# maxnorman569/Variational-Gridded-Gaussian-Processes

Measured on AMD Instinct MI355X. Metric: ELBO-step grid-points/sec (value + 5-component gradient), 1024x1024 RBF grid per GPU, higher is better.
Workload: dtype f64; 1 GPU; 2D Kronecker rbf GP (points basis), 1024x1024 grid (1024x1024 per GPU), m_d=128, Adam fit loop (lr 0.01), eigensolver warm start on; parallelism=single GPU

## Files before the change

include/vggp.h:

```cpp
#ifndef VGGP_H
#define VGGP_H

#include <stdint.h>

#ifdef __cplusplus
extern "C" {
#endif

#define VGGP_VERSION 200

#define VGGP_OK        0
#define VGGP_EINVAL   -1
#define VGGP_ENOTPD   -2
#define VGGP_EHIP     -3
#define VGGP_ENOMEM   -4
#define VGGP_ESTATE   -5
#define VGGP_ENOCONV  -6
#define VGGP_ERCCL    -7

#define VGGP_KIND_MATERN12 0
#define VGGP_KIND_MATERN32 1
#define VGGP_KIND_MATERN52 2
#define VGGP_KIND_RBF      3

#define VGGP_BASIS_POINTS 0
#define VGGP_BASIS_B0     1
#define VGGP_BASIS_ONE    2
#define VGGP_BASIS_VFF    3
#define VGGP_BASIS_B1     4

#define VGGP_FLAG_B0_F32_KDELTA 1
#define VGGP_FLAG_BLOCK_JACOBI 2
#define VGGP_FLAG_SCATTERED 4
#define VGGP_FLAG_PAIRED_Z 8

typedef struct vggp_ctx vggp_ctx;

typedef struct vggp_desc {
    int32_t kind1, basis1;
    int32_t kind2, basis2;
    int64_t n1, n2;
    int64_t m1, m2;
    int64_t n_total;
    const double* x1;
    const double* x2;
    const double* grid1;
    const double* grid2;
    int32_t warm_start;
    int32_t flags;
} vggp_desc;

typedef struct vggp_info {
    double jitter1, jitter2;
    int32_t sweeps1, sweeps2;
    int32_t rounds1, rounds2;
    int32_t status;
    int32_t polished;
} vggp_info;

int         vggp_version(void);
const char* vggp_last_error(void);

#define VGGP_UNIQUE_ID_BYTES 128
int vggp_create(vggp_ctx** out, int device, int n_ranks, int rank, const void* unique_id);
int vggp_destroy(vggp_ctx* ctx);
int vggp_unique_id(void* out );
typedef int (*vggp_allreduce_fn)(void* user, double* buf, int64_t count);
int vggp_set_allreduce(vggp_ctx* ctx, vggp_allreduce_fn fn, void* user);
int vggp_allreduce(vggp_ctx* ctx, double* buf, int64_t count, void* stream);
int vggp_comm_info(const vggp_ctx* ctx, int* n_ranks, int* rank, int* transport);
int vggp_plan(vggp_ctx* ctx, const vggp_desc* desc);
int64_t vggp_payload_len(const vggp_ctx* ctx);
int64_t vggp_workspace_bytes(const vggp_ctx* ctx);

int vggp_elbo_step(vggp_ctx* ctx, const double* Y, double yy_total, const double theta[5],
                   double* elbo_out, double grad_out[5], vggp_info* info, void* stream);

int vggp_elbo_partials(vggp_ctx* ctx, const double* Y, const double theta[5],
                       double* payload, void* stream);
int vggp_elbo_finish(vggp_ctx* ctx, const double* payload, double yy_total, const double theta[5],
                     double* elbo_out, double grad_out[5], vggp_info* info, void* stream);

int vggp_elbo_step_masked(vggp_ctx* ctx, const double* Ym, const double* W, double n_obs, double yy_obs,
                          const double theta[5], double* elbo_out, double grad_out[5], vggp_info* info, void* stream);
int vggp_elbo_step_masked_iter(vggp_ctx* ctx, const double* Ym, const double* W, double n_obs, double yy_obs,
                               const double theta[5], int n_probes, double tol, int max_iter, double* elbo_out, double grad_out[5],
                               vggp_info* info, void* stream);
int vggp_qv_masked(vggp_ctx* ctx, double* mean, double* var, void* stream);
int vggp_posterior_masked(vggp_ctx* ctx, const double* xs1, const double* xs2, int64_t n_star, double* mean, double* var,
                          void* stream);

#define VGGP_READOUT_LITERAL 1
int vggp_readout(vggp_ctx* ctx, const double* C1, int64_t mv1, const double* C2, int64_t mv2, const double* kd1, const double* kd2,
                 double* mean, double* var, int flags, void* stream);

int vggp_readout_masked(vggp_ctx* ctx, const double* C1, int64_t mv1, const double* C2, int64_t mv2, const double* kd1, const double* kd2,
                        double* mean, double* var, int flags, void* stream);

int vggp_qv(vggp_ctx* ctx, double* mean, double* var, void* stream);
int vggp_qv_cov(vggp_ctx* ctx, double* cov, void* stream);

int vggp_zgrad(vggp_ctx* ctx, const double* Y, double* gz1, double* gz2, void* stream);

int vggp_elbo_step_scattered(vggp_ctx* ctx, const double* y, double yy, const double theta[5], double* elbo_out,
                             double grad_out[5], vggp_info* info, void* stream);

int vggp_zgrad_scattered(vggp_ctx* ctx, const double* y, double* gz1, double* gz2, void* stream);

int vggp_set_inducing(vggp_ctx* ctx, int dim, const double* z, int64_t m);

int vggp_posterior(vggp_ctx* ctx, const double* xs1, const double* xs2, int64_t ns,
                   double* mean, double* var, void* stream);

int vggp_posterior_cov(vggp_ctx* ctx, const double* xs1, const double* xs2, int64_t ns, double* cov, void* stream);
int vggp_posterior_cov_masked(vggp_ctx* ctx, const double* xs1, const double* xs2, int64_t ns, double* cov, void* stream);
int vggp_qv_cov_masked(vggp_ctx* ctx, double* cov, void* stream);

int vggp_factor_build(vggp_ctx* ctx, int kind, int basis, const double* x, int64_t n,
                      const double* grid, int64_t m, double ell, int flags,
                      double* A0, double* dA0, double* K0, double* dK0, void* stream);

int vggp_cholesky_inverse(vggp_ctx* ctx, const double* K, int64_t m, double* L, double* Linv,
                          double* jitter_out, void* stream);

int vggp_eigh(vggp_ctx* ctx, const double* G, int64_t m, double* lam, double* Qt,
              int32_t* sweeps_out, int flags, void* stream);

int vggp_gemm(vggp_ctx* ctx, const double* A, int64_t sa_m, int64_t sa_k,
              const double* B, int64_t sb_k, int64_t sb_n,
              double* C, int64_t ldc, int64_t M, int64_t N, int64_t K, void* stream);

int vggp_trsm(vggp_ctx* ctx, const double* L, int64_t m, const double* R, int64_t ncols, double* X, int trans, void* stream);

int vggp_kron_solve(vggp_ctx* ctx, const double* L1, int64_t n1, const double* L2, int64_t n2,
                    const double* Y, double* X, void* stream);

#define VGGP_NSTAGE 20
int         vggp_profile(vggp_ctx* ctx, int enable);
int         vggp_profile_read(vggp_ctx* ctx, double ms_out[VGGP_NSTAGE], int32_t* steps_out, int reset);
const char* vggp_stage_name(int stage);
const char* vggp_project_kernel_name(void);

int vggp_sumsq(vggp_ctx* ctx, const double* y, int64_t n, double* out, void* stream);

#ifdef __cplusplus
}
#endif
#endif
```

variational_gridded_gaussian_processes_amd/_lib.py:

```python
from __future__ import annotations

import ctypes as C
import os

HERE = os.path.dirname(os.path.abspath(__file__))
LIB_PATH = os.path.join(HERE, "libvggp_hip.so")

VGGP_OK, VGGP_EINVAL, VGGP_ENOTPD, VGGP_EHIP, VGGP_ENOMEM, VGGP_ESTATE, VGGP_ENOCONV, VGGP_ERCCL = 0, -1, -2, -3, -4, -5, -6, -7
UNIQUE_ID_BYTES = 128
ALLREDUCE_FN = C.CFUNCTYPE(C.c_int, C.c_void_p, C.POINTER(C.c_double), C.c_int64)
KIND = {"matern12": 0, "matern32": 1, "matern52": 2, "rbf": 3}
NSTAGE = 20
FLAG_B0_F32_KDELTA = 1
FLAG_BLOCK_JACOBI = 2
FLAG_SCATTERED = 4
FLAG_PAIRED_Z = 8
BASIS = {"points": 0, "b0": 1, "one": 2, "vff": 3, "b1": 4}


class VggpError(RuntimeError):
    def __init__(self, code: int, msg: str):
        super().__init__(f"libvggp_hip: {msg} (code {code})")
        self.code = code


class Desc(C.Structure):
    _fields_ = [("kind1", C.c_int32), ("basis1", C.c_int32), ("kind2", C.c_int32), ("basis2", C.c_int32),
                ("n1", C.c_int64), ("n2", C.c_int64), ("m1", C.c_int64), ("m2", C.c_int64),
                ("n_total", C.c_int64),
                ("x1", C.c_void_p), ("x2", C.c_void_p), ("grid1", C.c_void_p), ("grid2", C.c_void_p),
                ("warm_start", C.c_int32), ("flags", C.c_int32)]


class Info(C.Structure):
    _fields_ = [("jitter1", C.c_double), ("jitter2", C.c_double),
                ("sweeps1", C.c_int32), ("sweeps2", C.c_int32),
                ("rounds1", C.c_int32), ("rounds2", C.c_int32),
                ("status", C.c_int32), ("polished", C.c_int32)]


_P, _I64, _D, _I = C.c_void_p, C.c_int64, C.c_double, C.c_int
SYMBOLS = {
    "vggp_version": (_I, []),
    "vggp_last_error": (C.c_char_p, []),
    "vggp_create": (_I, [C.POINTER(_P), _I, _I, _I, _P]),
    "vggp_unique_id": (_I, [_P]),
    "vggp_set_allreduce": (_I, [_P, ALLREDUCE_FN, _P]),
    "vggp_allreduce": (_I, [_P, _P, _I64, _P]),
    "vggp_comm_info": (_I, [_P, C.POINTER(_I), C.POINTER(_I), C.POINTER(_I)]),
    "vggp_destroy": (_I, [_P]),
    "vggp_plan": (_I, [_P, C.POINTER(Desc)]),
    "vggp_payload_len": (_I64, [_P]),
    "vggp_workspace_bytes": (_I64, [_P]),
    "vggp_elbo_step": (_I, [_P, _P, _D, C.POINTER(_D), C.POINTER(_D), C.POINTER(_D), C.POINTER(Info), _P]),
    "vggp_elbo_partials": (_I, [_P, _P, C.POINTER(_D), _P, _P]),
    "vggp_elbo_finish": (_I, [_P, _P, _D, C.POINTER(_D), C.POINTER(_D), C.POINTER(_D), C.POINTER(Info), _P]),
    "vggp_elbo_step_masked": (_I, [_P, _P, _P, _D, _D, C.POINTER(_D), C.POINTER(_D), C.POINTER(_D), C.POINTER(Info), _P]),
    "vggp_elbo_step_masked_iter": (_I, [_P, _P, _P, _D, _D, C.POINTER(_D), _I, _D, _I, C.POINTER(_D), C.POINTER(_D), C.POINTER(Info), _P]),
    "vggp_elbo_step_scattered": (_I, [_P, _P, _D, C.POINTER(_D), C.POINTER(_D), C.POINTER(_D), C.POINTER(Info), _P]),
    "vggp_qv_masked": (_I, [_P, _P, _P, _P]),
    "vggp_qv": (_I, [_P, _P, _P, _P]),
    "vggp_qv_cov": (_I, [_P, _P, _P]),
    "vggp_zgrad": (_I, [_P, _P, _P, _P, _P]),
    "vggp_zgrad_scattered": (_I, [_P, _P, _P, _P, _P]),
    "vggp_set_inducing": (_I, [_P, C.c_int, _P, C.c_int64]),
    "vggp_posterior": (_I, [_P, _P, _P, _I64, _P, _P, _P]),
    "vggp_readout": (_I, [_P, _P, _I64, _P, _I64, _P, _P, _P, _P, _I, _P]),
    "vggp_readout_masked": (_I, [_P, _P, _I64, _P, _I64, _P, _P, _P, _P, _I, _P]),
    "vggp_posterior_masked": (_I, [_P, _P, _P, _I64, _P, _P, _P]),
    "vggp_posterior_cov": (_I, [_P, _P, _P, _I64, _P, _P]),
    "vggp_posterior_cov_masked": (_I, [_P, _P, _P, _I64, _P, _P]),
    "vggp_qv_cov_masked": (_I, [_P, _P, _P]),
    "vggp_factor_build": (_I, [_P, _I, _I, _P, _I64, _P, _I64, _D, _I, _P, _P, _P, _P, _P]),
    "vggp_cholesky_inverse": (_I, [_P, _P, _I64, _P, _P, C.POINTER(_D), _P]),
    "vggp_eigh": (_I, [_P, _P, _I64, _P, _P, C.POINTER(C.c_int32), _I, _P]),
    "vggp_gemm": (_I, [_P, _P, _I64, _I64, _P, _I64, _I64, _P, _I64, _I64, _I64, _I64, _P]),
    "vggp_kron_solve": (_I, [_P, _P, _I64, _P, _I64, _P, _P, _P]),
    "vggp_trsm": (_I, [_P, _P, _I64, _P, _I64, _P, _I, _P]),
    "vggp_sumsq": (_I, [_P, _P, _I64, C.POINTER(_D), _P]),
    "vggp_profile": (_I, [_P, _I]),
    "vggp_profile_read": (_I, [_P, C.POINTER(_D), C.POINTER(C.c_int32), _I]),
    "vggp_stage_name": (C.c_char_p, [_I]),
    "vggp_project_kernel_name": (C.c_char_p, []),
}

_lib = None


def load() -> C.CDLL:
    global _lib
    if _lib is not None:
        return _lib
    if not os.path.exists(LIB_PATH):
        raise ImportError(
            f"{LIB_PATH} not found: build it with `python -m variational_gridded_gaussian_processes_amd.build` "
            "(needs hipcc); there is no CPU fallback")
    lib = C.CDLL(LIB_PATH)
    for name, (res, args) in SYMBOLS.items():
        fn = getattr(lib, name)
        fn.restype = res
        fn.argtypes = args
    _lib = lib
    return lib


def check(rc: int) -> None:
    if rc != VGGP_OK:
        msg = load().vggp_last_error()
        raise VggpError(rc, msg.decode() if msg else "unknown error")
```

variational_gridded_gaussian_processes_amd/build.py:

```python
from __future__ import annotations

import os
import shutil
import subprocess
import sys

HERE = os.path.dirname(os.path.abspath(__file__))
CSRC = os.path.join(HERE, "csrc")
SOURCES = ["api.hip", "gemm.hip", "factor_build.hip", "chol.hip", "trsm.hip", "eigh.hip", "mspace.hip", "thin.hip", "masked.hip", "comm.hip", "paired.hip"]
HEADERS = ["common.h", "ctx.h", "factor_elem.h", "gemm_body.h", os.path.join("..", "..", "include", "vggp.h")]
LIB = os.path.join(HERE, "libvggp_hip.so")


def _stale() -> bool:
    if not os.path.exists(LIB):
        return True
    t = os.path.getmtime(LIB)
    deps = [os.path.join(CSRC, s) for s in SOURCES] + [os.path.normpath(os.path.join(CSRC, h)) for h in HEADERS]
    return any(os.path.getmtime(d) > t for d in deps)


def build(force: bool = False, verbose: bool = False) -> str:
    if not force and not _stale():
        return LIB
    hipcc = shutil.which("hipcc") or "/opt/rocm/bin/hipcc"
    if not os.path.exists(hipcc):
        raise RuntimeError("hipcc not found: libvggp_hip.so cannot be built (ROCm toolchain required)")
    cmd = [hipcc, "--offload-arch=gfx950", "-O3", "-std=c++17", "-shared", "-fPIC", "-o", LIB + ".tmp"] + \
          [os.path.join(CSRC, s) for s in SOURCES] + ["-ldl"]
    if verbose:
        print(" ".join(cmd), file=sys.stderr)
    subprocess.run(cmd, check=True, cwd=CSRC)
    os.replace(LIB + ".tmp", LIB)
    return LIB


if __name__ == "__main__":
    print(build(force="--force" in sys.argv, verbose=True))
```

variational_gridded_gaussian_processes_amd/csrc/api.hip:

```cpp
#include "common.h"

#include <math.h>
#include <stdarg.h>
#include <stdio.h>
#include <stdlib.h>
#include <string.h>
#include <time.h>

#include <algorithm>
#include <vector>

static thread_local char g_err[512] = "";
void vg_set_error(const char* fmt, ...) {
    va_list ap;
    va_start(ap, fmt);
    vsnprintf(g_err, sizeof(g_err), fmt, ap);
    va_end(ap);
}
extern "C" const char* vggp_last_error(void) { return g_err; }
extern "C" int vggp_version(void) { return VGGP_VERSION; }

#include "ctx.h"
#include "factor_elem.h"
#define VG_CHOL_MAXJOBS_HOST 8
#define VG_SP_SLABS 4
#define VG_NEWTON_TOL 1e-12
#define VG_NEWTON_NULL 1e-12
#define VG_NEWTON_CLUSTER 1e-7
#define VG_NEWTON_NOISE 1e-13
#define VG_NEWTON_ACCEPT 1e-11

static void graphs_clear(vggp_ctx* c);
static int vg_quiesce(vggp_ctx* c);

static const char* VG_STAGE_NAMES[VGGP_NSTAGE] = {
    "factor_build", "cholesky_inverse", "trsm_BV(L^-1[A|dA|dK])", "extrap_basis(3 small gemms)", "gemm_project(S=[B2;V2]Y)",
    "gemm_C(B1*S)", "gemm_gram(G,H,Mk)", "reduce_slabs", "warm_first_gemm([Z,G]|TM)", "rowqr|refine", "warm_mid_gemms",
    "ritz_eigh", "warm_last_gemms(->Gw)", "jacobi_eigh+replay(fused)", "gemm_rotate_right", "gemm_rotate_left", "dstage",
    "gemm_betaGram", "final_reduce", "(unused)"};
extern "C" const char* vggp_stage_name(int i) { return (i >= 0 && i < VGGP_NSTAGE) ? VG_STAGE_NAMES[i] : ""; }

#define VG_MARK(id)                                                                                     \
    do {                                                                                                \
        if (c->prof && c->nev < VG_MAXEV) { VG_HIP(hipEventRecord(c->ev[c->nev], st)); c->ev_stage[c->nev++] = (id); } \
    } while (0)

static hipStream_t vg_side(vggp_ctx* c, hipStream_t st) {
    static const bool on = getenv("VGGP_FORK") != nullptr;
    return (c->prof || !on) ? st : c->side_stream;
}
#define VG_FORK(i)                                                                                      \
    do { if (sx != st) { VG_HIP(hipEventRecord(c->ev_fork[i], st)); VG_HIP(hipStreamWaitEvent(sx, c->ev_fork[i], 0)); } } while (0)
#define VG_JOIN_RECORD(i) do { if (sx != st) VG_HIP(hipEventRecord(c->ev_join[i], sx)); } while (0)
#define VG_JOIN_WAIT(i) do { if (sx != st) VG_HIP(hipStreamWaitEvent(st, c->ev_join[i], 0)); } while (0)

int vg_ensure_misc(vggp_ctx* c, size_t bytes) {
    if (c->misc_bytes >= bytes) return VGGP_OK;
    if (c->misc) { VG_HIP(hipFree(c->misc)); c->misc = nullptr; c->misc_bytes = 0; }
    VG_HIP(hipMalloc(&c->misc, bytes));
    c->misc_bytes = bytes;
    return VGGP_OK;
}

extern "C" int vggp_create(vggp_ctx** out, int device, int n_ranks, int rank, const void* unique_id) {
    if (!out) { vg_set_error("vggp_create: null out"); return VGGP_EINVAL; }
    VG_REQUIRE(n_ranks >= 1 && rank >= 0 && rank < n_ranks, "vggp_create: rank %d of %d", rank, n_ranks);
    int ndev = 0;
    VG_HIP(hipGetDeviceCount(&ndev));
    VG_REQUIRE(device >= 0 && device < ndev, "vggp_create: device %d out of range (%d devices)", device, ndev);
    VG_ENTER_DEVICE(device);
    hipDeviceProp_t prop;
    VG_HIP(hipGetDeviceProperties(&prop, device));
    if (strncmp(prop.gcnArchName, "gfx950", 6) != 0) {
        vg_set_error("vggp_create: device %d is %s; this library is built for gfx950 only", device, prop.gcnArchName);
        return VGGP_EHIP;
    }
    VG_HIP(vg_chol_setup());
    VG_HIP(vg_eigh_setup());
    VG_HIP(vg_trsm_setup());
    VG_HIP(vg_thin_tail_setup());
    vggp_ctx* c = new (std::nothrow) vggp_ctx();
    if (!c) { vg_set_error("out of host memory"); return VGGP_ENOMEM; }
    c->device = device;
    const char* ng = getenv("VGGP_NO_GRAPH");
    c->use_graph = !(ng && ng[0] == '1');
    VG_HIP(hipStreamCreate(&c->own_stream));
    VG_HIP(hipStreamCreateWithFlags(&c->side_stream, hipStreamNonBlocking));
    for (int i = 0; i < VG_NFORK; ++i) {
        VG_HIP(hipEventCreateWithFlags(&c->ev_fork[i], hipEventDisableTiming));
        VG_HIP(hipEventCreateWithFlags(&c->ev_join[i], hipEventDisableTiming));
    }
    VG_HIP(hipHostMalloc((void**)&c->h_theta, 8 * sizeof(double), hipHostMallocDefault));
    VG_HIP(hipHostMalloc((void**)&c->h_out, sizeof(HostOut), hipHostMallocDefault));
    VG_HIP(hipHostGetDevicePointer((void**)&c->d_hout, c->h_out, 0));
    VG_HIP(hipHostGetDevicePointer((void**)&c->d_htheta, c->h_theta, 0));
    VG_HIP(hipMalloc((void**)&c->ticket, 4 * sizeof(int)));
    VG_HIP(hipMemset(c->ticket, 0, 4 * sizeof(int)));
    VG_HIP(hipMalloc((void**)&c->sumsq_partial, 1024 * sizeof(double)));
    VG_HIP(hipMalloc((void**)&c->sumsq_out, 8 * sizeof(double)));
    const int rcc = vg_comm_init(c, n_ranks, rank, unique_id);
    if (rcc) { (void)vggp_destroy(c); return rcc; }
    *out = c;
    return VGGP_OK;
}

extern "C" int vggp_destroy(vggp_ctx* c) {
    if (!c) return VGGP_OK;
    VgDeviceGuard guard;
    (void)guard.enter(c->device);
    (void)vg_quiesce(c);
    for (int i = 0; i < 20; ++i) if (c->gexec[i]) (void)hipGraphExecDestroy(c->gexec[i]);
    for (int i = 0; i < VG_MAXEV; ++i) if (c->ev[i]) (void)hipEventDestroy(c->ev[i]);
    for (int i = 0; i < VG_NFORK; ++i) {
        if (c->ev_fork[i]) (void)hipEventDestroy(c->ev_fork[i]);
        if (c->ev_join[i]) (void)hipEventDestroy(c->ev_join[i]);
    }
    if (c->side_stream) (void)hipStreamDestroy(c->side_stream);
    vg_masked_free(c);
    vg_paired_free(c);
    vg_comm_destroy(c);
    if (c->own_stream) (void)hipStreamDestroy(c->own_stream);
    if (c->arena) (void)hipFree(c->arena);
    if (c->misc) (void)hipFree(c->misc);
    if (c->h_theta) (void)hipHostFree(c->h_theta);
    if (c->h_out) (void)hipHostFree(c->h_out);
    if (c->ticket) (void)hipFree(c->ticket);
    if (c->sumsq_partial) (void)hipFree(c->sumsq_partial);
    if (c->sumsq_out) (void)hipFree(c->sumsq_out);
    delete c;
    return VGGP_OK;
}

struct Bump {
    char* base;
    size_t off = 0;
    bool dry;
    template <typename T>
    T* take(size_t count) {
        off = (off + 255) & ~size_t(255);
        T* p = dry ? nullptr : reinterpret_cast<T*>(base + off);
        off += count * sizeof(T);
        return p;
    }
};

static int pick_split(int tiles, int K, int target) {
    int s = (target + tiles - 1) / tiles;
    int maxs = std::max(1, K / (4 * VG_BK));
    return std::max(1, std::min(s, maxs));
}

static long vg_grid_len(int basis, long m) {
    if (basis == VGGP_BASIS_B0) return m + 1;
    if (basis == VGGP_BASIS_VFF) return 2 + (m - 1) / 2 + 1;
    return m;
}
static int vg_uexp(int basis) { return (basis == VGGP_BASIS_VFF || basis == VGGP_BASIS_B1) ? -1 : 1; }

static void layout(vggp_ctx* c, Bump& b) {
    const vggp_desc& D = c->desc;
    const long n1 = D.n1, n2 = D.n2, m1 = D.m1, m2 = D.m2;
    c->out = b.take<double>(8);
    c->theta = b.take<double>(8);
    c->rowpart = b.take<double>(m1 * 8);
    c->r1 = b.take<double>(m1);
    c->r1l = b.take<double>(m1);
    c->r2 = b.take<double>(2 * m2);
    c->r2l = c->r2 + m2;
    c->dotpart = b.take<double>(64 * 4);
    c->ol = b.take<double>(2 * m1);
    for (int k = 0; k < 2; ++k) {
        VgDim& d = c->d[k];
        const long m = d.m, m2e = m + (m & 1);
        d.lam0 = b.take<double>(m);
        d.jitter = b.take<double>(2);
        d.counters = b.take<int>(8);
        d.counters2 = d.counters + 4;
        d.perm = b.take<int>(m2e);
        d.perm2 = b.take<int>(m2e);
        d.lam_s = b.take<double>(m);
        d.status = b.take<int>(2);
    }
    c->invD = b.take<double>(m1 * m2);
    c->beta = b.take<double>(m1 * m2);
    c->bl2 = b.take<double>(m1 * m2);
    c->bl1 = b.take<double>(m1 * m2);
    for (int k = 0; k < 2; ++k) {
        VgDim& d = c->d[k];
        d.E = b.take<double>((long)d.m * d.m);
        d.F = b.take<double>((long)d.m * d.m);
    }
    c->P3 = b.take<double>(3 * m1 * m2);
    c->T3 = b.take<double>(3 * m1 * m2);
    for (int k = 0; k < 2; ++k) {
        VgDim& d = c->d[k];
        const long m = d.m;
        d.TM = b.take<double>(m * m);
        d.TH = b.take<double>(m * m);
        d.Qt = b.take<double>(m * m);
        d.QtPrev = b.take<double>(m * m);
        d.QtPrev2 = b.take<double>(m * m);
        d.U = b.take<double>(m * m);
        d.Ep = b.take<double>(m * m);
        d.Fp = b.take<double>(m * m);
        d.Wp = b.take<double>(m * m);
        d.Id = b.take<double>(m * m);
        d.Gw = b.take<double>(m * m);
        d.GH = b.take<double>(2 * m * m);
        d.Mk = b.take<double>(m * m);
    }
    c->payload_len = 2 * m2 * m2 + 3 * m1 * m2;
    c->payload = b.take<double>(c->payload_len + 8);
    for (int k = 0; k < 2; ++k) {
        VgDim& d = c->d[k];
        const long m = d.m;
        const int glen = (int)vg_grid_len(d.basis, m);
        d.grid = b.take<double>(glen);
        d.K0 = b.take<double>(m * m);
        d.dK0 = b.take<double>(m * m);
        d.L0 = b.take<double>(m * m);
        d.Linv0 = b.take<double>(m * m);
        d.Dinv0 = b.take<double>(((m + 15) / 16) * 256);
        if (m > 128) {
            d.Kc = b.take<double>(4 * m * m); d.Lc = b.take<double>(4 * m * m); d.Dc = b.take<double>(4 * ((m + 15) / 16) * 256);
            d.st8 = b.take<int>(8);
        }
        d.X = b.take<double>(m * m);
        d.chol_scratch = b.take<double>(m * (m + 1));
        d.RQ = b.take<double>(m * m);
        d.RQsq = b.take<double>(m * m);
    }
    c->wq = b.take<double>(2 * m1 * m2);
    for (int k = 0; k < 2; ++k) {
        VgDim& d = c->d[k];
        const long m = d.m, n = d.n, m2e = m + (m & 1);
        d.x = b.take<double>(n);
        d.AD = b.take<double>(2 * m * n);
        d.BV = b.take<double>(2 * m * n);
        static const char* ghe = getenv("VGGP_GH_TARGET");
        d.gh_split = pick_split((int)(((m + 63) / 64) * ((m + 63) / 64)), (int)n, ghe ? atoi(ghe) : 32);
        d.GHslab = b.take<double>((size_t)d.gh_split * 2 * m * m);
        d.gwork = b.take<double>(m2e * (m2e + 1));
        d.max_rounds = (int)(VG_EIG_MAXSWEEP * (m2e - 1));
        d.rotlog = b.take<double2>(vg_eigh_log_bytes((int)m) / sizeof(double2) + 1);
        d.roundlog = b.take<int>(d.max_rounds);
        if (m >= 24 && m <= 256) {
            d.gwork2 = b.take<double>(m2e * (m2e + 1));
            d.rotlog2 = b.take<double2>(vg_eigh_log_bytes((int)m) / sizeof(double2) + 1);
            d.roundlog2 = b.take<int>(d.max_rounds);
            d.Zs = b.take<double>(m * m); d.V1s = b.take<double>(m * m); d.Hs = b.take<double>(m * m); d.Ws = b.take<double>(m * m);
            d.tMV = b.take<double>(VG_THIN_MAXR * m); d.tHV = b.take<double>(VG_THIN_MAXR * m);
            d.tAM = b.take<double>(VG_THIN_MAXR * VG_THIN_MAXR); d.tAH = b.take<double>(VG_THIN_MAXR * VG_THIN_MAXR);
            d.Omega = b.take<double>(VG_THIN_MAXR * m);
        }
    }
    const int st_tiles = (int)(((2 * m2 + 63) / 64) * ((n1 + 63) / 64));
    static const char* ste = getenv("VGGP_ST_TARGET");
    c->st_split = pick_split(st_tiles, (int)n2, ste ? atoi(ste) : 256);
    c->St = b.take<double>((size_t)std::max(c->st_split, VG_SP_SLABS) * 2 * m2 * n1);
    c->Sp = b.take<double>((size_t)VG_SP_SLABS * 2 * m2 * n1);
    const int cc_tiles = (int)(((2 * m1 + 63) / 64) * ((m2 + 63) / 64));
    const char* cce = getenv("VGGP_CC_TARGET");
    c->cc_split = pick_split(cc_tiles, (int)n1, cce ? atoi(cce) : 64);
    c->CCslab = b.take<double>((size_t)c->cc_split * 3 * m1 * m2);
    c->tCV = b.take<double>(3 * m1 * VG_THIN_MAXR);
    c->tAC = b.take<double>(3 * VG_THIN_MAXR * VG_THIN_MAXR + 64);
}

static int check_dim(int kind, int basis, long n, long m, const char* which) {
    VG_REQUIRE(kind >= 0 && kind <= 3, "vggp_plan: bad kind for %s", which);
    VG_REQUIRE(basis >= 0 && basis <= 4, "vggp_plan: bad basis for %s", which);
    VG_REQUIRE(!((basis == VGGP_BASIS_VFF || basis == VGGP_BASIS_B1) && kind != VGGP_KIND_MATERN12),
               "vggp_plan: the VFF and B1 features exist for Matern-1/2 only (%s)", which);
    VG_REQUIRE(!(basis == VGGP_BASIS_VFF && (m < 3 || (m & 1) == 0)), "vggp_plan: VFF needs m = 2M + 1 >= 3 (%s)", which);
    VG_REQUIRE(!(basis == VGGP_BASIS_B1 && m < 2), "vggp_plan: B1 needs at least 2 knots (%s)", which);
    VG_REQUIRE(!(basis == VGGP_BASIS_B0 && kind != VGGP_KIND_MATERN12),
               "vggp_plan: the B0 basis exists for Matern-1/2 only (%s)", which);
    VG_REQUIRE(n >= 1, "vggp_plan: %s has no observations", which);
    VG_REQUIRE(m >= 1 && m <= 256, "vggp_plan: m=%ld for %s outside [1, 256]", m, which);
    VG_REQUIRE(!(basis == VGGP_BASIS_ONE && m != 1), "vggp_plan: BASIS_ONE needs m=1 (%s)", which);
    return VGGP_OK;
}

extern "C" int vggp_plan(vggp_ctx* c, const vggp_desc* desc) {
    if (!c || !desc) { vg_set_error("vggp_plan: null argument"); return VGGP_EINVAL; }
    VG_ENTER_DEVICE(c->device);
    int rc;
    if (desc->flags & VGGP_FLAG_PAIRED_Z) {
        c->planned = false;
        graphs_clear(c);
        VG_HIP(hipDeviceSynchronize());
        c->have_partials = c->have_step = c->have_masked = false;
        c->acc_valid = false; c->last_payload = nullptr;
        c->is_paired = false;
        if ((rc = vg_paired_plan(c, desc))) return rc;
        c->desc = *desc;
        c->desc.x1 = c->desc.x2 = c->desc.grid1 = c->desc.grid2 = nullptr;
        c->desc.n_total = (desc->flags & VGGP_FLAG_SCATTERED) ? desc->n1 : desc->n1 * desc->n2;
        c->payload_len = 0;
        c->is_paired = true;
        c->planned = true;
        return VGGP_OK;
    }
    if (c->is_paired || c->paired) { VG_HIP(hipDeviceSynchronize()); vg_paired_free(c); c->is_paired = false; }
    if ((rc = check_dim(desc->kind1, desc->basis1, desc->n1, desc->m1, "dimension 1"))) return rc;
    if ((rc = check_dim(desc->kind2, desc->basis2, desc->n2, desc->m2, "dimension 2"))) return rc;
    VG_REQUIRE(desc->x1 && desc->x2, "vggp_plan: null coordinate arrays");
    VG_REQUIRE((desc->basis1 == VGGP_BASIS_ONE || desc->grid1) && (desc->basis2 == VGGP_BASIS_ONE || desc->grid2),
               "vggp_plan: null grid arrays");
    if (desc->flags & VGGP_FLAG_SCATTERED)
        VG_REQUIRE(desc->n1 == desc->n2 && desc->basis1 != VGGP_BASIS_ONE && desc->basis2 != VGGP_BASIS_ONE,
                   "vggp_plan: scattered points need n1 == n2 (one coordinate pair per point) and two real dimensions");
    else
        VG_REQUIRE(desc->n_total >= desc->n1 * desc->n2, "vggp_plan: n_total smaller than the local grid");
    VG_REQUIRE(desc->n1 < (1L << 24) && desc->n2 < (1L << 24), "vggp_plan: grid axis too long");
    c->planned = false;
    graphs_clear(c);
    VG_HIP(hipDeviceSynchronize());
    c->warm_run = 0;
    c->refine_next = false;
    c->sub_next = false; c->sub_mode = false; c->sub_r_cap[0] = c->sub_r_cap[1] = 0;
    c->pred_consumed = false;
    c->acc_valid = false; c->last_warm = false; c->last_slabs = false; c->last_payload = nullptr;
    c->last_thin = false; c->thin_off = false; c->thin_block = 0;
    c->cur_newton = 0; c->last_newton = false; c->newton_next = false; c->newton_block = 0; c->newton_iters = 3; c->newton_ok_run = 0;
    c->desc = *desc;
    c->d[0] = VgDim();
    c->d[1] = VgDim();
    c->d[0].kind = desc->kind1; c->d[0].basis = desc->basis1; c->d[0].n = (int)desc->n1; c->d[0].m = (int)desc->m1;
    c->d[1].kind = desc->kind2; c->d[1].basis = desc->basis2; c->d[1].n = (int)desc->n2; c->d[1].m = (int)desc->m2;
    Bump dry{nullptr, 0, true};
    layout(c, dry);
    const size_t need = dry.off + 4096;
    if (need > c->arena_bytes) {
        if (c->arena) { VG_HIP(hipFree(c->arena)); c->arena = nullptr; c->arena_bytes = 0; }
        VG_HIP(hipMalloc(&c->arena, need));
        c->arena_bytes = need;
    }
    Bump wet{reinterpret_cast<char*>(c->arena), 0, false};
    layout(c, wet);
    c->arena_used = wet.off;
    VG_HIP(hipMemset(c->arena, 0, c->arena_used));
    const double one = 1.0;
    for (int k = 0; k < 2; ++k) {
        VgDim& d = c->d[k];
        const double* hx = k == 0 ? desc->x1 : desc->x2;
        const double* hg = k == 0 ? desc->grid1 : desc->grid2;
        VG_HIP(hipMemcpy(d.x, hx, sizeof(double) * d.n, hipMemcpyHostToDevice));
        if (d.basis == VGGP_BASIS_ONE) {
            VG_HIP(hipMemcpy(d.grid, &one, sizeof(double), hipMemcpyHostToDevice));
        } else {
            const int glen = (int)vg_grid_len(d.basis, d.m);
            VG_HIP(hipMemcpy(d.grid, hg, sizeof(double) * glen, hipMemcpyHostToDevice));
        }
    }
    for (int k = 0; k < 2; ++k) VG_HIP(vg_identity_launch(c->d[k].Id, c->d[k].m, nullptr));
    for (int k = 0; k < 2; ++k) {
        VgDim& d = c->d[k];
        if (!d.Omega) continue;
        std::vector<double> om((size_t)VG_THIN_MAXR * d.m);
        unsigned long long z = 0x9E3779B97F4A7C15ull * (unsigned long long)(k + 1);
        for (double& v : om) {
            z += 0x9E3779B97F4A7C15ull;
            unsigned long long x = z;
            x = (x ^ (x >> 30)) * 0xBF58476D1CE4E5B9ull; x = (x ^ (x >> 27)) * 0x94D049BB133111EBull; x ^= x >> 31;
            v = (double)(x >> 11) * (2.0 / 9007199254740992.0) - 1.0;
        }
        VG_HIP(hipMemcpy(d.Omega, om.data(), sizeof(double) * om.size(), hipMemcpyHostToDevice));
    }
    VG_HIP(hipDeviceSynchronize());
    c->desc.x1 = c->desc.x2 = c->desc.grid1 = c->desc.grid2 = nullptr;
    c->have_partials = c->have_step = c->have_masked = false;
    vg_masked_new_plan(c);
    c->planned = true;
    return VGGP_OK;
}

extern "C" int vggp_set_inducing(vggp_ctx* c, int dim, const double* z, int64_t m) {
    if (c && c->is_paired) {
        if (!c->planned) { vg_set_error("context not planned"); return VGGP_ESTATE; }
        VG_ENTER_DEVICE(c->device);
        return vg_paired_set_inducing(c, dim, z, m);
// ... 38 lines not shown
                else
                    vg_gemm_add(&g, q.X + k0, q.sc, 1, Tp, t_k, t_i, q.X + r0, (int)q.sc, (int)q.ncols, (int)rb, (int)kn, 1, 0, 1, 0,
                                -1.0, 1);
            }
            if (nt >= 12) { vg_set_error("trsm_batch: too many jobs"); return VGGP_EINVAL; }
            tj[nt++] = VgTrsmJob{q.L + r0 * q.ldl + r0, q.Dinv + (r0 / 16) * q.dinv_blk, q.X + r0 * q.sk, q.X + r0 * q.sk, q.ldl,
                                 q.dinv_blk, q.dinv_ld, q.sk, q.sc, q.sk, q.sc, q.ncols, (int)rb, q.trans};
        }
        if (g.nprob) VG_HIP(vg_gemm_launch(&g, st));
        if (nt) VG_HIP(vg_trsm_launch(tj, nt, st));
    }
    return VGGP_OK;
}
static int trsm_inplace(const double* L, long m, long ldl, const double* Dinv, double* X, long x_sk, long x_sc, long ncols,
                        int trans, hipStream_t st) {
    VgTrsmSpec q{L, ldl, Dinv, 256, 16, X, x_sk, x_sc, ncols, m, trans};
    return trsm_batch(&q, 1, st);
}

static bool vg_ride(const vggp_ctx* c) {
    static const bool off = getenv("VGGP_NO_RIDE") != nullptr;
    return !off && !c->prof && c->desc.m1 <= 128 && c->desc.m2 <= 128;
}

static int vg_chol_big_enqueue(vggp_ctx* c, const int* dims, int ndims, hipStream_t st) {
    VgCholJob cj[VG_CHOL_MAXJOBS_HOST];
    int nj = 0;
    for (int t = 0; t < ndims; ++t) {
        VgDim& d = c->d[dims[t]];
        VG_HIP(vg_jitcopy_launch(d.K0, d.m, d.Kc, st));
    }
    const long NB = 128;
    for (int stage = 0; stage < 2; ++stage) {
        if (stage == 1) {
            VgTrsmJob tj[8];
            int nt = 0;
            VgGemmBatch g;
            vg_gemm_init(&g);
            for (int t = 0; t < ndims; ++t) {
                VgDim& d = c->d[dims[t]];
                const long m = d.m, mm = m * m, rest = m - NB, nb16 = (m + 15) / 16;
                for (int l = 0; l < 4; ++l) {
                    double* Kl = d.Kc + l * mm;
                    double* Ll = d.Lc + l * mm;
                    tj[nt++] = VgTrsmJob{Ll, d.Dc + l * nb16 * 256, Kl + NB * m, Ll + NB * m, m, 256, 16, 1, m, 1, m, rest, (int)NB, 0};
                    vg_gemm_add(&g, Ll + NB * m, m, 1, Ll + NB * m, 1, m, Kl + NB * m + NB, (int)m, (int)rest, (int)rest, (int)NB, 1, 0, 1, 0, -1.0, 1);
                }
            }
            VG_HIP(vg_trsm_launch(tj, nt, st));
            VG_HIP(vg_gemm_launch(&g, st));
        }
        nj = 0;
        for (int t = 0; t < ndims; ++t) {
            VgDim& d = c->d[dims[t]];
            const long m = d.m, mm = m * m, nb16 = (m + 15) / 16;
            const long o = stage ? NB : 0;
            const int mb = stage ? (int)(m - NB) : (int)NB;
            for (int l = 0; l < 4; ++l) {
                VgCholJob j{d.Kc + l * mm + o * m + o, d.Lc + l * mm + o * m + o, nullptr, d.chol_scratch, nullptr, d.st8 + 2 * l + stage, mb};
                j.ldk = (int)m; j.ldl = (int)m; j.only_level0 = 1;
                j.Dinv_out = d.Dc + l * nb16 * 256 + (o / 16) * 256;
                cj[nj++] = j;
            }
        }
        VG_HIP(vg_chol_launch(cj, nj, st));
    }
    for (int t = 0; t < ndims; ++t) {
        VgDim& d = c->d[dims[t]];
        VG_HIP(vg_cholsel_launch(d.Lc, d.Dc, d.st8, d.m, d.L0, d.Dinv0, d.jitter, d.status, st));
    }
    return VGGP_OK;
}

int vg_partials_enqueue(vggp_ctx* c, const double* Y, double* payload, hipStream_t st, bool reduce, bool extrap, bool fused, bool apply_ns,
                        int early) {
    const long n1 = c->desc.n1, n2 = c->desc.n2, m1 = c->desc.m1, m2 = c->desc.m2;
    VgDim &d1 = c->d[0], &d2 = c->d[1];
    hipStream_t sx = vg_side(c, st);
    VgGemmBatch g;
    VG_MARK(-1);

    VgFactorJob fj[2];
    VgCholJob cj[2];
    static const bool chol_legacy = getenv("VGGP_CHOL_LEGACY") != nullptr;
    const bool dinv_path = d1.m <= VG_TRSM_BLK && d2.m <= VG_TRSM_BLK && !chol_legacy;
    VgClearArgs clr;
    clr.n = 0;
    for (int k = 0; k < 2; ++k) {
        VgDim& d = c->d[k];
        fj[k] = VgFactorJob{d.x, d.grid, d.AD, d.AD + (long)d.m * d.n, d.K0, d.dK0, d.n, d.m, d.kind, d.basis, k, 0.0, c->desc.flags};
        clr.ptr[clr.n] = d.status; clr.nwords[clr.n++] = 2;
        clr.ptr[clr.n] = reinterpret_cast<int*>(d.chol_scratch); clr.nwords[clr.n++] = 16;
        clr.ptr[clr.n] = d.counters; clr.nwords[clr.n++] = 8;
        if (k == 0) { clr.ptr[clr.n] = reinterpret_cast<int*>(c->payload + c->payload_len); clr.nwords[clr.n++] = 2; }
        if (d.st8) { clr.ptr[clr.n] = d.st8; clr.nwords[clr.n++] = 8; }
        cj[k] = VgCholJob{d.K0, d.L0, dinv_path ? nullptr : d.Linv0, d.chol_scratch, d.jitter, d.status, d.m};
        cj[k].Dinv_out = d.Dinv0;
    }
    VG_HIP(vg_factor_build_launch(fj, 2, c->d_htheta, st, c->theta, &clr));
    VG_MARK(0);

    const bool ns_on_chol = extrap && apply_ns && dinv_path;
    VgGemmBatch gns;
    vg_gemm_init(&gns);
    if (ns_on_chol)
        for (int k = 0; k < 2; ++k) {
            VgDim& d = c->d[k];
            vg_gemm_add(&gns, d.Wp, d.m, 1, d.Ep, d.m, 1, d.Fp, d.m, d.m, d.m, d.m, 1, 0, 1, 0, -0.5, 1);
        }
    static const bool chol_big_off = getenv("VGGP_NO_CHOL_BIG") != nullptr;
    const bool any_big = (d1.m > VG_TRSM_BLK || d2.m > VG_TRSM_BLK) && !chol_legacy && !chol_big_off;
    VgGemmBatch gsp;
    vg_gemm_init(&gsp);
    int sp_slabs = 1;
    if (early) {
        const bool ok_fused = fused && !reduce && (vg_ride(c) || c->prof);
        const bool ok_partials = reduce;
        if (!(dinv_path && !any_big && (ok_fused || ok_partials) && Y && sx == st)) {
            vg_set_error("internal: the early projection was requested where it cannot run");
            return VGGP_ESTATE;
        }
        vg_gemm_add(&gsp, d2.AD, n2, 1, Y, n1, 1, c->Sp, (int)n1, (int)(2 * m2), (int)n1, (int)n2, std::min(c->st_split, VG_SP_SLABS), 2L * m2 * n1);
        sp_slabs = gsp.p[0].ksplit;
        if (c->prof) {
            vg_gemm_xcd_group(&gsp, 0);
            VG_HIP(vg_gemm_launch(&gsp, st, VG_GEMM_TAG_GRAM_PROJECT));
            VG_MARK(4);
        }
    }
    if (!any_big) {
        VgGemmBatch gr2 = gns;
        if (early && !c->prof) {
            gr2 = gsp;
            if (ns_on_chol)
                for (int k = 0; k < 2; ++k) {
                    VgDim& d = c->d[k];
                    vg_gemm_add(&gr2, d.Wp, d.m, 1, d.Ep, d.m, 1, d.Fp, d.m, d.m, d.m, d.m, 1, 0, 1, 0, -0.5, 1);
                }
        }
        VG_HIP(vg_chol_launch(cj, 2, st, ((early && !c->prof) || ns_on_chol) ? &gr2 : nullptr));
    } else {
        int big[2], nbig = 0;
        for (int k = 0; k < 2; ++k) {
            if (c->d[k].m > VG_TRSM_BLK) big[nbig++] = k;
            else { cj[k].Linv = nullptr; VG_HIP(vg_chol_launch(&cj[k], 1, st)); }
        }
        const int rcb = vg_chol_big_enqueue(c, big, nbig, st);
        if (rcb) return rcb;
    }
    c->dinv_valid = dinv_path || any_big;
    VG_MARK(1);

    {
        const bool big = d1.m > VG_TRSM_BLK || d2.m > VG_TRSM_BLK;
        if (!big) {
            VgTrsmJob tj[16];
            int nt = 0;
            for (int k = 0; k < 2; ++k) {
                VgDim& d = c->d[k];
                const long mn = (long)d.m * d.n;
                const double* dv = dinv_path ? d.Dinv0 : d.Linv0;
                const long dblk = dinv_path ? 256 : 16L * d.m + 16, dld = dinv_path ? 16 : d.m;
                for (int b = 0; b < 2; ++b)
                    tj[nt++] = VgTrsmJob{d.L0, dv, d.AD + b * mn, d.BV + b * mn, d.m, dblk, dld, d.n, 1, d.n, 1, d.n, d.m, 0};
                tj[nt++] = VgTrsmJob{d.L0, dv, d.dK0, d.X, d.m, dblk, dld, d.m, 1, d.m, 1, d.m, d.m, 0};
                if (dinv_path) {
                    tj[nt] = VgTrsmJob{d.L0, dv, d.L0, d.Linv0, d.m, dblk, dld, d.m, 1, d.m, 1, d.m, d.m, 0};
                    tj[nt++].rhs_ident = 1;
                }
            }
            if (early)
                for (int sl = 0; sl < sp_slabs; ++sl)
                    for (int b = 0; b < 2; ++b) {
                        const long o = (long)sl * 2 * m2 * n1 + (long)b * m2 * n1;
                        tj[nt++] = VgTrsmJob{d2.L0, d2.Dinv0, c->Sp + o, c->St + o, m2, 256, 16, n1, 1, n1, 1, n1, (int)m2, 0};
                    }
            VG_HIP(vg_trsm_launch(tj, nt, st));
        } else {
            VgTrsmSpec q[8];
            int nq = 0;
            for (int k = 0; k < 2; ++k) {
                VgDim& d = c->d[k];
                const long mn = (long)d.m * d.n;
                const double* dv = any_big ? d.Dinv0 : d.Linv0;
                const long dblk = any_big ? 256 : 16L * d.m + 16, dld = any_big ? 16 : d.m;
                VG_HIP(hipMemcpyAsync(d.BV, d.AD, sizeof(double) * 2 * mn, hipMemcpyDeviceToDevice, st));
                VG_HIP(hipMemcpyAsync(d.X, d.dK0, sizeof(double) * d.m * d.m, hipMemcpyDeviceToDevice, st));
                for (int b = 0; b < 2; ++b) q[nq++] = VgTrsmSpec{d.L0, d.m, dv, dblk, dld, d.BV + b * mn, d.n, 1, d.n, d.m, 0};
                q[nq++] = VgTrsmSpec{d.L0, d.m, dv, dblk, dld, d.X, d.m, 1, d.m, d.m, 0};
                if (any_big) {
                    VG_HIP(hipMemcpyAsync(d.Linv0, d.Id, sizeof(double) * d.m * d.m, hipMemcpyDeviceToDevice, st));
                    q[nq++] = VgTrsmSpec{d.L0, d.m, dv, dblk, dld, d.Linv0, d.m, 1, d.m, d.m, 0};
                }
            }
            const int rc = trsm_batch(q, nq, st);
            if (rc) return rc;
        }
    }
    VG_MARK(2);

    if (!Y) {
        vg_gemm_init(&g);
        for (int k = 0; k < 2; ++k) {
            VgDim& d = c->d[k];
            vg_gemm_add(&g, d.X, d.m, 1, d.Linv0, 1, d.m, d.Mk, d.m, d.m, d.m, d.m);
        }
        VG_HIP(vg_gemm_launch(&g, st));
        return VGGP_OK;
    }
    hipStream_t sp = (fused && !extrap) ? sx : st;
    const bool ride = fused && !reduce && sp == st && vg_ride(c);
    if (sp != st) VG_FORK(1);
    VgGemmBatch gp, gc;
    vg_gemm_init(&gp);
    vg_gemm_add(&gp, d2.BV, n2, 1, Y, n1, 1, c->St, (int)n1, (int)(2 * m2), (int)n1, (int)n2, c->st_split, 2L * m2 * n1);
    const int st_slabs = early ? sp_slabs : gp.p[0].ksplit;
    vg_gemm_xcd_group(&gp, 0);
    auto add_ns = [&](VgGemmBatch* b) {
        if (extrap && apply_ns && !ns_on_chol)
            for (int k = 0; k < 2; ++k) {
                VgDim& d = c->d[k];
                vg_gemm_add(b, d.Wp, d.m, 1, d.Ep, d.m, 1, d.Fp, d.m, d.m, d.m, d.m, 1, 0, 1, 0, -0.5, 1);
            }
    };
    if (!ride && !early) {
        add_ns(&gp);
        VG_HIP(vg_gemm_launch(&gp, sp, VG_GEMM_TAG_GRAM_PROJECT));
        if (sp == st) VG_MARK(4);
    }
    vg_gemm_init(&gc);
    const long cc_slab = 3L * m1 * m2;
    vg_gemm_add(&gc, d1.BV, n1, 1, c->St, 1, n1, c->CCslab, (int)m2, (int)(2 * m1), (int)m2, (int)n1, c->cc_split, cc_slab,
                st_slabs, 2L * m2 * n1);
    vg_gemm_add(&gc, d1.BV, n1, 1, c->St + m2 * n1, 1, n1, c->CCslab + 2 * m1 * m2, (int)m2, (int)m1, (int)m2, (int)n1,
                c->cc_split, cc_slab, st_slabs, 2L * m2 * n1);
    const int cc_slabs = gc.p[0].ksplit;
    int gh_slabs[2] = {1, 1};
    auto add_gram = [&](VgGemmBatch* b) {
        for (int k = 0; k < 2; ++k) {
            VgDim& d = c->d[k];
            const int ig = vg_gemm_add(b, d.BV, d.n, 1, d.BV, 1, d.n, d.GHslab, d.m, 2 * d.m, d.m, d.n, d.gh_split, 2L * d.m * d.m);
            gh_slabs[k] = b->p[ig].ksplit;
            vg_gemm_add(b, d.X, d.m, 1, d.Linv0, 1, d.m, d.Mk, d.m, d.m, d.m, d.m);
        }
    };
    if (ride) {
        vg_gemm_init(&g);
        add_gram(&g);
        add_ns(&g);
        VG_HIP(vg_gemm_launch(&g, st));
        c->ride_proj = gp; c->ride_cc = gc;
        c->ride_pending = early != 1;
        c->ride_stage0 = early == 2 ? 1 : 0;
    } else {
        if (sp == st) add_gram(&gc);
        VG_HIP(vg_gemm_launch(&gc, sp));
        if (sp == st) { VG_MARK(5); VG_MARK(6); }
        if (sp != st) {
            VG_JOIN_RECORD(1);
            vg_gemm_init(&g);
            add_gram(&g);
            VG_HIP(vg_gemm_launch(&g, st));
            VG_MARK(6);
        }
    }

    c->gh_slabs[0] = gh_slabs[0]; c->gh_slabs[1] = gh_slabs[1]; c->cc_slabs = cc_slabs; c->st_slabs = st_slabs;
    if (!reduce) return VGGP_OK;
    if (sp != st) VG_JOIN_WAIT(1);
    VgRedBatch r;
    vg_red_init(&r);
    vg_red_add(&r, d1.GHslab, d1.GH, 2L * m1 * m1, 2L * m1 * m1, gh_slabs[0]);
    vg_red_add(&r, d2.GHslab, payload, 2L * m2 * m2, 2L * m2 * m2, gh_slabs[1]);
    vg_red_add(&r, c->CCslab, payload + 2 * m2 * m2, 3L * m1 * m2, cc_slab, cc_slabs);
    VG_HIP(vg_red_launch(&r, st));
    VG_MARK(7);
    return VGGP_OK;
}

static bool vg_sub_ident() { static const bool ex = getenv("VGGP_SUB_EXTRAP") != nullptr; return !ex; }

static int finish_enqueue(vggp_ctx* c, const double* payload, double yy_total, bool warm, hipStream_t st, bool copy_theta,
                          bool from_slabs = false, bool extrap = false, bool refine = false, bool subspace = false, bool thin = false,
                          int newton = 0, bool thin_early = false) {
    if (copy_theta) VG_HIP(hipMemcpyAsync(c->theta, c->h_theta, 6 * sizeof(double), hipMemcpyHostToDevice, st));
    const long m1 = c->desc.m1, m2 = c->desc.m2;
    VgDim &d1 = c->d[0], &d2 = c->d[1];
    const double* G0[2] = {from_slabs ? d1.GHslab : d1.GH, from_slabs ? d2.GHslab : payload};
    const double* H0[2] = {G0[0] + m1 * m1, G0[1] + m2 * m2};
    const double* C3 = from_slabs ? c->CCslab : payload + 2 * m2 * m2;
    const int ghn[2] = {from_slabs ? c->gh_slabs[0] : 1, from_slabs ? c->gh_slabs[1] : 1};
    const long ghs[2] = {2L * m1 * m1, 2L * m2 * m2};
    const int ccn = from_slabs ? c->cc_slabs : 1;
    const long ccs = 3L * m1 * m2;
    VgGemmBatch g;
    const bool ride = from_slabs && c->ride_pending;
    int ride_stage = ride ? c->ride_stage0 : 0;

    hipStream_t sx = vg_side(c, st);
    VG_MARK(-1);
    const double* Hr[2] = {H0[0], H0[1]};
    int hrn[2] = {ghn[0], ghn[1]};
    VgEigJob ej[2];
    if (warm && subspace && thin) {
        const bool early = thin_early && !ride;
        const double* Gr[2] = {G0[0], G0[1]};
        int grn[2] = {ghn[0], ghn[1]};
        double* gdst[2] = {d1.GH, c->payload};
        vg_gemm_init(&g);
        for (int k = 0; k < 2; ++k) {
            VgDim& d = c->d[k];
            vg_gemm_add(&g, d.QtPrev, d.m, 1, G0[k], d.m, 1, d.TM, d.m, d.sub_r, d.m, d.m, 1, 0, ghn[k], ghs[k]);
            if (from_slabs && ghn[k] > 1) {
                vg_gemm_add(&g, d.Id, d.m, 1, G0[k], d.m, 1, gdst[k], d.m, d.m, d.m, d.m, 1, 0, ghn[k], ghs[k]);
                vg_gemm_add(&g, d.Id, d.m, 1, H0[k], d.m, 1, gdst[k] + (long)d.m * d.m, d.m, d.m, d.m, d.m, 1, 0, ghn[k], ghs[k]);
            }
        }
        VG_HIP(vg_gemm_launch(&g, st));
        VG_MARK(8);
        for (int k = 0; k < 2; ++k)
            if (from_slabs && ghn[k] > 1) { Gr[k] = gdst[k]; grn[k] = 1; Hr[k] = gdst[k] + (long)c->d[k].m * c->d[k].m; hrn[k] = 1; }
        VgRowQrJob qj[2];
        for (int k = 0; k < 2; ++k) { VgDim& d = c->d[k]; qj[k] = VgRowQrJob{d.TM, d.V1s, d.sub_r, d.m, nullptr, nullptr, 0}; }
        VG_HIP(vg_rowqr_launch(qj, 2, st, early ? ((c->prof || !from_slabs) ? nullptr : &c->ride_cc) : (ride ? &c->ride_proj : nullptr)));
        if (ride) ride_stage = 1;
        VG_MARK(9);
        vg_gemm_init(&g);
        for (int k = 0; k < 2; ++k) {
            VgDim& d = c->d[k];
            const int r = d.sub_r;
            vg_gemm_add(&g, d.V1s, d.m, 1, Gr[k], d.m, 1, d.Zs, d.m, r, d.m, d.m, 1, 0, grn[k], ghs[k]);
            vg_gemm_add(&g, d.V1s, d.m, 1, d.Mk, d.m, 1, d.tMV, d.m, r, d.m, d.m);
            vg_gemm_add(&g, d.V1s, d.m, 1, Hr[k], d.m, 1, d.tHV, d.m, r, d.m, d.m, 1, 0, hrn[k], ghs[k]);
        }
        if (early) {
            const int ic = vg_gemm_add(&g, C3, m2, 1, d2.V1s, 1, m2, c->tCV, d2.sub_r, (int)(3 * m1), d2.sub_r, (int)m2);
            g.p[ic].a_nslab = ccn; g.p[ic].a_slab = ccs;
        }
        VG_HIP(vg_gemm_launch(&g, st));
        VG_MARK(10);
        VgGemmBatch gx;
        vg_gemm_init(&gx);
        if (ride) gx = c->ride_cc;
        for (int k = 0; k < 2; ++k) {
            VgDim& d = c->d[k];
            const int r = d.sub_r;
            vg_gemm_add(&gx, d.tMV, d.m, 1, d.V1s, 1, d.m, d.tAM, r, r, r, d.m);
            vg_gemm_add(&gx, d.tHV, d.m, 1, d.V1s, 1, d.m, d.tAH, r, r, r, d.m);
        }
        if (early)
            for (int q = 0; q < 3; ++q)
                vg_gemm_add(&gx, d1.V1s, m1, 1, c->tCV + (long)q * m1 * d2.sub_r, d2.sub_r, 1, c->tAC + (long)q * d1.sub_r * d2.sub_r,
                            d2.sub_r, d1.sub_r, d2.sub_r, (int)m1);
        VgEigJob sj[2];
        for (int k = 0; k < 2; ++k) {
            VgDim& d = c->d[k];
            sj[k] = VgEigJob{nullptr, d.lam_s, d.Ws, nullptr, d.gwork2, d.rotlog2, d.roundlog2, d.counters2, d.sub_r, d.max_rounds,
                             (long)vg_eigh_log_bytes(d.m), 0};
            sj[k].Hl = d.Zs; sj[k].Hr = d.V1s; sj[k].hk = d.m;
            sj[k].perm = d.perm2;
            sj[k].err = d.status + 1;
            sj[k].newton = 1;
        }
        VG_HIP(vg_eigh_launch(sj, 2, st, &gx));
        if (ride) ride_stage = 2;
        c->ride_pending = false;
        VG_MARK(11);
        const int ac_nslab = 1;
        const long ac_slab = 3L * d1.sub_r * d2.sub_r;
        if (!early) {
            vg_gemm_init(&g);
            {
                const int ic = vg_gemm_add(&g, C3, m2, 1, d2.V1s, 1, m2, c->tCV, d2.sub_r, (int)(3 * m1), d2.sub_r, (int)m2);
                g.p[ic].a_nslab = ccn; g.p[ic].a_slab = ccs;
            }
            for (int k = 0; k < 2; ++k) {
                VgDim& d = c->d[k];
                vg_gemm_add(&g, d.Ws, d.sub_r, 1, d.V1s, d.m, 1, d.QtPrev, d.m, d.sub_r, d.m, d.sub_r);
            }
            VG_HIP(vg_gemm_launch(&g, st));
            VG_MARK(14);
            vg_gemm_init(&g);
            for (int q = 0; q < 3; ++q)
                vg_gemm_add(&g, d1.V1s, m1, 1, c->tCV + (long)q * m1 * d2.sub_r, d2.sub_r, 1, c->tAC + (long)q * d1.sub_r * d2.sub_r, d2.sub_r,
                            d1.sub_r, d2.sub_r, (int)m1);
            VG_HIP(vg_gemm_launch(&g, st));
            VG_MARK(15);
        }
        VgThinTail tt{};
        tt.theta = c->theta; tt.n_total = (double)c->desc.n_total; tt.yy = yy_total;
        tt.r1 = d1.sub_r; tt.r2 = d2.sub_r; tt.m1 = (int)m1; tt.m2 = (int)m2;
        tt.W1 = d1.Ws; tt.W2 = d2.Ws; tt.lam1 = d1.lam_s; tt.lam2 = d2.lam_s;
        tt.AM1 = d1.tAM; tt.AH1 = d1.tAH; tt.AM2 = d2.tAM; tt.AH2 = d2.tAH; tt.AC = c->tAC;
        tt.ac_nslab = ac_nslab; tt.ac_slab = ac_slab;
        tt.G1 = Gr[0]; tt.H1 = Hr[0]; tt.G2 = Gr[1]; tt.H2 = Hr[1];
        tt.out = c->out; tt.hout = c->d_hout;
        tt.beta_out = c->beta; tt.invd_out = c->invD;
        tt.peer_fail = (payload == c->payload && (c->n_ranks > 1 || c->comm || c->cb)) ? c->payload + c->payload_len : nullptr;
        for (int k = 0; k < 2; ++k) { tt.jit[k] = c->d[k].jitter; tt.status[k] = c->d[k].status; tt.rcounters[k] = c->d[k].counters2; }
#ifdef VGGP_DIAG
        tt.stamps = reinterpret_cast<unsigned long long*>(c->tAC + 3 * VG_THIN_MAXR * VG_THIN_MAXR);
#endif
        VG_HIP(vg_thin_tail_launch(&tt, st));
        VG_MARK(18);
        if (early) {
            vg_gemm_init(&g);
            for (int k = 0; k < 2; ++k) {
                VgDim& d = c->d[k];
                vg_gemm_add(&g, d.Ws, d.sub_r, 1, d.V1s, d.m, 1, d.QtPrev, d.m, d.sub_r, d.m, d.sub_r);
            }
            VG_HIP(vg_gemm_launch(&g, st));
        }
        return VGGP_OK;
    }
    if (warm && subspace) {
        VgRowQrJob qj[2];
        const double* Gr[2] = {G0[0], G0[1]};
        int grn[2] = {ghn[0], ghn[1]};
        double* gdst[2] = {d1.GH, c->payload};
        vg_gemm_init(&g);
        for (int k = 0; k < 2; ++k) {
            VgDim& d = c->d[k];
            vg_gemm_add(&g, d.Fp, d.m, 1, G0[k], d.m, 1, d.TM, d.m, d.m, d.m, d.m, 1, 0, ghn[k], ghs[k]);
            if (from_slabs && ghn[k] > 1) {
                vg_gemm_add(&g, d.Id, d.m, 1, G0[k], d.m, 1, gdst[k], d.m, d.m, d.m, d.m, 1, 0, ghn[k], ghs[k]);
                vg_gemm_add(&g, d.Id, d.m, 1, H0[k], d.m, 1, gdst[k] + (long)d.m * d.m, d.m, d.m, d.m, d.m, 1, 0, ghn[k], ghs[k]);
            }
        }
        VG_HIP(vg_gemm_launch(&g, st));
        VG_MARK(8);
        for (int k = 0; k < 2; ++k)
            if (from_slabs && ghn[k] > 1) { Gr[k] = gdst[k]; grn[k] = 1; Hr[k] = gdst[k] + (long)c->d[k].m * c->d[k].m; hrn[k] = 1; }
        for (int k = 0; k < 2; ++k) {
            VgDim& d = c->d[k];
            const long r = d.sub_r;
            qj[k] = VgRowQrJob{d.TM, d.V1s, d.sub_r, d.m, d.Fp + r * d.m, d.E + r * d.m, (long)(d.m - r) * d.m};
        }
        VG_HIP(vg_rowqr_launch(qj, 2, st, ride ? &c->ride_proj : nullptr));
        if (ride) ride_stage = 1;
        VG_MARK(9);
        vg_gemm_init(&g);
        for (int k = 0; k < 2; ++k) {
            VgDim& d = c->d[k];
            const long r = d.sub_r;
            vg_gemm_add(&g, d.V1s, d.m, 1, Gr[k], d.m, 1, d.Zs, d.m, (int)r, d.m, d.m, 1, 0, grn[k], ghs[k]);
            vg_gemm_add(&g, d.Fp + r * d.m, d.m, 1, d.V1s, 1, d.m, d.TH, (int)r, (int)(d.m - r), (int)r, d.m);
        }
        VG_HIP(vg_gemm_launch(&g, st));
        VG_MARK(10);
        VgGemmBatch gx;
        vg_gemm_init(&gx);
        if (ride) gx = c->ride_cc;
        for (int k = 0; k < 2; ++k) {
            VgDim& d = c->d[k];
            const long r = d.sub_r;
            vg_gemm_add(&gx, d.TH, r, 1, d.V1s, d.m, 1, d.E + r * d.m, d.m, (int)(d.m - r), d.m, (int)r, 1, 0, 1, 0, -1.0, 1);
            vg_gemm_add(&gx, d.TH, r, 1, d.Zs, d.m, 1, d.TM + r * d.m, d.m, (int)(d.m - r), d.m, (int)r, 1, 0, 1, 0, -1.0, 1);
        }
        VgEigJob sj[2];
        for (int k = 0; k < 2; ++k) {
            VgDim& d = c->d[k];
            sj[k] = VgEigJob{nullptr, d.lam_s, d.Ws, nullptr, d.gwork2, d.rotlog2, d.roundlog2, d.counters2, d.sub_r, d.max_rounds,
                             (long)vg_eigh_log_bytes(d.m), 0};
            sj[k].Hl = d.Zs; sj[k].Hr = d.V1s; sj[k].hk = d.m;
            sj[k].perm = d.perm2;
            sj[k].err = d.status + 1;
            sj[k].newton = 1;
        }
        VG_HIP(vg_eigh_launch(sj, 2, st, &gx));
        if (ride) ride_stage = 2;
        VG_MARK(11);
        vg_gemm_init(&g);
        for (int k = 0; k < 2; ++k) {
            VgDim& d = c->d[k];
            const long r = d.sub_r;
            vg_gemm_add(&g, d.Ws, r, 1, d.V1s, d.m, 1, d.E, d.m, (int)r, d.m, (int)r);
            vg_gemm_add(&g, d.Ws, r, 1, d.Zs, d.m, 1, d.TM, d.m, (int)r, d.m, (int)r);
        }
        VG_HIP(vg_gemm_launch(&g, st));
        vg_gemm_init(&g);
        for (int k = 0; k < 2; ++k) {
            VgDim& d = c->d[k];
            vg_gemm_add(&g, d.TM, d.m, 1, d.E, 1, d.m, d.Gw, d.m, d.m, d.m, d.m);
        }
        VG_HIP(vg_gemm_launch(&g, st));
    } else if (warm && newton > 0) {
        const double* Gr[2] = {G0[0], G0[1]};
        int grn[2] = {ghn[0], ghn[1]};
        double* gdst[2] = {d1.GH, c->payload};
        const double* Scur[2] = {extrap ? d1.Fp : d1.QtPrev, extrap ? d2.Fp : d2.QtPrev};
        vg_gemm_init(&g);
        for (int k = 0; k < 2; ++k) {
            VgDim& d = c->d[k];
            vg_gemm_add(&g, Scur[k], d.m, 1, G0[k], d.m, 1, d.TM, d.m, d.m, d.m, d.m, 1, 0, ghn[k], ghs[k]);
            if (from_slabs && ghn[k] > 1) {
                vg_gemm_add(&g, d.Id, d.m, 1, G0[k], d.m, 1, gdst[k], d.m, d.m, d.m, d.m, 1, 0, ghn[k], ghs[k]);
                vg_gemm_add(&g, d.Id, d.m, 1, H0[k], d.m, 1, gdst[k] + (long)d.m * d.m, d.m, d.m, d.m, d.m, 1, 0, ghn[k], ghs[k]);
            }
        }
        VG_HIP(vg_gemm_launch(&g, st));
        VG_MARK(8);
        for (int k = 0; k < 2; ++k)
            if (from_slabs && ghn[k] > 1) { Gr[k] = gdst[k]; grn[k] = 1; Hr[k] = gdst[k] + (long)c->d[k].m * c->d[k].m; hrn[k] = 1; }
        vg_gemm_init(&g);
        for (int k = 0; k < 2; ++k) { VgDim& d = c->d[k]; vg_gemm_add(&g, d.TM, d.m, 1, Scur[k], 1, d.m, d.Gw, d.m, d.m, d.m, d.m); }
        VG_HIP(vg_gemm_launch(&g, st));
        VG_MARK(12);
        static const bool newton_null = getenv("VGGP_NO_NULL_SKIP") == nullptr;
        int bi = 0;
        for (int it = 0; it < newton; ++it) {
            VgRefineJob rj[2];
            for (int k = 0; k < 2; ++k) {
                VgDim& d = c->d[k];
                rj[k] = VgRefineJob{d.Gw, d.U, d.TH, d.m, VG_NEWTON_TOL};
                rj[k].emax = 0.3; rj[k].flag = d.counters2; rj[k].noise = VG_NEWTON_NOISE;
                if (newton_null) { rj[k].lam_prev = d.lam0; rj[k].null_cut = it == 0 ? VG_NEWTON_CLUSTER : VG_NEWTON_NULL; }
            }
            const VgGemmBatch* rd = !ride ? nullptr : (ride_stage == 0 ? &c->ride_proj : (ride_stage == 1 ? &c->ride_cc : nullptr));
            VG_HIP(vg_refine_launch(rj, 2, st, rd));
            if (rd) ++ride_stage;
            VG_MARK(9);
            vg_gemm_init(&g);
            for (int k = 0; k < 2; ++k) { VgDim& d = c->d[k]; vg_gemm_add(&g, d.U, d.m, 1, d.U, d.m, 1, d.TH, d.m, d.m, d.m, d.m, 1, 0, 1, 0, 0.5, 1); }
            VG_HIP(vg_gemm_launch(&g, st));
            double* Snew[2];
            vg_gemm_init(&g);
            for (int k = 0; k < 2; ++k) {
                VgDim& d = c->d[k];
                double* bufs[3] = {d.E, d.X, d.F};
                Snew[k] = bufs[bi];
                vg_gemm_add(&g, d.TH, d.m, 1, Scur[k], d.m, 1, Snew[k], d.m, d.m, d.m, d.m);
            }
            VG_HIP(vg_gemm_launch(&g, st));
            bi = (bi + 1) % 3;
            if (it + 1 < newton) {
                double* Sns[2];
                vg_gemm_init(&g);
                for (int k = 0; k < 2; ++k) {
                    VgDim& d = c->d[k];
                    double* bufs[3] = {d.E, d.X, d.F};
                    Sns[k] = bufs[bi];
                    vg_gemm_add(&g, Snew[k], d.m, 1, Snew[k], 1, d.m, d.TM, d.m, d.m, d.m, d.m);
                    vg_gemm_add(&g, d.Id, d.m, 1, Snew[k], d.m, 1, Sns[k], d.m, d.m, d.m, d.m, 1, 0, 1, 0, 1.5, 0);
                }
                VG_HIP(vg_gemm_launch(&g, st));
                vg_gemm_init(&g);
                for (int k = 0; k < 2; ++k) { VgDim& d = c->d[k]; vg_gemm_add(&g, d.TM, d.m, 1, Snew[k], d.m, 1, Sns[k], d.m, d.m, d.m, d.m, 1, 0, 1, 0, -0.5, 1); }
                VG_HIP(vg_gemm_launch(&g, st));
                bi = (bi + 1) % 3;
                for (int k = 0; k < 2; ++k) Scur[k] = Sns[k];
            } else {
                for (int k = 0; k < 2; ++k) Scur[k] = Snew[k];
            }
            vg_gemm_init(&g);
            for (int k = 0; k < 2; ++k) { VgDim& d = c->d[k]; vg_gemm_add(&g, Scur[k], d.m, 1, Gr[k], d.m, 1, d.TM, d.m, d.m, d.m, d.m, 1, 0, grn[k], ghs[k]); }
            VG_HIP(vg_gemm_launch(&g, st));
            vg_gemm_init(&g);
            for (int k = 0; k < 2; ++k) { VgDim& d = c->d[k]; vg_gemm_add(&g, d.TM, d.m, 1, Scur[k], 1, d.m, d.Gw, d.m, d.m, d.m, d.m); }
            VG_HIP(vg_gemm_launch(&g, st));
        }
        VgNewtonCheckJob nj[2];
        for (int k = 0; k < 2; ++k) {
            VgDim& d = c->d[k];
            nj[k] = VgNewtonCheckJob{d.Gw, d.lam0, d.counters, d.status + 1, d.counters2, d.m, newton, VG_NEWTON_ACCEPT, VG_NEWTON_NOISE};
            if (newton_null) nj[k].null_cut = VG_NEWTON_NULL;
            VG_HIP(hipMemcpyAsync(d.Qt, Scur[k], sizeof(double) * d.m * d.m, hipMemcpyDeviceToDevice, st));
        }
        VG_HIP(vg_newton_check_launch(nj, 2, st));
        {
            const int* er[2] = {d1.status + 1, d2.status + 1};
            const double* sa[2] = {Scur[0], Scur[1]};
            double* da[2] = {d1.QtPrev, d2.QtPrev};
            const double* sb[2] = {d1.QtPrev, d2.QtPrev};
            double* db[2] = {d1.QtPrev2, d2.QtPrev2};
            const long nn[2] = {m1 * m1, m2 * m2};
            VG_HIP(vg_copy_if_launch(er, sa, da, sb, db, nn, 2, st));
        }
        VG_MARK(13);
        while (ride && ride_stage < 2) {
            VG_HIP(vg_gemm_launch(ride_stage == 0 ? &c->ride_proj : &c->ride_cc, st));
            ++ride_stage;
        }
    } else if (warm) {
        const double* Gr[2] = {G0[0], G0[1]};
        int grn[2] = {ghn[0], ghn[1]};
        double* gdst[2] = {d1.GH, c->payload};
        vg_gemm_init(&g);
        for (int k = 0; k < 2; ++k) {
            VgDim& d = c->d[k];
            vg_gemm_add(&g, extrap ? d.Fp : d.QtPrev, d.m, 1, G0[k], d.m, 1, d.TM, d.m, d.m, d.m, d.m, 1, 0, ghn[k], ghs[k]);
            if (from_slabs && ghn[k] > 1) {
                if (refine) {
                    vg_gemm_add(&g, d.Id, d.m, 1, G0[k], d.m, 1, gdst[k], d.m, d.m, d.m, d.m, 1, 0, ghn[k], ghs[k]);
                    Gr[k] = gdst[k]; grn[k] = 1;
                }
                vg_gemm_add(&g, d.Id, d.m, 1, H0[k], d.m, 1, gdst[k] + (long)d.m * d.m, d.m, d.m, d.m, d.m, 1, 0, ghn[k], ghs[k]);
                Hr[k] = gdst[k] + (long)d.m * d.m; hrn[k] = 1;
            }
        }
        VG_HIP(vg_gemm_launch(&g, st));
        VG_MARK(8);
        vg_gemm_init(&g);
        for (int k = 0; k < 2; ++k) {
            VgDim& d = c->d[k];
            vg_gemm_add(&g, d.TM, d.m, 1, extrap ? d.Fp : d.QtPrev, 1, d.m, d.Gw, d.m, d.m, d.m, d.m);
        }
        VG_HIP(vg_gemm_launch(&g, st));
        VG_MARK(12);
        if (refine) {
            VgRefineJob rj[2];
            static const bool null_skip = getenv("VGGP_NO_NULL_SKIP") == nullptr;
            for (int k = 0; k < 2; ++k) {
                VgDim& d = c->d[k];
                rj[k] = VgRefineJob{d.Gw, d.U, d.TH, d.m, 0.0};
                if (null_skip) { rj[k].lam_prev = d.lam0; rj[k].null_cut = 1e-12; }
            }
            {
                const VgGemmBatch* rr = !ride ? nullptr : (ride_stage == 0 ? &c->ride_proj : (ride_stage == 1 ? &c->ride_cc : nullptr));
                VG_HIP(vg_refine_launch(rj, 2, st, rr));
                if (rr) ++ride_stage;
            }
            VG_MARK(9);
            vg_gemm_init(&g);
            for (int k = 0; k < 2; ++k) {
                VgDim& d = c->d[k];
                const double* S0 = extrap ? d.Fp : d.QtPrev;
                vg_gemm_add(&g, d.TH, d.m, 1, S0, d.m, 1, d.E, d.m, d.m, d.m, d.m);
                vg_gemm_add(&g, d.U, d.m, 1, d.U, d.m, 1, d.X, d.m, d.m, d.m, d.m);
            }
            VG_HIP(vg_gemm_launch(&g, st));
            vg_gemm_init(&g);
            for (int k = 0; k < 2; ++k) {
                VgDim& d = c->d[k];
                const double* S0 = extrap ? d.Fp : d.QtPrev;
                vg_gemm_add(&g, d.X, d.m, 1, S0, d.m, 1, d.E, d.m, d.m, d.m, d.m, 1, 0, 1, 0, 0.5, 1);
            }
            VG_HIP(vg_gemm_launch(&g, st));
            vg_gemm_init(&g);
            for (int k = 0; k < 2; ++k) {
                VgDim& d = c->d[k];
                vg_gemm_add(&g, d.E, d.m, 1, Gr[k], d.m, 1, d.TM, d.m, d.m, d.m, d.m, 1, 0, grn[k], ghs[k]);
            }
            VG_HIP(vg_gemm_launch(&g, st));
            vg_gemm_init(&g);
            for (int k = 0; k < 2; ++k) {
                VgDim& d = c->d[k];
                vg_gemm_add(&g, d.TM, d.m, 1, d.E, 1, d.m, d.Gw, d.m, d.m, d.m, d.m);
            }
            VG_HIP(vg_gemm_launch(&g, st));
        }
    }
    VG_MARK(12);
    for (int k = 0; k < 2; ++k) {
        VgDim& d = c->d[k];
        ej[k] = VgEigJob{warm ? d.Gw : G0[k], d.lam0, d.Qt, warm ? ((refine || subspace) ? d.E : (extrap ? d.Fp : d.QtPrev)) : nullptr, d.gwork, d.rotlog, d.roundlog,
                         d.counters, d.m, d.max_rounds, (long)vg_eigh_log_bytes(d.m),
                         (c->desc.flags & VGGP_FLAG_BLOCK_JACOBI) ? 1 : 0};
        ej[k].Qt2 = d.QtPrev;
        ej[k].perm = d.perm;
        ej[k].cp_src = d.QtPrev; ej[k].cp_dst = d.QtPrev2;
        ej[k].err = d.status + 1;
        ej[k].polish0 = (warm && refine) ? 1 : 0;
        ej[k].sparse_first = (warm && subspace) ? 1 : 0;
        ej[k].null_from = (warm && subspace) ? d.sub_r : 0;
    }
    const VgGemmBatch* mr = !ride ? nullptr : (ride_stage == 0 ? &c->ride_proj : (ride_stage == 1 ? &c->ride_cc : nullptr));
    if (!(warm && newton > 0)) {
        VG_HIP(vg_eigh_launch(ej, 2, st, mr));
        VG_MARK(13);
        if (mr) ++ride_stage;
    }
    if (ride && ride_stage == 1) { VG_HIP(vg_gemm_launch(&c->ride_cc, st)); ride_stage = 2; }
    c->ride_pending = false;
    if (from_slabs) VG_JOIN_WAIT(1);

    vg_gemm_init(&g);
    for (int k = 0; k < 2; ++k) {
        VgDim& d = c->d[k];
        vg_gemm_add(&g, d.Mk, d.m, 1, d.Qt, 1, d.m, d.TM, d.m, d.m, d.m, d.m);
        const int ih = vg_gemm_add(&g, Hr[k], d.m, 1, d.Qt, 1, d.m, d.TH, d.m, d.m, d.m, d.m);
        g.p[ih].a_nslab = hrn[k]; g.p[ih].a_slab = ghs[k];
    }
    const int ic = vg_gemm_add(&g, C3, m2, 1, d2.Qt, 1, m2, c->T3, (int)m2, (int)(3 * m1), (int)m2, (int)m2);
    g.p[ic].a_nslab = ccn; g.p[ic].a_slab = ccs;
    const bool predict = c->desc.warm_start && !(c->desc.flags & VGGP_FLAG_BLOCK_JACOBI);
    const bool pred_ident = c->sub_mode && vg_sub_ident();
    if (predict && !pred_ident)
        for (int k = 0; k < 2; ++k) {
            VgDim& d = c->d[k];
            vg_gemm_add(&g, d.QtPrev, d.m, 1, d.QtPrev2, 1, d.m, d.U, d.m, d.m, d.m, d.m);
        }
    VG_HIP(vg_gemm_launch(&g, st));
    VG_MARK(14);
    vg_gemm_init(&g);
    for (int k = 0; k < 2; ++k) {
        VgDim& d = c->d[k];
        vg_gemm_add(&g, d.Qt, d.m, 1, d.TM, d.m, 1, d.E, d.m, d.m, d.m, d.m);
        vg_gemm_add(&g, d.Qt, d.m, 1, d.TH, d.m, 1, d.F, d.m, d.m, d.m, d.m);
    }
    for (int q = 0; q < 3; ++q)
        vg_gemm_add(&g, d1.Qt, m1, 1, c->T3 + q * m1 * m2, m2, 1, c->P3 + q * m1 * m2, (int)m2, (int)m1, (int)m2, (int)m1);
    if (predict)
        for (int k = 0; k < 2; ++k) {
            VgDim& d = c->d[k];
            const double* Uk = pred_ident ? d.Id : d.U;
            vg_gemm_add(&g, Uk, d.m, 1, d.QtPrev, d.m, 1, d.Ep, d.m, d.m, d.m, d.m);
            vg_gemm_add(&g, Uk, d.m, 1, d.QtPrev, d.m, 1, d.Fp, d.m, d.m, d.m, d.m, 1, 0, 1, 0, 1.5, 0);
        }
    VG_HIP(vg_gemm_launch(&g, st));
    VG_MARK(15);

    VgMspace ms;
    ms.theta = c->theta; ms.lam1 = d1.lam0; ms.lam2 = d2.lam0; ms.P3 = c->P3;
    ms.E1 = d1.E; ms.F1 = d1.F; ms.E2 = d2.E; ms.F2 = d2.F;
    ms.beta = c->beta; ms.bl2 = c->bl2; ms.bl1 = c->bl1; ms.invD = c->invD;
    ms.rowpart = c->rowpart; ms.r1 = c->r1; ms.r1l = c->r1l; ms.out = c->out;
    ms.r2 = c->r2; ms.r2l = c->r2l; ms.dotp = c->dotpart; ms.ol = c->ol;
    ms.m1 = (int)m1; ms.m2 = (int)m2; ms.n_total = (double)c->desc.n_total; ms.yy = yy_total;
    ms.ticket = c->ticket; ms.hout = c->d_hout;
    ms.peer_fail = (payload == c->payload && (c->n_ranks > 1 || c->comm || c->cb)) ? c->payload + c->payload_len : nullptr;
    for (int k = 0; k < 2; ++k) { ms.jit[k] = c->d[k].jitter; ms.status[k] = c->d[k].status; ms.counters[k] = c->d[k].counters; }
    VG_HIP(vg_dstage_launch(&ms, st));
    VG_MARK(16);
    vg_gemm_init(&g);
    {
        const int idot[4] = {
            vg_gemm_add(&g, d1.E, 1, m1, c->beta, m2, 1, nullptr, (int)m2, (int)m1, (int)m2, (int)m1),
            vg_gemm_add(&g, d1.F, 1, m1, c->bl2, m2, 1, nullptr, (int)m2, (int)m1, (int)m2, (int)m1),
            vg_gemm_add(&g, c->beta, m2, 1, d2.E, m2, 1, nullptr, (int)m2, (int)m1, (int)m2, (int)m2),
            vg_gemm_add(&g, c->bl1, m2, 1, d2.F, m2, 1, nullptr, (int)m2, (int)m1, (int)m2, (int)m2)};
        for (int q = 0; q < 4; ++q) { g.p[idot[q]].dotw = c->beta; g.p[idot[q]].dotw_ld = (int)m2; g.p[idot[q]].dot_out = c->dotpart + 64 * q; }
        vg_gemm_add(&g, c->ol, m1, 1, c->invD, m2, 1, c->r2, (int)m2, 2, (int)m2, (int)m1);
    }
    if (predict)
        for (int k = 0; k < 2; ++k) {
            VgDim& d = c->d[k];
            vg_gemm_add(&g, d.Ep, d.m, 1, d.Ep, 1, d.m, d.Wp, d.m, d.m, d.m, d.m);
        }
    VG_HIP(vg_gemm_launch(&g, st));
    VG_MARK(17);
    VG_HIP(vg_final_launch(&ms, st));
    VG_MARK(18);

    return VGGP_OK;
}

enum { VG_G_PARTIALS = 0, VG_G_PARTIALS_X, VG_G_FINISH_COLD, VG_G_FINISH_WARM, VG_G_FINISH_WARM_X, VG_G_STEP_COLD, VG_G_STEP_WARM,
       VG_G_STEP_WARM_X, VG_G_FINISH_WARM_XR, VG_G_STEP_WARM_XR, VG_G_FINISH_WARM_S, VG_G_STEP_WARM_S, VG_G_FINISH_WARM_T, VG_G_STEP_WARM_T,
       VG_G_FINISH_WARM_N, VG_G_STEP_WARM_N, VG_G_PARTIALS_E, VG_G_FINISH_WARM_TE, VG_G_STEP_COLD_T, VG_G_PARTIALS_XE, VG_G_COUNT };
static_assert(VG_G_COUNT <= 20, "vggp_ctx::gexec");

static void graphs_clear(vggp_ctx* c) {
    (void)vg_quiesce(c);
    for (int i = 0; i < VG_G_COUNT; ++i) {
        if (c->gexec[i]) { (void)hipGraphExecDestroy(c->gexec[i]); c->gexec[i] = nullptr; }
        c->gkey[i] = VgGraphKey();
    }
}

template <typename F>
static int run_graph(vggp_ctx* c, int which, const VgGraphKey& key, hipStream_t st, F enqueue, bool bypass = false) {
    if (!c->use_graph || c->prof || bypass) return enqueue();
    if (!c->gexec[which] || !(c->gkey[which] == key)) {
        if (c->gexec[which]) { (void)vg_quiesce(c); (void)hipGraphExecDestroy(c->gexec[which]); c->gexec[which] = nullptr; }
        VG_HIP(hipStreamBeginCapture(st, hipStreamCaptureModeThreadLocal));
        const int rc = enqueue();
        hipGraph_t graph = nullptr;
        const hipError_t e = hipStreamEndCapture(st, &graph);
        if (rc) { if (graph) (void)hipGraphDestroy(graph); return rc; }
        if (e != hipSuccess) { vg_set_error("hipStreamEndCapture -> %s", hipGetErrorString(e)); return VGGP_EHIP; }
        const hipError_t ei = hipGraphInstantiate(&c->gexec[which], graph, nullptr, nullptr, 0);
        (void)hipGraphDestroy(graph);
        if (ei != hipSuccess) { c->gexec[which] = nullptr; vg_set_error("hipGraphInstantiate -> %s", hipGetErrorString(ei)); return VGGP_EHIP; }
        c->gkey[which] = key;
    }
    VG_HIP(hipGraphLaunch(c->gexec[which], st));
    return VGGP_OK;
}

static bool vg_refine(const vggp_ctx* c, bool extrap) {
    static const bool off = getenv("VGGP_NO_REFINE") != nullptr;
    return !off && extrap && c->refine_next;
}

static bool vg_extrapolate(const vggp_ctx* c) {
    static const bool off = getenv("VGGP_NO_EXTRAP") != nullptr;
    return !off && c->desc.warm_start && !(c->desc.flags & VGGP_FLAG_BLOCK_JACOBI) && c->d[0].have_prev && c->d[1].have_prev &&
           c->d[0].have_prev2 && c->d[1].have_prev2;
}

struct VgStart { bool extrap, refine, subspace, thin; int newton; };
static bool vg_thin_ok(const vggp_ctx* c, bool own_payload) {
    static const bool off = getenv("VGGP_NO_THIN") != nullptr;
    if (off || c->thin_off || c->thin_block > 0 || !own_payload || !c->desc.warm_start || (c->desc.flags & VGGP_FLAG_BLOCK_JACOBI) || !c->sub_next) return false;
    for (int k = 0; k < 2; ++k) {
        const VgDim& d = c->d[k];
        if (!d.have_prev || !d.tMV || d.sub_r < 1 || d.sub_r > VG_THIN_MAXR || d.sub_r > d.thin_rows) return false;
    }
    return true;
}
static bool vg_warm(vggp_ctx* c, bool own_payload) {
    bool warm = c->desc.warm_start && c->d[0].have_prev && c->d[1].have_prev;
    if (warm && (c->d[0].thin_rows < c->d[0].m || c->d[1].thin_rows < c->d[1].m) && !vg_thin_ok(c, own_payload)) {
        c->warm_run = 0;
        for (int k = 0; k < 2; ++k) c->d[k].have_prev = c->d[k].have_prev2 = false;
        warm = false;
    }
    return warm;
}
static int vg_start_prepare(vggp_ctx* c, bool warm, hipStream_t st, VgStart* out, bool own_payload) {
    out->thin = warm && vg_thin_ok(c, own_payload);
    out->extrap = !out->thin && vg_extrapolate(c);
    const bool lds_sized = c->d[0].m <= 128 && c->d[1].m <= 128;
    out->subspace = out->thin || (lds_sized && warm && out->extrap && c->sub_next && c->d[0].sub_r > 0 && c->d[1].sub_r > 0);
    {
        static const bool off = getenv("VGGP_NO_NEWTON_CHAIN") != nullptr;
        static const char* ite = getenv("VGGP_NEWTON_ITERS");
        const bool big = c->d[0].m > 128 || c->d[1].m > 128;
        const bool roomy = c->d[0].m >= 96 && c->d[1].m >= 96;
        const bool want = warm && !out->subspace && out->extrap && !off && c->newton_block == 0 && (big || (c->newton_next && roomy)) &&
                          !(c->desc.flags & VGGP_FLAG_BLOCK_JACOBI) && c->d[0].m >= 8 && c->d[1].m >= 8;
        out->newton = want ? (ite ? atoi(ite) : c->newton_iters) : 0;
        if (c->newton_block > 0) --c->newton_block;
    }
    out->refine = warm && !out->subspace && !out->newton && vg_refine(c, out->extrap);
    c->sub_mode = out->subspace;
    if (out->subspace && (c->sub_r_cap[0] != c->d[0].sub_r || c->sub_r_cap[1] != c->d[1].sub_r)) {
        for (int v : {(int)VG_G_FINISH_WARM_S, (int)VG_G_STEP_WARM_S, (int)VG_G_FINISH_WARM_T, (int)VG_G_STEP_WARM_T, (int)VG_G_FINISH_WARM_TE})
            if (c->gexec[v]) { (void)vg_quiesce(c); (void)hipGraphExecDestroy(c->gexec[v]); c->gexec[v] = nullptr; c->gkey[v] = VgGraphKey(); }
        c->sub_r_cap[0] = c->d[0].sub_r; c->sub_r_cap[1] = c->d[1].sub_r;
    }
    if (out->newton && out->newton != c->newton_cap) {
        for (int v : {(int)VG_G_FINISH_WARM_N, (int)VG_G_STEP_WARM_N})
            if (c->gexec[v]) { (void)vg_quiesce(c); (void)hipGraphExecDestroy(c->gexec[v]); c->gexec[v] = nullptr; c->gkey[v] = VgGraphKey(); }
        c->newton_cap = out->newton;
    }
    c->cur_thin = out->thin;
    c->cur_extrap = out->extrap;
    c->cur_newton = out->newton;
    c->cur_r[0] = c->d[0].sub_r; c->cur_r[1] = c->d[1].sub_r;
    return VGGP_OK;
}

static int set_theta(vggp_ctx* c, const double theta[5]) {
    for (int i = 0; i < 5; ++i) {
        VG_REQUIRE(theta[i] > 0.0 && std::isfinite(theta[i]), "theta[%d]=%g must be positive and finite", i, theta[i]);
        c->h_theta[i] = theta[i];
    }
    c->h_theta[5] = (double)(++c->seq);
    return VGGP_OK;
}

static int vg_quiesce(vggp_ctx* c) {
    if (c->poll_stream_valid) { c->poll_stream_valid = false; VG_HIP(hipStreamSynchronize(c->poll_stream)); }
    return VGGP_OK;
}
static int vg_wait_step(vggp_ctx* c, hipStream_t st) {
    static const bool nopoll = getenv("VGGP_NO_POLL") != nullptr;
    const volatile double* seq = &c->h_out->seq;
    const double want = c->h_theta[5];
    if (nopoll || c->prof || (c->n_ranks > 1 && !c->comm && !c->cb)) { c->poll_stream_valid = false; return vg_comm_wait(c, st); }
    if (c->comm && !c->cb) {
        const int wrc = vg_comm_wait(c, st, seq, want);
        c->poll_stream = st; c->poll_stream_valid = (wrc == VGGP_OK);
        return wrc;
    }
    timespec t0, t1;
    clock_gettime(CLOCK_MONOTONIC, &t0);
    for (long spin = 0;; ++spin) {
        if (*seq == want) {
            __atomic_thread_fence(__ATOMIC_ACQUIRE);
            c->poll_stream = st; c->poll_stream_valid = true;
            return VGGP_OK;
        }
        __builtin_ia32_pause();
        if ((spin & 4095) == 4095) {
            clock_gettime(CLOCK_MONOTONIC, &t1);
            if ((double)(t1.tv_sec - t0.tv_sec) + 1e-9 * (double)(t1.tv_nsec - t0.tv_nsec) > 0.02) break;
        }
    }
    c->poll_stream_valid = false;
    VG_HIP(hipStreamSynchronize(st));
    return VGGP_OK;
}

static int finish_collect(vggp_ctx* c, double* elbo_out, double grad_out[5], vggp_info* info, hipStream_t st) {
    {
        const int wrc = vg_wait_step(c, st);
        if (wrc) {
            c->warm_run = 0;
            for (int k = 0; k < 2; ++k) c->d[k].have_prev = c->d[k].have_prev2 = false;
            c->have_step = false;
            return wrc;
        }
    }
    c->pred_consumed = false;
    c->acc_valid = false;
    if (c->prof && c->nev > 1) {
        for (int i = 1; i < c->nev; ++i) {
            const int id = c->ev_stage[i];
            float ms = 0.f;
            if (id >= 0 && id < VGGP_NSTAGE && hipEventElapsedTime(&ms, c->ev[i - 1], c->ev[i]) == hipSuccess) c->prof_ms[id] += ms;
        }
        c->prof_steps++;
    }
    c->nev = 0;
    if (c->h_out->seq != c->h_theta[5]) {
        vg_set_error("step %.0f: the result block carries sequence number %.0f (stale results)", c->h_theta[5], c->h_out->seq);
        c->warm_run = 0;
        for (int k = 0; k < 2; ++k) c->d[k].have_prev = c->d[k].have_prev2 = false;
        c->have_step = false;
        return VGGP_ESTATE;
    }
    if (c->h_out->out[6] != 0.0) {
        vg_set_error("rank %d / %d: %.0f rank(s) of the job failed their half of this step; the result is discarded", c->rank,
                     c->n_ranks, c->h_out->out[6]);
        c->warm_run = 0;
        for (int k = 0; k < 2; ++k) c->d[k].have_prev = c->d[k].have_prev2 = false;
        c->have_step = false;
        return VGGP_ERCCL;
    }
    *elbo_out = c->h_out->out[0];
    for (int i = 0; i < 5; ++i) grad_out[i] = c->h_out->out[1 + i];
    int status = 0;
    for (int k = 0; k < 2; ++k) {
        if (c->h_out->status[k]) status = c->h_out->status[k];
        else if (c->h_out->counters[k][2]) status = c->h_out->counters[k][2];
    }
    if (info) {
        info->jitter1 = c->h_out->jitter[0]; info->jitter2 = c->h_out->jitter[1];
        info->sweeps1 = c->h_out->counters[0][1] & 0xff; info->sweeps2 = c->h_out->counters[1][1] & 0xff;
        info->rounds1 = c->h_out->counters[0][0]; info->rounds2 = c->h_out->counters[1][0];
        info->status = status;
        info->polished = ((c->h_out->counters[0][3] >> 28) & 1) | (((c->h_out->counters[1][3] >> 28) & 1) << 1);
    }
    {
        static const bool off = getenv("VGGP_NO_SUBSPACE") != nullptr;
        bool ok = !status && !off && c->desc.warm_start && !(c->desc.flags & VGGP_FLAG_BLOCK_JACOBI);
        for (int k = 0; k < 2; ++k) {
            VgDim& d = c->d[k];
            const int rank = (c->h_out->counters[k][1] >> 8) & 0x1ff;
            int want = 0;
            static const bool relax = getenv("VGGP_NO_SUB_RELAX") == nullptr;
            if (d.Zs && rank >= 1 && 3 * rank <= d.m) {
                static const bool m8 = getenv("VGGP_SUB_MARGIN8") != nullptr;
                want = m8 ? ((rank + 4 + 7) / 8) * 8 : ((rank + 3 + 1) / 2) * 2;
                if (want < 16) want = 16;
                if (want > 64 || 2 * want > d.m) want = 0;
            } else if (relax && d.Zs && rank >= 1 && d.m <= 64 && rank + 2 <= d.m - 8) {
                want = ((rank + 2 + 3) / 4) * 4;
                if (want > d.m - 8) want = d.m - 8;
                if (want < 8 || want > 48) want = 0;
            }
            if (d.m > 128 && want > VG_THIN_MAXR) want = 0;
            if (want == 0) d.sub_r = 0;
            else if (want > d.sub_r || want < d.sub_r - 8) d.sub_r = want;
            ok = ok && d.sub_r > 0;
        }
        c->sub_next = ok;
    }
    c->refine_next = !status && ((c->h_out->counters[0][3] >> 28) & 1) && ((c->h_out->counters[1][3] >> 28) & 1) &&
                     (c->h_out->counters[0][1] & 0xff) <= 1 && (c->h_out->counters[1][1] & 0xff) <= 1;
    if (status == VG_ESUBMISS && c->cur_newton) {
        static const bool dbg = getenv("VGGP_NEWTON_DBG") != nullptr;
        if (dbg)
            fprintf(stderr, "[vggp] step %ld: Newton chain (%d iterations) missed: dim1 flags %d, 10 log10(offdiag / thr) = %d; dim2 flags %d, %d\n",
                    c->seq, c->cur_newton, c->h_out->counters[0][3] & 0xff, (c->h_out->counters[0][3] >> 8) - 100,
                    c->h_out->counters[1][3] & 0xff, (c->h_out->counters[1][3] >> 8) - 100);
        c->newton_block = (c->d[0].m > 128 || c->d[1].m > 128) ? 2 : 16; c->newton_next = false;
        if (c->newton_iters < 5) ++c->newton_iters;
        c->newton_ok_run = 0;
        c->have_step = false;
        return VG_ESUBMISS;
    }
    if (status) {
        c->warm_run = 0;
        for (int k = 0; k < 2; ++k) c->d[k].have_prev = c->d[k].have_prev2 = false;
        c->have_step = false;
    }
    if (status == VG_ESUBMISS) {
        c->sub_next = false;
        if (c->cur_thin) c->thin_block = 32;
        return VG_ESUBMISS;
    }
    if (status == VGGP_ENOTPD) { vg_set_error("a Kuu factor is not positive definite after jitter 1e-6"); return VGGP_ENOTPD; }
    if (status == VGGP_ENOCONV) { vg_set_error("Jacobi eigensolver did not converge"); return VGGP_ENOCONV; }
    for (int k = 0; k < 2; ++k) {
        c->d[k].have_prev2 = c->d[k].have_prev;
        c->d[k].have_prev = true;
        c->d[k].thin_rows = c->cur_thin ? c->cur_r[k] : c->d[k].m;
    }
    c->last_thin = c->cur_thin;
    if (c->thin_block > 0) --c->thin_block;
    c->last_newton = c->cur_newton > 0;
    if (c->cur_newton > 0 && ++c->newton_ok_run >= 64) {
        c->newton_ok_run = 0;
        if (c->newton_iters > 3) --c->newton_iters;
    }
    {
        const bool polished = ((c->h_out->counters[0][3] >> 28) & 1) && ((c->h_out->counters[1][3] >> 28) & 1);
        c->newton_next = c->cur_newton > 0 ||
                         (c->last_warm && c->cur_extrap && !c->cur_thin && !polished && (c->h_out->counters[0][0] + c->h_out->counters[1][0]) > 0) ||
                         (c->last_warm && c->cur_extrap && !c->cur_thin && c->d[0].m >= 96 && c->d[1].m >= 96 &&
                          (2 * c->h_out->counters[0][0] >= 3 * c->d[0].m || 2 * c->h_out->counters[1][0] >= 3 * c->d[1].m));
    }
    if (++c->warm_run >= 512) {
        c->warm_run = 0;
        for (int k = 0; k < 2; ++k) c->d[k].have_prev = c->d[k].have_prev2 = false;
    }
    c->have_step = true;
    return VGGP_OK;
}

extern "C" int vggp_elbo_partials(vggp_ctx* c, const double* Y, const double theta[5], double* payload, void* stream) {
    VG_NOT_PAIRED(c, "vggp_elbo_partials");
    if (!c || !c->planned) { vg_set_error("vggp_elbo_partials: context not planned"); return VGGP_ESTATE; }
    VG_REQUIRE(Y && theta && payload, "vggp_elbo_partials: null argument");
    VG_ENTER_DEVICE(c->device);
    hipStream_t st = stream ? (hipStream_t)stream : c->own_stream;
    int rc = set_theta(c, theta);
    if (rc) return rc;
    c->nev = 0;
    const VgGraphKey key{Y, payload, 0.0};
    VgStart sp;
    if ((rc = vg_start_prepare(c, vg_warm(c, false), st, &sp, false))) return rc;
    const bool extrap = sp.extrap;
    const bool apply_ns = extrap && !c->pred_consumed;
    rc = run_graph(c, extrap ? VG_G_PARTIALS_X : VG_G_PARTIALS, key, st,
                   [&] { return vg_partials_enqueue(c, Y, payload, st, true, extrap, false, apply_ns); }, extrap && !apply_ns);
    if (rc) return rc;
    if (extrap) c->pred_consumed = true;
    c->have_partials = true;
    return VGGP_OK;
}

static int elbo_finish_once(vggp_ctx* c, const double* payload, double yy_total, const double theta[5],
                            double* elbo_out, double grad_out[5], vggp_info* info, void* stream);
extern "C" int vggp_elbo_finish(vggp_ctx* c, const double* payload, double yy_total, const double theta[5],
                                double* elbo_out, double grad_out[5], vggp_info* info, void* stream) {
    VG_NOT_PAIRED(c, "vggp_elbo_finish");
    int rc = elbo_finish_once(c, payload, yy_total, theta, elbo_out, grad_out, info, stream);
    if (rc == VG_ESUBMISS) rc = elbo_finish_once(c, payload, yy_total, theta, elbo_out, grad_out, info, stream);
// ... 332 lines not shown
    const long m1 = c->desc.m1, m2 = c->desc.m2;
    const long chunk = std::min<long>(ns, 65536);
    if (ns == 0) return VGGP_OK;
    const size_t per = (size_t)chunk * (2 * m1 + 3 * m2 + 2 * m1) + (size_t)(m1 * m1 + m2 * m2);
    const bool thin_ro = vg_thin_readout(c);
    int rc = thin_ro ? VGGP_OK : vg_accurate_state(c, st);
    if (rc) return rc;
    const int q1 = thin_ro ? c->d[0].thin_rows : (int)m1, q2 = thin_ro ? c->d[1].thin_rows : (int)m2;
    if ((rc = vg_ensure_misc(c, per * sizeof(double)))) return rc;
    double* p = (double*)c->misc;
    double* A1 = p; p += m1 * chunk;
    double* T1 = p; p += m1 * chunk;
    double* A2 = p; p += m2 * chunk;
    double* T2 = p; p += m2 * chunk;
    double* T2sq = p; p += m2 * chunk;
    double* U = p; p += m1 * chunk;
    double* Uv = p; p += m1 * chunk;
    double* W1 = p; p += m1 * m1;
    double* W2 = p;
    VgDim &d1 = c->d[0], &d2 = c->d[1];
    VG_HIP(vg_qv_weights_launch(c->theta, c->beta, c->invD, c->wq, (long)q1 * q2, st));
    {
        VgGemmBatch g;
        vg_gemm_init(&g);
        vg_gemm_add(&g, d1.QtPrev, m1, 1, d1.Linv0, m1, 1, W1, (int)m1, q1, (int)m1, (int)m1);
        vg_gemm_add(&g, d2.QtPrev, m2, 1, d2.Linv0, m2, 1, W2, (int)m2, q2, (int)m2, (int)m2);
        VG_HIP(vg_gemm_launch(&g, st));
    }
    for (long off = 0; off < ns; off += chunk) {
        const int cn = (int)std::min<long>(chunk, ns - off);
        VgFactorJob fj[2] = {
            VgFactorJob{xs1 + off, d1.grid, A1, nullptr, nullptr, nullptr, cn, d1.m, d1.kind, d1.basis, 0, 0.0, c->desc.flags},
            VgFactorJob{xs2 + off, d2.grid, A2, nullptr, nullptr, nullptr, cn, d2.m, d2.kind, d2.basis, 1, 0.0, c->desc.flags}};
        VG_HIP(vg_factor_build_launch(fj, 2, c->theta, st));
        VgGemmBatch g;
        vg_gemm_init(&g);
        vg_gemm_add(&g, W1, m1, 1, A1, cn, 1, T1, cn, q1, cn, (int)m1);
        vg_gemm_add(&g, W2, m2, 1, A2, cn, 1, T2, cn, q2, cn, (int)m2);
        VG_HIP(vg_gemm_launch(&g, st));
        VG_HIP(vg_scale_sq_launch(T2, T2sq, (long)q2 * cn, st));
        vg_gemm_init(&g);
        vg_gemm_add(&g, c->wq, q2, 1, T2, cn, 1, U, cn, q1, cn, q2);
        vg_gemm_add(&g, c->wq + (long)q1 * q2, q2, 1, T2sq, cn, 1, Uv, cn, q1, cn, q2);
        VG_HIP(vg_gemm_launch(&g, st));
        VG_HIP(vg_post_combine_launch(c->theta, T1, U, Uv, nullptr, q1, q2, cn, mean + off, var + off, st));
    }
    return VGGP_OK;
}

__global__ void vg_khatri_rao_kernel(const double* U1, const double* U2, const double* w, int m1, int m2, long ns, double* T,
                                     double* Tw) {
    const long idx = (long)blockIdx.x * blockDim.x + threadIdx.x;
    const long total = (long)m1 * m2 * ns;
    if (idx >= total) return;
    const long u = idx / ns, p = idx - u * ns;
    const int i1 = (int)(u / m2), i2 = (int)(u - (long)i1 * m2);
    const double v = U1[(long)i1 * ns + p] * U2[(long)i2 * ns + p];
    T[idx] = v;
    if (Tw) Tw[idx] = v * w[u];
}
__global__ void vg_prior_cov_kernel(const double* xs1, const double* xs2, long ns, int kind1, int kind2, const double* theta,
                                    double* cov) {
    const long idx = (long)blockIdx.x * blockDim.x + threadIdx.x;
    if (idx >= ns * ns) return;
    const long p = idx / ns, q = idx - p * ns;
    double k1, k2, d;
    vg_kappa(kind1, fabs(xs1[p] - xs1[q]), 1.0 / theta[0], k1, d);
    vg_kappa(kind2, fabs(xs2[p] - xs2[q]), 1.0 / theta[1], k2, d);
    cov[idx] += theta[2] * theta[3] * k1 * k2;
}
hipError_t vg_prior_cov_launch(const double* xs1, const double* xs2, long ns, int kind1, int kind2, const double* theta,
                               double* cov, hipStream_t st) {
    hipLaunchKernelGGL(vg_prior_cov_kernel, dim3((unsigned)((ns * ns + 255) / 256)), dim3(256), 0, st, xs1, xs2, ns, kind1,
                       kind2, theta, cov);
    return hipGetLastError();
}

static int posterior_factors(vggp_ctx* c, const double* xs1, const double* xs2, int ns, double* A1, double* A2, double* U1,
                             double* U2, hipStream_t st, bool rotate) {
    VgDim &d1 = c->d[0], &d2 = c->d[1];
    VgFactorJob fj[2] = {
        VgFactorJob{xs1, d1.grid, A1, nullptr, nullptr, nullptr, ns, d1.m, d1.kind, d1.basis, 0, 0.0, c->desc.flags},
        VgFactorJob{xs2, d2.grid, A2, nullptr, nullptr, nullptr, ns, d2.m, d2.kind, d2.basis, 1, 0.0, c->desc.flags}};
    VG_HIP(vg_factor_build_launch(fj, 2, c->theta, st));
    VgTrsmSpec q[2] = {{d1.L0, d1.m, d1.Linv0, 16L * d1.m + 16, d1.m, A1, ns, 1, ns, d1.m, 0},
                       {d2.L0, d2.m, d2.Linv0, 16L * d2.m + 16, d2.m, A2, ns, 1, ns, d2.m, 0}};
    int rc = trsm_batch(q, 2, st);
    if (rc || !rotate) return rc;
    VgGemmBatch g;
    vg_gemm_init(&g);
    vg_gemm_add(&g, d1.QtPrev, d1.m, 1, A1, ns, 1, U1, ns, d1.m, ns, d1.m);
    vg_gemm_add(&g, d2.QtPrev, d2.m, 1, A2, ns, 1, U2, ns, d2.m, ns, d2.m);
    VG_HIP(vg_gemm_launch(&g, st));
    return VGGP_OK;
}

extern "C" int vggp_posterior_cov(vggp_ctx* c, const double* xs1, const double* xs2, int64_t ns, double* cov, void* stream) {
    VG_NOT_PAIRED(c, "vggp_posterior_cov");
    if (!c || !c->have_step) { vg_set_error("vggp_posterior_cov: no finished ELBO step"); return VGGP_ESTATE; }
    VG_REQUIRE(xs1 && xs2 && cov && ns >= 1, "vggp_posterior_cov: bad argument");
    const long m1 = c->desc.m1, m2 = c->desc.m2, M = m1 * m2;
    VG_REQUIRE(ns <= 8192 && M * ns <= (1L << 27), "vggp_posterior_cov: ns=%ld points x M=%ld is too large for a dense covariance "
               "(use vggp_posterior for mean / variance)", (long)ns, M);
    VG_ENTER_DEVICE(c->device);
    hipStream_t st = stream ? (hipStream_t)stream : c->own_stream;
    const size_t need = (size_t)(2 * (m1 + m2) * ns + 2 * M * ns + M) * sizeof(double);
    int rc = vg_accurate_state(c, st);
    if (rc) return rc;
    if ((rc = vg_ensure_misc(c, need))) return rc;
    double* p = (double*)c->misc;
    double* A1 = p; p += m1 * ns;
    double* A2 = p; p += m2 * ns;
    double* U1 = p; p += m1 * ns;
    double* U2 = p; p += m2 * ns;
    double* T = p; p += M * ns;
    double* Tw = p; p += M * ns;
    if ((rc = posterior_factors(c, xs1, xs2, (int)ns, A1, A2, U1, U2, st, true))) return rc;
    VG_HIP(vg_qv_weights_launch(c->theta, c->beta, c->invD, c->wq, M, st));
    hipLaunchKernelGGL(vg_khatri_rao_kernel, dim3((unsigned)((M * ns + 255) / 256)), dim3(256), 0, st, U1, U2, c->wq + M, (int)m1,
                       (int)m2, (long)ns, T, Tw);
    VG_HIP(hipGetLastError());
    VgGemmBatch g;
    vg_gemm_init(&g);
    vg_gemm_add(&g, Tw, 1, ns, T, ns, 1, cov, (int)ns, (int)ns, (int)ns, (int)M, 1, 0, 1, 0, c->h_theta[2] * c->h_theta[3], 0);
    VG_HIP(vg_gemm_launch(&g, st));
    VG_HIP(vg_prior_cov_launch(xs1, xs2, ns, c->d[0].kind, c->d[1].kind, c->theta, cov, st));
    return VGGP_OK;
}

extern "C" int vggp_readout(vggp_ctx* c, const double* C1, int64_t mv1, const double* C2, int64_t mv2, const double* kd1,
                            const double* kd2, double* mean, double* var, int flags, void* stream) {
    VG_NOT_PAIRED(c, "vggp_readout");
    if (!c || !c->have_step) { vg_set_error("vggp_readout: no finished ELBO step"); return VGGP_ESTATE; }
    VG_REQUIRE(C1 && C2 && kd1 && kd2 && mean && var && mv1 >= 1 && mv2 >= 1, "vggp_readout: bad argument");
    VG_ENTER_DEVICE(c->device);
    hipStream_t st = stream ? (hipStream_t)stream : c->own_stream;
    const long m1 = c->desc.m1, m2 = c->desc.m2;
    const size_t need = (size_t)(3 * (m1 * mv1 + m2 * mv2) + 2 * m1 * mv2) * sizeof(double);
    int rc = vg_accurate_state(c, st);
    if (rc) return rc;
    if ((rc = vg_ensure_misc(c, need))) return rc;
    double* p = (double*)c->misc;
    double* X1 = p; p += m1 * mv1;
    double* T1 = p; p += m1 * mv1;
    double* S1 = p; p += m1 * mv1;
    double* X2 = p; p += m2 * mv2;
    double* T2 = p; p += m2 * mv2;
    double* S2 = p; p += m2 * mv2;
    double* U = p; p += m1 * mv2;
    double* Uv = p;
    VgDim &d1 = c->d[0], &d2 = c->d[1];
    VG_HIP(vg_readout_weights_launch(c->theta, c->beta, c->invD, c->wq, m1 * m2, (flags & VGGP_READOUT_LITERAL) ? 1 : 0, st));
    VgGemmBatch g;
    vg_gemm_init(&g);
    vg_gemm_add(&g, d1.Linv0, m1, 1, C1, 1, m1, X1, (int)mv1, (int)m1, (int)mv1, (int)m1);
    vg_gemm_add(&g, d2.Linv0, m2, 1, C2, 1, m2, X2, (int)mv2, (int)m2, (int)mv2, (int)m2);
    VG_HIP(vg_gemm_launch(&g, st));
    vg_gemm_init(&g);
    vg_gemm_add(&g, d1.QtPrev, m1, 1, X1, mv1, 1, T1, (int)mv1, (int)m1, (int)mv1, (int)m1);
    vg_gemm_add(&g, d2.QtPrev, m2, 1, X2, mv2, 1, T2, (int)mv2, (int)m2, (int)mv2, (int)m2);
    VG_HIP(vg_gemm_launch(&g, st));
    VG_HIP(vg_scale_sq_launch(T1, S1, m1 * mv1, st));
    VG_HIP(vg_scale_sq_launch(T2, S2, m2 * mv2, st));
    vg_gemm_init(&g);
    vg_gemm_add(&g, c->wq, m2, 1, T2, mv2, 1, U, (int)mv2, (int)m1, (int)mv2, (int)m2);
    vg_gemm_add(&g, c->wq + m1 * m2, m2, 1, S2, mv2, 1, Uv, (int)mv2, (int)m1, (int)mv2, (int)m2);
    VG_HIP(vg_gemm_launch(&g, st));
    vg_gemm_init(&g);
    vg_gemm_add(&g, T1, 1, mv1, U, mv2, 1, mean, (int)mv2, (int)mv1, (int)mv2, (int)m1);
    vg_gemm_add(&g, S1, 1, mv1, Uv, mv2, 1, var, (int)mv2, (int)mv1, (int)mv2, (int)m1);
    VG_HIP(vg_gemm_launch(&g, st));
    VG_HIP(vg_readout_var_launch(c->theta, kd1, kd2, mv1, mv2, var, st));
    return VGGP_OK;
}

extern "C" int vggp_factor_build(vggp_ctx* c, int kind, int basis, const double* x, int64_t n, const double* grid,
                                 int64_t m, double ell, int flags, double* A0, double* dA0, double* K0, double* dK0, void* stream) {
    if (!c) { vg_set_error("null context"); return VGGP_EINVAL; }
    VG_REQUIRE(kind >= 0 && kind <= 3 && basis >= 0 && basis <= 4, "vggp_factor_build: bad kind/basis");
    VG_REQUIRE(!((basis == VGGP_BASIS_VFF || basis == VGGP_BASIS_B1) && kind != VGGP_KIND_MATERN12),
               "vggp_factor_build: VFF / B1 are Matern-1/2 only");
    VG_REQUIRE(!(basis == VGGP_BASIS_B0 && kind != VGGP_KIND_MATERN12), "vggp_factor_build: B0 is Matern-1/2 only");
    VG_REQUIRE(n >= 0 && m >= 1 && ell > 0.0, "vggp_factor_build: bad sizes / lengthscale");
    VG_REQUIRE(grid || basis == VGGP_BASIS_ONE, "vggp_factor_build: null grid");
    VG_REQUIRE((x || !(A0 || dA0)), "vggp_factor_build: null x");
    VG_ENTER_DEVICE(c->device);
    VgFactorJob j{x, grid, n > 0 ? A0 : nullptr, n > 0 ? dA0 : nullptr, K0, dK0, (int)n, (int)m, kind, basis, -1, ell, flags};
    VG_HIP(vg_factor_build_launch(&j, 1, nullptr, stream ? (hipStream_t)stream : c->own_stream));
    return VGGP_OK;
}

__global__ void vg_copy_jitter_kernel(const double* K, double* W, long m, double jit) {
    const long idx = (long)blockIdx.x * blockDim.x + threadIdx.x;
    if (idx >= m * m) return;
    W[idx] = K[idx] + ((idx / m == idx % m) ? jit : 0.0);
}

extern "C" int vggp_cholesky_inverse(vggp_ctx* c, const double* K, int64_t m, double* L, double* Linv, double* jitter_out,
                                     void* stream) {
    if (!c) { vg_set_error("null context"); return VGGP_EINVAL; }
    VG_REQUIRE(K && L && Linv && m >= 1 && m <= 8192, "vggp_cholesky_inverse: bad argument (1 <= m <= 8192)");
    VG_ENTER_DEVICE(c->device);
    hipStream_t st = stream ? (hipStream_t)stream : c->own_stream;
    if (m > 128) {
        const size_t nblk = (size_t)(m + VG_DENSE_MB - 1) / VG_DENSE_MB;
        const size_t need = ((size_t)m * m + nblk * VG_DENSE_MB * VG_DENSE_MB + (size_t)VG_DENSE_MB * m + VG_DENSE_MB * (VG_DENSE_MB + 1) + 64) * sizeof(double);
        int rc = vg_ensure_misc(c, need);
        if (rc) return rc;
        double* p = (double*)c->misc;
        VgDenseChol w{};
        w.S = p; p += (size_t)m * m;
        w.DI = p; p += nblk * VG_DENSE_MB * VG_DENSE_MB;
        w.Tmp = p; p += (size_t)VG_DENSE_MB * m;
        w.scratch = p; p += VG_DENSE_MB * (VG_DENSE_MB + 1);
        w.jit = p; p += 8;
        w.status = reinterpret_cast<int*>(p);
        w.L = L; w.X = Linv; w.M = m; w.Sinv = nullptr;
        static const double levels[4] = {0.0, 1e-8, 1e-7, 1e-6};
        for (int lvl = 0; lvl < 4; ++lvl) {
            VG_HIP(hipMemsetAsync(w.status, 0, 2 * sizeof(int), st));
            hipLaunchKernelGGL(vg_copy_jitter_kernel, dim3((unsigned)(((size_t)m * m + 255) / 256)), dim3(256), 0, st, K, w.S, (long)m, levels[lvl]);
            VG_HIP(hipGetLastError());
            if ((rc = vg_blocked_chol_inverse(w, st))) return rc;
            int hs = 0;
            VG_HIP(hipMemcpyAsync(&hs, w.status, sizeof(int), hipMemcpyDeviceToHost, st));
            VG_HIP(hipStreamSynchronize(st));
            if (!hs) { if (jitter_out) *jitter_out = levels[lvl]; return VGGP_OK; }
        }
        if (jitter_out) *jitter_out = -1.0;
        vg_set_error("vggp_cholesky_inverse: not positive definite after jitter 1e-6");
        return VGGP_ENOTPD;
    }
    int rc = vg_ensure_misc(c, (size_t)(m * (m + 1) + 16) * sizeof(double));
    if (rc) return rc;
    double* scratch = (double*)c->misc;
    double* jit = scratch + m * (m + 1);
    int* status = (int*)(jit + 2);
    VgClearArgs clr;
    clr.n = 2;
    clr.ptr[0] = reinterpret_cast<int*>(jit); clr.nwords[0] = 16;
    clr.ptr[1] = reinterpret_cast<int*>(scratch); clr.nwords[1] = 16;
    VG_HIP(vg_clear_launch(&clr, st));
    VgCholJob j{K, L, Linv, scratch, jit, status, (int)m};
    VG_HIP(vg_chol_launch(&j, 1, st));
    double hj = 0.0;
    int hs = 0;
    VG_HIP(hipMemcpyAsync(&hj, jit, sizeof(double), hipMemcpyDeviceToHost, st));
    VG_HIP(hipMemcpyAsync(&hs, status, sizeof(int), hipMemcpyDeviceToHost, st));
    VG_HIP(hipStreamSynchronize(st));
    if (jitter_out) *jitter_out = hj;
    if (hs) { vg_set_error("vggp_cholesky_inverse: not positive definite after jitter 1e-6"); return VGGP_ENOTPD; }
    return VGGP_OK;
}

extern "C" int vggp_eigh(vggp_ctx* c, const double* G, int64_t m, double* lam, double* Qt, int32_t* sweeps_out, int flags,
                         void* stream) {
    if (!c) { vg_set_error("null context"); return VGGP_EINVAL; }
    VG_REQUIRE(G && lam && Qt && m >= 1 && m <= 256, "vggp_eigh: bad argument (1 <= m <= 256)");
    VG_ENTER_DEVICE(c->device);
    hipStream_t st = stream ? (hipStream_t)stream : c->own_stream;
    const long m2e = m + (m & 1);
    const int max_rounds = (int)(VG_EIG_MAXSWEEP * (m2e - 1));
    const size_t logb = (vg_eigh_log_bytes((int)m) + 15) & ~size_t(15);
    const size_t need = (size_t)m2e * (m2e + 1) * 8 + logb + (size_t)max_rounds * 4 + 256 + (size_t)m2e * 4 + 64;
    int rc = vg_ensure_misc(c, need);
    if (rc) return rc;
    char* p = (char*)c->misc;
    double* gwork = (double*)p; p += (size_t)m2e * (m2e + 1) * 8;
    double2* rotlog = (double2*)p; p += logb;
    int* roundlog = (int*)p; p += (size_t)max_rounds * 4;
    p = (char*)(((uintptr_t)p + 63) & ~uintptr_t(63));
    int* counters = (int*)p;
    int* perm = counters + 16;
    VgClearArgs clr;
    clr.n = 1;
    clr.ptr[0] = counters; clr.nwords[0] = 8;
    VG_HIP(vg_clear_launch(&clr, st));
    VgEigJob j{G, lam, Qt, nullptr, gwork, rotlog, roundlog, counters, (int)m, max_rounds, (long)logb,
               (flags & VGGP_FLAG_BLOCK_JACOBI) ? 1 : 0};
    j.perm = perm;
    j.err = counters + 4;
    VG_HIP(vg_eigh_launch(&j, 1, st));
    int hc[8] = {0, 0, 0, 0, 0, 0, 0, 0};
    VG_HIP(hipMemcpyAsync(hc, counters, sizeof(hc), hipMemcpyDeviceToHost, st));
    VG_HIP(hipStreamSynchronize(st));
    if (sweeps_out) *sweeps_out = hc[1] & 0xff;
    if (hc[2] || hc[4]) { vg_set_error("vggp_eigh: no convergence"); return VGGP_ENOCONV; }
    return VGGP_OK;
}

extern "C" int vggp_gemm(vggp_ctx* c, const double* A, int64_t sa_m, int64_t sa_k, const double* B, int64_t sb_k,
                         int64_t sb_n, double* C, int64_t ldc, int64_t M, int64_t N, int64_t K, void* stream) {
    if (!c) { vg_set_error("null context"); return VGGP_EINVAL; }
    VG_REQUIRE(A && B && C && M >= 1 && N >= 1 && K >= 1 && ldc >= N, "vggp_gemm: bad argument");
    VG_REQUIRE(M < (1L << 30) && N < (1L << 30) && K < (1L << 30), "vggp_gemm: dimension too large");
    VG_ENTER_DEVICE(c->device);
    VgGemmBatch g;
    vg_gemm_init(&g);
    vg_gemm_add(&g, A, sa_m, sa_k, B, sb_k, sb_n, C, (int)ldc, (int)M, (int)N, (int)K);
    VG_HIP(vg_gemm_launch(&g, stream ? (hipStream_t)stream : c->own_stream));
    return VGGP_OK;
}

extern "C" int vggp_trsm(vggp_ctx* c, const double* L, int64_t m, const double* R, int64_t ncols, double* X, int trans,
                         void* stream) {
    if (!c) { vg_set_error("null context"); return VGGP_EINVAL; }
    VG_REQUIRE(L && R && X && m >= 1 && m <= 16384 && ncols >= 1, "vggp_trsm: bad argument (1 <= m <= 16384)");
    VG_REQUIRE(m * ncols < (1L << 31) && m * m < (1L << 31), "vggp_trsm: matrix too large");
    VG_ENTER_DEVICE(c->device);
    hipStream_t st = stream ? (hipStream_t)stream : c->own_stream;
    const long nb16 = (m + 15) / 16;
    int rc = vg_ensure_misc(c, (size_t)nb16 * 256 * sizeof(double));
    if (rc) return rc;
    double* Dinv = (double*)c->misc;
    VG_HIP(vg_tri_diaginv_launch(L, m, (int)m, Dinv, st));
    if (X != R) VG_HIP(hipMemcpyAsync(X, R, sizeof(double) * m * ncols, hipMemcpyDeviceToDevice, st));
    return trsm_inplace(L, m, m, Dinv, X, ncols, 1, ncols, trans ? 1 : 0, st);
}

struct VgTriInvSpec { const double* L; long n; const double* Dinv16; double* Xinv; double* tmp; };
static int tri_inverse_batch(const VgTriInvSpec* sp, int nf, hipStream_t st) {
    VgTrsmJob tj[16];
    int nt = 0;
    for (int f = 0; f < nf; ++f)
        for (long r0 = 0; r0 < sp[f].n; r0 += VG_TRSM_BLK) {
            const long rb = std::min<long>(VG_TRSM_BLK, sp[f].n - r0);
            if (nt == 16) { VG_HIP(vg_trsm_launch(tj, nt, st)); nt = 0; }
            VgTrsmJob j{sp[f].L + r0 * sp[f].n + r0, sp[f].Dinv16 + (r0 / 16) * 256, nullptr, sp[f].Xinv + r0 * sp[f].n + r0, sp[f].n, 256, 16,
                        sp[f].n, 1, sp[f].n, 1, rb, (int)rb, 0};
            j.rhs_ident = 1;
            tj[nt++] = j;
        }
    if (nt) VG_HIP(vg_trsm_launch(tj, nt, st));
    long nmax = 0;
    for (int f = 0; f < nf; ++f) nmax = std::max(nmax, sp[f].n);
    for (long b = VG_TRSM_BLK; b < nmax; b *= 2) {
        for (int pass = 0; pass < 2; ++pass) {
            VgGemmBatch g;
            vg_gemm_init(&g);
            for (int f = 0; f < nf; ++f) {
                const long n = sp[f].n;
                for (long a0 = 0; a0 + b < n; a0 += 2 * b) {
                    const long c0 = a0 + b, cb = std::min<long>(b, n - c0);
                    if (g.nprob == VG_GEMM_MAXP) { VG_HIP(vg_gemm_launch(&g, st)); vg_gemm_init(&g); }
                    int ip;
                    if (pass == 0) {
                        ip = vg_gemm_add(&g, sp[f].L + c0 * n + a0, n, 1, sp[f].Xinv + a0 * n + a0, n, 1, sp[f].tmp + c0 * n + a0, (int)n, (int)cb,
                                         (int)b, (int)b);
                        g.p[ip].tri = VG_TRI_B_LOWER;
                    } else {
                        ip = vg_gemm_add(&g, sp[f].Xinv + c0 * n + c0, n, 1, sp[f].tmp + c0 * n + a0, n, 1, sp[f].Xinv + c0 * n + a0, (int)n,
                                         (int)cb, (int)b, (int)cb, 1, 0, 1, 0, -1.0, 0);
                        g.p[ip].tri = VG_TRI_A_LOWER;
                    }
                }
            }
            if (g.nprob) VG_HIP(vg_gemm_launch(&g, st));
        }
    }
    return VGGP_OK;
}

extern "C" int vggp_kron_solve(vggp_ctx* c, const double* L1, int64_t n1, const double* L2, int64_t n2, const double* Y,
                               double* X, void* stream) {
    if (!c) { vg_set_error("null context"); return VGGP_EINVAL; }
    VG_REQUIRE(L1 && L2 && Y && X && n1 >= 1 && n2 >= 1 && n1 <= 16384 && n2 <= 16384, "vggp_kron_solve: bad argument");
    VG_REQUIRE(n1 * n2 < (1L << 31) && n1 * n1 < (1L << 31) && n2 * n2 < (1L << 31), "vggp_kron_solve: matrix too large");
    VG_ENTER_DEVICE(c->device);
    hipStream_t st = stream ? (hipStream_t)stream : c->own_stream;
    const long nb1 = (n1 + 15) / 16, nb2 = (n2 + 15) / 16;
    static const bool subst_only = getenv("VGGP_KRON_SUBST") != nullptr;
    const bool small = (n1 <= VG_TRSM_BLK && n2 <= VG_TRSM_BLK) || subst_only;
    const size_t need = (size_t)(nb1 + nb2) * 256 + (small ? 0 : (size_t)(2 * (n1 * n1 + n2 * n2) + 4 * n1 * n2));
    int rc = vg_ensure_misc(c, need * sizeof(double));
    if (rc) return rc;
    double* D1 = (double*)c->misc;
    double* D2 = D1 + nb1 * 256;
    VG_HIP(vg_tri_diaginv_launch(L1, n1, (int)n1, D1, st, L2, n2, (int)n2, D2));
    if (small) {
        if (X != Y) VG_HIP(hipMemcpyAsync(X, Y, sizeof(double) * n1 * n2, hipMemcpyDeviceToDevice, st));
        if ((rc = trsm_inplace(L1, n1, n1, D1, X, n2, 1, n2, 0, st))) return rc;
        if ((rc = trsm_inplace(L2, n2, n2, D2, X, 1, n2, n1, 0, st))) return rc;
        if ((rc = trsm_inplace(L1, n1, n1, D1, X, n2, 1, n2, 1, st))) return rc;
        if ((rc = trsm_inplace(L2, n2, n2, D2, X, 1, n2, n1, 1, st))) return rc;
        return VGGP_OK;
    }
    double* Li1 = D2 + nb2 * 256;
    double* Li2 = Li1 + n1 * n1;
    double* tmp1 = Li2 + n2 * n2;
    double* tmp2 = tmp1 + n1 * n1;
    double* T1 = tmp2 + n2 * n2;
    double* T2 = T1 + 2 * n1 * n2;
    VgTriInvSpec sp[2] = {{L1, (long)n1, D1, Li1, tmp1}, {L2, (long)n2, D2, Li2, tmp2}};
    if ((rc = tri_inverse_batch(sp, 2, st))) return rc;
    static const bool four = getenv("VGGP_KRON_FOUR") != nullptr;
    VgGemmBatch g;
    if (!four) {
        double* P1 = tmp1;
        double* P2 = tmp2;
        vg_gemm_init(&g);
        { const int i = vg_gemm_add(&g, Li1, 1, n1, Li1, n1, 1, P1, (int)n1, (int)n1, (int)n1, (int)n1); g.p[i].tri = VG_TRI_A_UPPER_B_LOWER; }
        { const int i = vg_gemm_add(&g, Li2, 1, n2, Li2, n2, 1, P2, (int)n2, (int)n2, (int)n2, (int)n2); g.p[i].tri = VG_TRI_A_UPPER_B_LOWER; g.p[i].rev = 1; }
        VG_HIP(vg_gemm_launch(&g, st, VG_GEMM_TAG_WIDE));
        vg_gemm_init(&g);
        vg_gemm_add(&g, P1, n1, 1, Y, n2, 1, T1, (int)n2, (int)n1, (int)n2, (int)n1);
        VG_HIP(vg_gemm_launch(&g, st, VG_GEMM_TAG_WIDE));
        vg_gemm_init(&g);
        vg_gemm_add(&g, T1, n2, 1, P2, n2, 1, X, (int)n2, (int)n1, (int)n2, (int)n2);
        VG_HIP(vg_gemm_launch(&g, st, VG_GEMM_TAG_WIDE));
        return VGGP_OK;
    }
    const long slab = (long)n1 * n2;
    static const char* kse = getenv("VGGP_KRON_KSPLIT");
    const int ks = kse ? atoi(kse) : 1;
    vg_gemm_init(&g);
    { const int i = vg_gemm_add(&g, Li1, n1, 1, Y, n2, 1, T1, (int)n2, (int)n1, (int)n2, (int)n1, ks, slab); g.p[i].tri = VG_TRI_A_LOWER; }
    const int s1 = g.p[0].ksplit;
    VG_HIP(vg_gemm_launch(&g, st, VG_GEMM_TAG_WIDE));
    vg_gemm_init(&g);
    { const int i = vg_gemm_add(&g, T1, n2, 1, Li2, 1, n2, T2, (int)n2, (int)n1, (int)n2, (int)n2, ks, slab); g.p[i].tri = VG_TRI_B_UPPER;
      g.p[i].a_nslab = s1; g.p[i].a_slab = slab; }
    const int s2 = g.p[0].ksplit;
    VG_HIP(vg_gemm_launch(&g, st, VG_GEMM_TAG_WIDE));
    vg_gemm_init(&g);
    { const int i = vg_gemm_add(&g, Li1, 1, n1, T2, n2, 1, T1, (int)n2, (int)n1, (int)n2, (int)n1, ks, slab, s2, slab); g.p[i].tri = VG_TRI_A_UPPER; }
    const int s3 = g.p[0].ksplit;
    VG_HIP(vg_gemm_launch(&g, st, VG_GEMM_TAG_WIDE));
    vg_gemm_init(&g);
    { const int i = vg_gemm_add(&g, T1, n2, 1, Li2, n2, 1, X, (int)n2, (int)n1, (int)n2, (int)n2); g.p[i].tri = VG_TRI_B_LOWER;
      g.p[i].a_nslab = s3; g.p[i].a_slab = slab; }
    VG_HIP(vg_gemm_launch(&g, st, VG_GEMM_TAG_WIDE));
    return VGGP_OK;
}

int vg_trsm_batch(const VgTrsmSpec* sp, int n, hipStream_t st) { return trsm_batch(sp, n, st); }

extern "C" int vggp_zgrad(vggp_ctx* c, const double* Y, double* gz1, double* gz2, void* stream) {
    if (c && c->is_paired) {
        if (!c->planned) { vg_set_error("context not planned"); return VGGP_ESTATE; }
        VG_ENTER_DEVICE(c->device);
        return vg_paired_zgrad(c, Y, gz1, gz2, stream ? (hipStream_t)stream : c->own_stream, false);
    }
    if (!c || !c->have_step) { vg_set_error("vggp_zgrad: no finished ELBO step"); return VGGP_ESTATE; }
    VG_REQUIRE(Y && gz1 && gz2, "vggp_zgrad: null argument");
    const bool multi = c->n_ranks > 1 || c->comm || c->cb;
    const bool lead = !multi || c->rank == 0;
    VG_ENTER_DEVICE(c->device);
    hipStream_t st = stream ? (hipStream_t)stream : c->own_stream;
    if (c->last_thin) {
        c->thin_off = true;
        const int rca = vg_accurate_state(c, st);
        if (rca) return rca;
    }
    const long n1 = c->desc.n1, n2 = c->desc.n2, m1 = c->desc.m1, m2 = c->desc.m2;
    VgDim &d1 = c->d[0], &d2 = c->d[1];
    const bool pts[2] = {d1.basis == VGGP_BASIS_POINTS, d2.basis == VGGP_BASIS_POINTS};
    if (!pts[0]) VG_HIP(hipMemsetAsync(gz1, 0, sizeof(double) * m1, st));
    if (!pts[1]) VG_HIP(hipMemsetAsync(gz2, 0, sizeof(double) * m2, st));
    if (!pts[0] && !pts[1]) return VGGP_OK;
    const double s1 = c->h_theta[2], s2 = c->h_theta[3], v = c->h_theta[4];
    const long mm1 = m1 * m1, mm2 = m2 * m2, m12 = m1 * m2;
    const size_t need = sizeof(double) * (size_t)(6 * mm1 + 6 * mm2 + 2 * m12 + m1 * n1 + m2 * n2 + m1 * n2 + m1 + m2);
    int rc = vg_ensure_misc(c, need);
    if (rc) return rc;
    double* w = reinterpret_cast<double*>(c->misc);
    double *Xa[2], *Xl[2], *WE[2], *WF[2], *TA[2], *TB[2];
    for (int k = 0; k < 2; ++k) {
        const long mm = k ? mm2 : mm1;
        Xa[k] = w; w += mm; Xl[k] = w; w += mm; WE[k] = w; w += mm; WF[k] = w; w += mm; TA[k] = w; w += mm; TB[k] = w; w += mm;
    }
    double* U = w; w += m12;
    double* T1 = w; w += m12;
    double* WV[2] = {w, w + m1 * n1}; w += m1 * n1 + m2 * n2;
    double* R1 = w; w += m1 * n2;
    double* gzbuf = w;
    VgGemmBatch g;
    vg_gemm_init(&g);
    vg_gemm_add(&g, c->beta, m2, 1, c->beta, 1, m2, Xa[0], (int)m1, (int)m1, (int)m1, (int)m2);
    vg_gemm_add(&g, c->bl2, m2, 1, c->beta, 1, m2, Xl[0], (int)m1, (int)m1, (int)m1, (int)m2);
    vg_gemm_add(&g, c->beta, 1, m2, c->beta, m2, 1, Xa[1], (int)m2, (int)m2, (int)m2, (int)m1);
    vg_gemm_add(&g, c->bl1, 1, m2, c->beta, m2, 1, Xl[1], (int)m2, (int)m2, (int)m2, (int)m1);
    if (pts[1]) vg_gemm_add(&g, d1.BV, n1, 1, Y, 1, n1, R1, (int)n2, (int)m1, (int)n2, (int)n1);
    VG_HIP(vg_gemm_launch(&g, st));
    VG_HIP(vg_zw_launch(c->theta, 0, d1.lam0, d2.lam0, (int)m1, (int)m2, Xa[0], Xl[0], c->r1, c->r1l, WE[0], WF[0], st));
    VG_HIP(vg_zw_launch(c->theta, 1, d2.lam0, d1.lam0, (int)m2, (int)m1, Xa[1], Xl[1], c->r2, c->r2l, WE[1], WF[1], st));
    vg_gemm_init(&g);
    for (int k = 0; k < 2; ++k) {
        VgDim& d = c->d[k];
        vg_gemm_add(&g, WE[k], d.m, 1, d.Qt, d.m, 1, TA[k], d.m, d.m, d.m, d.m);
        vg_gemm_add(&g, WF[k], d.m, 1, d.Qt, d.m, 1, TB[k], d.m, d.m, d.m, d.m);
    }
    vg_gemm_add(&g, c->beta, m2, 1, d2.Qt, m2, 1, U, (int)m2, (int)m1, (int)m2, (int)m2, 1, 0, 1, 0, 1.0 / (v * v));
    VG_HIP(vg_gemm_launch(&g, st));
    vg_gemm_init(&g);
    for (int k = 0; k < 2; ++k) {
        VgDim& d = c->d[k];
        vg_gemm_add(&g, d.Qt, 1, d.m, TA[k], d.m, 1, WE[k], d.m, d.m, d.m, d.m, 1, 0, 1, 0, lead ? 1.0 : 0.0);
        vg_gemm_add(&g, d.Qt, 1, d.m, TB[k], d.m, 1, WF[k], d.m, d.m, d.m, d.m);
    }
    vg_gemm_add(&g, d1.Qt, 1, m1, U, m2, 1, T1, (int)m2, (int)m1, (int)m2, (int)m1);
    VG_HIP(vg_gemm_launch(&g, st));
    vg_gemm_init(&g);
    for (int k = 0; k < 2; ++k) {
        VgDim& d = c->d[k];
        if (!pts[k]) continue;
        vg_gemm_add(&g, WF[k], d.m, 1, d.BV, d.n, 1, WV[k], d.n, d.m, d.n, d.m, 1, 0, 1, 0, k ? s2 : (lead ? s1 : 0.0));
    }
    VG_HIP(vg_gemm_launch(&g, st));
    vg_gemm_init(&g);
    const double rs = std::sqrt(s1 * s2);
    if (pts[0]) {
        const int ip = vg_gemm_add(&g, T1, m2, 1, c->St, n1, 1, WV[0], (int)n1, (int)m1, (int)n1, (int)m2, 1, 0, c->st_slabs, 2L * m2 * n1, rs, 1);
        (void)ip;
    }
    if (pts[1]) {
        vg_gemm_add(&g, T1, 1, m2, R1, n2, 1, WV[1], (int)n2, (int)m2, (int)n2, (int)m1, 1, 0, 1, 0, rs, 1);
    }
    VG_HIP(vg_gemm_launch(&g, st));
    for (int pass = 0; pass < 2; ++pass) {
        VgTrsmSpec q[4];
        int nq = 0;
        for (int k = 0; k < 2; ++k) {
            VgDim& d = c->d[k];
            if (!pts[k]) continue;
            const bool dv = d.m <= VG_TRSM_BLK && d.Dinv0 && c->dinv_valid;
            const double* dp = dv ? d.Dinv0 : d.Linv0;
            const long blk = dv ? 256 : 16L * d.m + 16, dld = dv ? 16 : d.m;
            if (pass == 0) {
                q[nq++] = VgTrsmSpec{d.L0, d.m, dp, blk, dld, WV[k], d.n, 1, d.n, d.m, 1};
                q[nq++] = VgTrsmSpec{d.L0, d.m, dp, blk, dld, WE[k], d.m, 1, d.m, d.m, 1};
            } else {
                q[nq++] = VgTrsmSpec{d.L0, d.m, dp, blk, dld, WE[k], 1, d.m, d.m, d.m, 1};
            }
        }
        if ((rc = trsm_batch(q, nq, st))) return rc;
    }
    double *o1 = multi ? gzbuf : gz1, *o2 = multi ? gzbuf + m1 : gz2;
    if (multi) VG_HIP(hipMemsetAsync(gzbuf, 0, sizeof(double) * (m1 + m2), st));
    if (pts[0]) VG_HIP(vg_zdot_launch(c->theta, 0, d1.grid, d1.x, (int)m1, n1, WV[0], d1.AD + m1 * n1, WE[0], d1.dK0, o1, st));
    if (pts[1]) VG_HIP(vg_zdot_launch(c->theta, 1, d2.grid, d2.x, (int)m2, n2, WV[1], d2.AD + m2 * n2, WE[1], d2.dK0, o2, st));
    if (multi) {
        if ((rc = vg_allreduce(c, gzbuf, m1 + m2, st))) return rc;
        VG_HIP(hipMemcpyAsync(gz1, gzbuf, sizeof(double) * m1, hipMemcpyDeviceToDevice, st));
        VG_HIP(hipMemcpyAsync(gz2, gzbuf + m1, sizeof(double) * m2, hipMemcpyDeviceToDevice, st));
    }
    { const int wrc_ = vg_comm_wait(c, st); if (wrc_) return wrc_; }
    return VGGP_OK;
}

#if defined(VGGP_DIAG) || defined(VG_EIG_RT) || defined(VG_CHOL_STAMP)
extern "C" int vggp_debug_read_out(vggp_ctx* c, double* host8) {
    if (!c || !c->out) return VGGP_EINVAL;
    VG_HIP(hipMemcpy(host8, c->out, 8 * sizeof(double), hipMemcpyDeviceToHost));
    return VGGP_OK;
}

extern "C" int vggp_debug_read_gwork(vggp_ctx* c, int dim, int which, void* host, int64_t offset_doubles, int64_t bytes) {
    if (!c || !c->planned || dim < 0 || dim > 1) return VGGP_EINVAL;
    if (which == 6) { VG_HIP(hipMemcpy(host, c->tAC + offset_doubles, bytes, hipMemcpyDeviceToHost)); return VGGP_OK; }
    const double* src = which == 5 ? reinterpret_cast<const double*>(c->d[dim].counters2) : which == 2 ? c->d[dim].Gw : which == 3 ? c->d[dim].Hs : which == 4 ? c->d[dim].lam0 : which ? c->d[dim].gwork2 : c->d[dim].gwork;
    if (!src) return VGGP_EINVAL;
    VG_HIP(hipMemcpy(host, src + offset_doubles, bytes, hipMemcpyDeviceToHost));
    return VGGP_OK;
}

extern "C" int vggp_debug_read_misc(vggp_ctx* c, void* host, int64_t bytes) {
    if (!c || !c->misc || (size_t)bytes > c->misc_bytes) return VGGP_EINVAL;
    VG_HIP(hipMemcpy(host, c->misc, bytes, hipMemcpyDeviceToHost));
    return VGGP_OK;
}
#endif

extern "C" const char* vggp_project_kernel_name(void) { return vg_last_project_kernel(); }

extern "C" int vggp_profile(vggp_ctx* c, int enable) {
    if (!c) { vg_set_error("null context"); return VGGP_EINVAL; }
    VG_ENTER_DEVICE(c->device);
    if (enable && !c->ev[0])
        for (int i = 0; i < VG_MAXEV; ++i) VG_HIP(hipEventCreate(&c->ev[i]));
    c->prof = enable != 0;
    return VGGP_OK;
}

extern "C" int vggp_profile_read(vggp_ctx* c, double ms_out[VGGP_NSTAGE], int32_t* steps_out, int reset) {
    if (!c || !ms_out) { vg_set_error("null argument"); return VGGP_EINVAL; }
    for (int i = 0; i < VGGP_NSTAGE; ++i) ms_out[i] = c->prof_ms[i];
    if (steps_out) *steps_out = c->prof_steps;
    if (reset) { for (int i = 0; i < VGGP_NSTAGE; ++i) c->prof_ms[i] = 0.0; c->prof_steps = 0; }
    return VGGP_OK;
}

extern "C" int vggp_sumsq(vggp_ctx* c, const double* y, int64_t n, double* out, void* stream) {
    if (!c) { vg_set_error("null context"); return VGGP_EINVAL; }
    VG_REQUIRE(y && out && n >= 0, "vggp_sumsq: bad argument");
    VG_ENTER_DEVICE(c->device);
    hipStream_t st = stream ? (hipStream_t)stream : c->own_stream;
    VG_HIP(vg_sumsq_launch(y, n, c->sumsq_partial, c->sumsq_out, st));
    const int rca = vg_allreduce(c, c->sumsq_out, 1, st);
    if (rca) return rca;
    VG_HIP(hipMemcpyAsync(out, c->sumsq_out, sizeof(double), hipMemcpyDeviceToHost, st));
    { const int wrc_ = vg_comm_wait(c, st); if (wrc_) return wrc_; }
    return VGGP_OK;
}
```

variational_gridded_gaussian_processes_amd/csrc/common.h:

```cpp
#pragma once
#if defined(__HIP_DEVICE_COMPILE__) && !defined(__gfx950__)
#error "libvggp_hip is written for gfx950 (MI355X) only: kernels rely on its wave64 barrier semantics, MFMA shapes and LDS size"
#endif
#include <hip/hip_runtime.h>
#include <stdint.h>
#include "../../include/vggp.h"

#define VG_WAVE 64

void vg_set_error(const char* fmt, ...);
#define VG_HIP(call)                                                              \
    do {                                                                          \
        hipError_t _e = (call);                                                   \
        if (_e != hipSuccess) {                                                   \
            vg_set_error("%s:%d: %s -> %s", __FILE__, __LINE__, #call,            \
                         hipGetErrorString(_e));                                  \
            return VGGP_EHIP;                                                     \
        }                                                                         \
    } while (0)
#define VG_REQUIRE(cond, ...)                                                     \
    do {                                                                          \
        if (!(cond)) {                                                            \
            vg_set_error(__VA_ARGS__);                                            \
            return VGGP_EINVAL;                                                   \
        }                                                                         \
    } while (0)

struct VgDeviceGuard {
    int prev = -1;
    bool switched = false;
    hipError_t enter(int dev) {
        hipError_t e = hipGetDevice(&prev);
        if (e != hipSuccess) return e;
        if (prev != dev) { e = hipSetDevice(dev); switched = (e == hipSuccess); }
        return e;
    }
    ~VgDeviceGuard() { if (switched) (void)hipSetDevice(prev); }
};
#define VG_ENTER_DEVICE(dev) VgDeviceGuard vg_dev_guard_; VG_HIP(vg_dev_guard_.enter(dev))

#define VG_GEMM_MAXP 12
#define VG_BM 64
#define VG_BN 64
#define VG_BK 16

struct VgGemmP {
    const double* A;
    const double* B;
    double* C;
    long sa_m, sa_k, sb_k, sb_n;
    long c_slab;
    long b_slab;
    long a_slab;
    int a_nslab;
    int M, N, K;
    int ldc;
    int ksplit;
    int b_nslab;
    int tiles_m, tiles_n;
    int tile_start;
    int kchunk;
    double alpha;
    int accum;
    int xcd_group;
    int tri;
    const double* dotw;
    double* dot_out;
    int dotw_ld;
    int deep;
    int rev;
};
#define VG_TRI_NONE 0
#define VG_TRI_A_LOWER 1
#define VG_TRI_A_UPPER 2
#define VG_TRI_B_UPPER 3
#define VG_TRI_B_LOWER 4
#define VG_TRI_A_UPPER_B_LOWER 5
struct VgGemmBatch {
    int nprob;
    int total_tiles;
    VgGemmP p[VG_GEMM_MAXP];
};

void vg_gemm_init(VgGemmBatch* b);
int vg_gemm_add(VgGemmBatch* b, const double* A, long sa_m, long sa_k, const double* B, long sb_k,
                long sb_n, double* C, int ldc, int M, int N, int K, int ksplit = 1, long c_slab = 0,
                int b_nslab = 1, long b_slab = 0, double alpha = 1.0, int accum = 0);
#define VG_GEMM_TAG_GRAM_PROJECT 1
#define VG_GEMM_TAG_WIDE 2
void vg_gemm_xcd_group(VgGemmBatch* b, int prob);
hipError_t vg_gemm_launch(const VgGemmBatch* b, hipStream_t st, int tag = 0);
const char* vg_last_project_kernel();

#define VG_RED_MAXSEG 8
struct VgRedSeg { const double* in; double* out; long n; long slab; int nslab; int block_start; };
struct VgRedBatch { int nseg; int total_blocks; VgRedSeg s[VG_RED_MAXSEG]; };
void vg_red_init(VgRedBatch* b);
void vg_red_add(VgRedBatch* b, const double* in, double* out, long n, long slab, int nslab);
hipError_t vg_red_launch(const VgRedBatch* b, hipStream_t st);

struct VgFactorJob {
    const double* x;
    const double* grid;
    double* A0;
    double* dA0;
    double* K0;
    double* dK0;
    int n, m, kind, basis;
    int theta_idx;
    double ell_imm;
    int flags;
};
struct VgClearArgs;
hipError_t vg_factor_build_launch(const VgFactorJob* jobs, int njobs, const double* theta_dev, hipStream_t st,
                                  double* theta_copy = nullptr, const VgClearArgs* clr = nullptr);

struct VgCholJob {
    const double* K;
    double* L;
    double* Linv;
    double* scratch;
    double* jitter_out;
    int* status;
    int m;
    int ldk = 0, ldl = 0;
    int only_level0 = 0;
    double* Dinv_out = nullptr;
};
struct VgGemmBatch;
hipError_t vg_chol_launch(const VgCholJob* jobs, int njobs, hipStream_t st, const VgGemmBatch* rider = nullptr);
hipError_t vg_chol_setup();
hipError_t vg_jitcopy_launch(const double* K, int m, double* Kc, hipStream_t st);
hipError_t vg_cholsel_launch(const double* Lc, const double* Dc, const int* st8, int m, double* L0, double* Dinv0, double* jitter_out,
                             int* status, hipStream_t st);

struct VgTrsmJob {
    const double* L;
    const double* Dinv;
    const double* R;
    double* X;
    long ldl, dinv_blk, dinv_ld;
    long r_sk, r_sc, x_sk, x_sc;
    long ncols;
    int m;
    int trans;
    int rhs_ident = 0;
};
hipError_t vg_trsm_launch(const VgTrsmJob* jobs, int njobs, hipStream_t st);
hipError_t vg_trsm_setup();
hipError_t vg_tri_diaginv_launch(const double* L, long ldl, int m, double* out , hipStream_t st,
                                 const double* L2 = nullptr, long ldl2 = 0, int m2 = 0, double* out2 = nullptr);

#define VG_EIG_MAXSWEEP 60
struct VgEigJob {
    const double* G;
    double* lam;
    double* Qt;
    const double* Qt0;
    double* gwork;
    double2* rotlog;
    int* roundlog;
    int* counters;
    int m;
    int max_rounds;
    long log_bytes;
    int block;
    double tol = 0.0;
    double* Qt2 = nullptr;
    const double* cp_src = nullptr;
    double* cp_dst = nullptr;
    int* perm = nullptr;
    int fast_switch = 112;
    int polish = 1;
    int* err = nullptr;
    int polish0 = 0;
    const double* Hl = nullptr;
    const double* Hr = nullptr;
    int hk = 0;
    int null_from = 0;
    int newton = 0;
    int sparse_first = 0;
};
#define VG_EIG_RANK_CUT 1e-14
struct VgRowQrJob { const double* Z; double* V1; int r; int m; const double* cp_src; double* cp_dst; long cp_n; };
struct VgGemmBatch;
hipError_t vg_rowqr_launch(const VgRowQrJob* jobs, int njobs, hipStream_t st, const VgGemmBatch* rider = nullptr);
hipError_t vg_identity_launch(double* A, int m, hipStream_t st);
struct VgRefineJob { const double* Gw; double* E; double* R1; int m; double tol;
                     double emax = 0.0;
                     int* flag = nullptr;
                     double noise = 0.0;
                     const double* lam_prev = nullptr;
                     double null_cut = 0.0;
};
struct VgNewtonCheckJob { const double* Gw; double* lam; int* counters; int* err; const int* flag; int m; int iters; double tol; double noise;
                          double null_cut = 0.0;
};
hipError_t vg_newton_check_launch(const VgNewtonCheckJob* jobs, int njobs, hipStream_t st);
hipError_t vg_copy_if_launch(const int* const* err, const double* const* src_a, double* const* dst_a, const double* const* src_b,
                             double* const* dst_b, const long* n, int njobs, hipStream_t st);
hipError_t vg_refine_launch(const VgRefineJob* jobs, int njobs, hipStream_t st, const VgGemmBatch* rider = nullptr);
size_t vg_eigh_log_bytes(int m);
hipError_t vg_eigh_launch(const VgEigJob* jobs, int njobs, hipStream_t st, const VgGemmBatch* rider = nullptr);
hipError_t vg_eigh_setup();

#define VG_ESUBMISS (-100)
struct VgHostOut {
    double out[8];
    double jitter[2];
    int counters[2][4];
    int status[2];
    double seq;
};
struct VgMspace {
    const double* theta;
    const double* lam1;
    const double* lam2;
    const double* P3;
    const double* E1;
    const double* F1;
    const double* E2;
    const double* F2;
    double* beta;
    double* bl2;
    double* bl1;
    double* invD;
    double* rowpart;
    double* r1;
    double* r1l;
    double* ol;
    const double* dotp;
    double* r2;
    double* r2l;
    double* dotpart;
    double* out;
    int m1, m2;
    double n_total;
    double yy;
    int* ticket = nullptr;
    VgHostOut* hout = nullptr;
    const double* peer_fail = nullptr;
    const double* jit[2] = {nullptr, nullptr};
    const int* status[2] = {nullptr, nullptr};
    const int* counters[2] = {nullptr, nullptr};
};
hipError_t vg_dstage_launch(const VgMspace* ms, hipStream_t st);
#define VG_THIN_MAXR 32
#define VG_THIN_ELBO_TOL 1e-10
#define VG_THIN_MISS 1e-12
struct VgThinTail {
    const double* theta;
    double n_total, yy;
    int r1, r2, m1, m2;
    const double *W1, *W2;
    const double *lam1, *lam2;
    const double *AM1, *AH1, *AM2, *AH2;
    const double* AC;
    int ac_nslab; long ac_slab;
    const double *G1, *H1, *G2, *H2;
    double* out;
    double *beta_out, *invd_out;
    VgHostOut* hout;
    const double* peer_fail;
    const double* jit[2];
    const int* status[2];
    const int* rcounters[2];
    unsigned long long* stamps = nullptr;
};
hipError_t vg_thin_tail_launch(const VgThinTail* tt, hipStream_t st);
struct VgPivCholJob { const double* G; const double* Omega; double* V; int m; int r; };
struct VgPivCholArgs { VgPivCholJob job[2]; };
hipError_t vg_pivchol_launch(const VgPivCholJob* jobs, int njobs, hipStream_t st);
hipError_t vg_thin_tail_setup();
hipError_t vg_final_launch(const VgMspace* ms, hipStream_t st);
hipError_t vg_zw_launch(const double* theta, int self, const double* lam_self, const double* lam_other, int m, int m_other,
                        const double* X, const double* Xl, const double* r, const double* rl, double* WE, double* WFs, hipStream_t st);
hipError_t vg_zdot_launch(const double* theta, int self, const double* z, const double* x, int m, long n, const double* Abar,
                          const double* dA0, const double* Kbar, const double* dK0, double* out, hipStream_t st);

#define VG_CLEAR_MAX 12
struct VgClearArgs { int* ptr[VG_CLEAR_MAX]; int nwords[VG_CLEAR_MAX]; int n; };
hipError_t vg_clear_launch(const VgClearArgs* a, hipStream_t st);

hipError_t vg_readout_weights_launch(const double* theta, const double* beta, const double* invD, double* w, long n, int literal,
                                     hipStream_t st);
hipError_t vg_readout_var_launch(const double* theta, const double* kd1, const double* kd2, long mv1, long mv2, double* var, hipStream_t st);
hipError_t vg_scale_sq_launch(const double* in, double* out_sq, long n, hipStream_t st);
hipError_t vg_qv_weights_launch(const double* theta, const double* beta, const double* invD, double* w_mean,
                                long n, hipStream_t st, int e1 = 1, int e2 = 1);
hipError_t vg_sumsq_launch(const double* y, long n, double* partial, double* out, hipStream_t st);
hipError_t vg_post_combine_launch(const double* theta, const double* T1, const double* T2, const double* beta,
                                  const double* invD, int m1, int m2, long ns, double* mean, double* var,
                                  hipStream_t st);
hipError_t vg_scale_launch(double* x, long n, const double* theta, int mode, hipStream_t st, int e1 = 1, int e2 = 1);
```

variational_gridded_gaussian_processes_amd/engine.py:

```python
from __future__ import annotations

import ctypes as C
from typing import Optional, Sequence, Tuple

import numpy as np
import torch

from . import _lib
from ._lib import BASIS, KIND, Desc, Info, check


def _ptr(t: Optional[torch.Tensor]) -> Optional[int]:
    if t is None:
        return None
    if not (t.is_cuda and t.dtype == torch.float64 and t.is_contiguous()):
        raise TypeError("engine tensors must be contiguous float64 on the GPU")
    return t.data_ptr()


def _stream(device=None) -> int:
    return torch.cuda.current_stream(device).cuda_stream


def _dvec(x) -> np.ndarray:
# ... 22 lines not shown
        self.device = torch.device("cuda", self.device_index)
        self.n_ranks, self.rank = int(n_ranks), int(rank)
        if unique_id is not None and len(unique_id) != _lib.UNIQUE_ID_BYTES:
            raise ValueError(f"unique_id must be {_lib.UNIQUE_ID_BYTES} bytes")
        h = C.c_void_p()
        uid = C.create_string_buffer(bytes(unique_id), _lib.UNIQUE_ID_BYTES) if unique_id is not None else None
        check(self.lib.vggp_create(C.byref(h), self.device_index, self.n_ranks, self.rank, C.cast(uid, C.c_void_p) if uid else None))
        self._h = h
        self._cb = None
        if allreduce is not None:
            def _trampoline(_user, buf, count, fn=allreduce):
                try:
                    fn(np.ctypeslib.as_array(buf, shape=(int(count),)))
                    return 0
                except Exception:
                    import traceback
                    traceback.print_exc()
                    return 1
            self._cb = _lib.ALLREDUCE_FN(_trampoline)
            check(self.lib.vggp_set_allreduce(self._h, self._cb, None))
        self.m1 = self.m2 = self.n1 = self.n2 = 0
        self.planned = False
        self._step_bufs = None
        self.paired = False
        self.plan_token = 0

    @staticmethod
    def unique_id() -> bytes:
        buf = C.create_string_buffer(_lib.UNIQUE_ID_BYTES)
        check(_lib.load().vggp_unique_id(C.cast(buf, C.c_void_p)))
        return buf.raw

    @property
    def transport(self) -> str:
        t = C.c_int()
        check(self.lib.vggp_comm_info(self._h, None, None, C.byref(t)))
        return {0: "none", 1: "rccl", 2: "callback"}[t.value]

    def comm_info(self) -> dict:
        n, r, t = C.c_int(), C.c_int(), C.c_int()
        check(self.lib.vggp_comm_info(self._h, C.byref(n), C.byref(r), C.byref(t)))
        return {"n_ranks": n.value, "rank": r.value, "transport": {0: "none", 1: "rccl", 2: "callback"}[t.value]}

    def allreduce(self, t: torch.Tensor) -> torch.Tensor:
        check(self.lib.vggp_allreduce(self._h, _ptr(t), t.numel(), _stream(self.device)))
        return t

    def close(self):
        if getattr(self, "_h", None):
            self.lib.vggp_destroy(self._h)
            self._h = None

    def __del__(self):
        try:
            self.close()
        except Exception:
            pass

    def plan(self, kind1: str, basis1: str, grid1, x1, kind2: str, basis2: str, grid2, x2,
             n_total: Optional[int] = None, warm_start: bool = False, b0_f32_kdelta: bool = False,
             block_jacobi: bool = False, scattered: bool = False) -> None:
        x1, x2 = _dvec(x1), _dvec(x2)
        g1 = _dvec(grid1) if basis1 != "one" else np.ones(1)
        g2 = _dvec(grid2) if basis2 != "one" else np.ones(1)
        m1, m2 = _basis_m(basis1, g1), _basis_m(basis2, g2)
        d = Desc()
        d.kind1, d.basis1, d.kind2, d.basis2 = KIND[kind1], BASIS[basis1], KIND[kind2], BASIS[basis2]
        d.n1, d.n2, d.m1, d.m2 = len(x1), len(x2), m1, m2
        d.n_total = int(n_total) if n_total is not None else len(x1) * len(x2)
        d.x1, d.x2 = x1.ctypes.data, x2.ctypes.data
        d.grid1, d.grid2 = g1.ctypes.data, g2.ctypes.data
        d.warm_start = 1 if warm_start else 0
        d.flags = (_lib.FLAG_B0_F32_KDELTA if b0_f32_kdelta else 0) | (_lib.FLAG_BLOCK_JACOBI if block_jacobi else 0) | \
                  (_lib.FLAG_SCATTERED if scattered else 0)
        if scattered:
            if len(x1) != len(x2):
                raise ValueError("scattered plan: x1 and x2 must hold one coordinate pair per point")
            d.n_total = int(n_total) if n_total is not None else len(x1)
        self.scattered = bool(scattered)
        with torch.cuda.device(self.device):
            check(self.lib.vggp_plan(self._h, C.byref(d)))
        self.paired = False
        self.m1, self.m2, self.n1, self.n2 = m1, m2, len(x1), len(x2)
        self.payload_len = int(self.lib.vggp_payload_len(self._h))
        self.planned = True
        self.plan_token += 1

    def plan_paired(self, kind: str, Z, x1, x2, scattered: bool = False) -> None:
        Zn = np.ascontiguousarray(np.asarray(Z, dtype=np.float64).reshape(-1, 2))
        z1, z2 = np.ascontiguousarray(Zn[:, 0]), np.ascontiguousarray(Zn[:, 1])
        x1, x2 = _dvec(x1), _dvec(x2)
        if scattered and len(x1) != len(x2):
            raise ValueError("scattered plan: x1 and x2 must hold one coordinate pair per point")
        M = Zn.shape[0]
        d = Desc()
        d.kind1 = d.kind2 = KIND[kind]
        d.basis1 = d.basis2 = BASIS["points"]
        d.n1, d.n2, d.m1, d.m2 = len(x1), len(x2), M, M
        d.n_total = len(x1) if scattered else len(x1) * len(x2)
        d.x1, d.x2, d.grid1, d.grid2 = x1.ctypes.data, x2.ctypes.data, z1.ctypes.data, z2.ctypes.data
        d.warm_start = 0
        d.flags = _lib.FLAG_PAIRED_Z | (_lib.FLAG_SCATTERED if scattered else 0)
        with torch.cuda.device(self.device):
            check(self.lib.vggp_plan(self._h, C.byref(d)))
        self.scattered = bool(scattered)
        self.paired = True
        self.m1, self.m2, self.n1, self.n2 = M, M, len(x1), len(x2)
        self.payload_len = 0
        self.planned = True
        self.plan_token += 1

    @property
    def workspace_bytes(self) -> int:
        return int(self.lib.vggp_workspace_bytes(self._h))

    def _check_Y(self, Y: torch.Tensor):
        if tuple(Y.shape) != (self.n2, self.n1):
            raise ValueError(f"Y must be [n2={self.n2}, n1={self.n1}] (x1 fastest), got {tuple(Y.shape)}")

    def elbo_step(self, Y: torch.Tensor, yy_total: float, theta: Sequence[float]):
        self._check_Y(Y)
        b = self._step_bufs
        if b is None:
            th, elbo, grad, info = (C.c_double * 5)(), C.c_double(), (C.c_double * 5)(), Info()
            b = self._step_bufs = (th, elbo, grad, info, C.byref(elbo), C.byref(info), np.frombuffer(grad, dtype=np.float64))
        th = b[0]
        th[0], th[1], th[2], th[3], th[4] = theta
        check(self.lib.vggp_elbo_step(self._h, _ptr(Y), float(yy_total), th, b[4], b[2], b[5], _stream(self.device)))
        return b[1].value, b[6].copy(), self._info(b[3])

    def elbo_step_masked(self, Ym: torch.Tensor, W: torch.Tensor, n_obs: float, yy_obs: float, theta: Sequence[float]):
        self._check_Y(Ym)
        self._check_Y(W)
        th = (C.c_double * 5)(*[float(t) for t in theta])
        elbo = C.c_double()
        grad = (C.c_double * 5)()
        info = Info()
        check(self.lib.vggp_elbo_step_masked(self._h, _ptr(Ym), _ptr(W), float(n_obs), float(yy_obs), th, C.byref(elbo),
                                             grad, C.byref(info), _stream(self.device)))
        return elbo.value, np.array(list(grad)), self._info(info)

    def elbo_step_masked_iter(self, Ym: torch.Tensor, W: torch.Tensor, n_obs: float, yy_obs: float, theta: Sequence[float],
                              n_probes: int = 16, tol: float = 1e-10, max_iter: int = 100):
        self._check_Y(Ym)
        self._check_Y(W)
        th = (C.c_double * 5)(*[float(t) for t in theta])
        elbo = C.c_double()
        grad = (C.c_double * 5)()
        info = Info()
        check(self.lib.vggp_elbo_step_masked_iter(self._h, _ptr(Ym), _ptr(W), float(n_obs), float(yy_obs), th, int(n_probes), float(tol),
                                                  int(max_iter), C.byref(elbo), grad, C.byref(info), _stream(self.device)))
        return elbo.value, np.array(list(grad)), self._info(info)

    def elbo_step_scattered(self, y: torch.Tensor, yy: float, theta: Sequence[float]):
        if not (y.is_cuda and y.dtype == torch.float64 and y.is_contiguous() and y.numel() == self.n1):
            raise TypeError("y must be a contiguous float64 GPU tensor with one value per planned point")
        th = (C.c_double * 5)(*[float(t) for t in theta])
        elbo = C.c_double()
        grad = (C.c_double * 5)()
        info = Info()
        check(self.lib.vggp_elbo_step_scattered(self._h, _ptr(y), float(yy), th, C.byref(elbo), grad, C.byref(info),
                                                _stream(self.device)))
        return elbo.value, np.array(list(grad)), self._info(info)

    def qv_masked(self) -> Tuple[torch.Tensor, torch.Tensor]:
        shape = (self.m1,) if self.paired else (self.m1, self.m2)
        mean = torch.empty(*shape, dtype=torch.float64, device=self.device)
        var = torch.empty_like(mean)
        check(self.lib.vggp_qv_masked(self._h, _ptr(mean), _ptr(var), _stream(self.device)))
        return mean, var

    def elbo_partials(self, Y: torch.Tensor, theta: Sequence[float], payload: Optional[torch.Tensor] = None):
        self._check_Y(Y)
        if payload is None:
            payload = torch.empty(self.payload_len, dtype=torch.float64, device=self.device)
        th = (C.c_double * 5)(*[float(t) for t in theta])
        check(self.lib.vggp_elbo_partials(self._h, _ptr(Y), th, _ptr(payload), _stream(self.device)))
        return payload

    def elbo_finish(self, payload: torch.Tensor, yy_total: float, theta: Sequence[float]):
        th = (C.c_double * 5)(*[float(t) for t in theta])
        elbo = C.c_double()
        grad = (C.c_double * 5)()
        info = Info()
        check(self.lib.vggp_elbo_finish(self._h, _ptr(payload), float(yy_total), th, C.byref(elbo), grad,
                                        C.byref(info), _stream(self.device)))
        return elbo.value, np.array(list(grad)), self._info(info)

    @staticmethod
    def _info(i: Info) -> dict:
        return dict(jitter=(i.jitter1, i.jitter2), sweeps=(i.sweeps1, i.sweeps2), rounds=(i.rounds1, i.rounds2),
                    status=i.status, polished=(bool(i.polished & 1), bool(i.polished & 2)))

    def qv(self) -> Tuple[torch.Tensor, torch.Tensor]:
        mean = torch.empty(self.m1, self.m2, dtype=torch.float64, device=self.device)
        var = torch.empty_like(mean)
        check(self.lib.vggp_qv(self._h, _ptr(mean), _ptr(var), _stream(self.device)))
        return mean, var

    def qv_cov(self) -> torch.Tensor:
        M = self.m1 * self.m2
        cov = torch.empty(M, M, dtype=torch.float64, device=self.device)
        check(self.lib.vggp_qv_cov(self._h, _ptr(cov), _stream(self.device)))
        return cov

    def readout(self, C1: torch.Tensor, C2: torch.Tensor, kd1: torch.Tensor, kd2: torch.Tensor, literal: bool = True,
                masked: bool = False):
        C1, C2 = C1.to(self.device, torch.float64).contiguous(), C2.to(self.device, torch.float64).contiguous()
        kd1, kd2 = kd1.to(self.device, torch.float64).contiguous(), kd2.to(self.device, torch.float64).contiguous()
        if C1.shape[1] != self.m1 or C2.shape[1] != self.m2:
            raise ValueError("C_d must be [mv_d, m_d]")
        mean = torch.empty(C1.shape[0], C2.shape[0], dtype=torch.float64, device=self.device)
        var = torch.empty_like(mean)
        fn = self.lib.vggp_readout_masked if masked else self.lib.vggp_readout
        check(fn(self._h, _ptr(C1), C1.shape[0], _ptr(C2), C2.shape[0], _ptr(kd1), _ptr(kd2), _ptr(mean),
                 _ptr(var), 1 if literal else 0, _stream(self.device)))
        return mean, var

    def posterior_cov(self, x_star: torch.Tensor, masked: bool = False) -> torch.Tensor:
        xs = x_star.to(self.device, torch.float64)
        if xs.dim() == 1:
            xs = torch.stack([xs, torch.zeros_like(xs)], dim=1)
        xs1, xs2 = xs[:, 0].contiguous(), xs[:, 1].contiguous()
        ns = xs1.shape[0]
        cov = torch.empty(ns, ns, dtype=torch.float64, device=self.device)
        fn = self.lib.vggp_posterior_cov_masked if masked else self.lib.vggp_posterior_cov
        check(fn(self._h, _ptr(xs1), _ptr(xs2), ns, _ptr(cov), _stream(self.device)))
        return cov

    def set_inducing(self, dim: int, z) -> None:
        zz = _dvec(z)
        with torch.cuda.device(self.device):
            check(self.lib.vggp_set_inducing(self._h, int(dim), zz.ctypes.data, len(zz)))

    def zgrad(self, Y: torch.Tensor):
        g1 = torch.empty(self.m1, dtype=torch.float64, device=self.device)
        g2 = torch.empty(self.m2, dtype=torch.float64, device=self.device)
        check(self.lib.vggp_zgrad(self._h, _ptr(Y), _ptr(g1), _ptr(g2), _stream(self.device)))
        return g1, g2

    def zgrad_scattered(self, y: torch.Tensor):
        g1 = torch.empty(self.m1, dtype=torch.float64, device=self.device)
        g2 = torch.empty(self.m2, dtype=torch.float64, device=self.device)
        check(self.lib.vggp_zgrad_scattered(self._h, _ptr(y), _ptr(g1), _ptr(g2), _stream(self.device)))
        return g1, g2

    def qv_cov_masked(self) -> torch.Tensor:
        M = self.m1 if self.paired else self.m1 * self.m2
        cov = torch.empty(M, M, dtype=torch.float64, device=self.device)
        check(self.lib.vggp_qv_cov_masked(self._h, _ptr(cov), _stream(self.device)))
        return cov

    def posterior_masked(self, x_star: torch.Tensor) -> Tuple[torch.Tensor, torch.Tensor]:
        return self.posterior(x_star, _fn="vggp_posterior_masked")

    def posterior(self, x_star: torch.Tensor, _fn: str = "vggp_posterior") -> Tuple[torch.Tensor, torch.Tensor]:
        xs = x_star.to(self.device, torch.float64)
        if xs.dim() == 1:
            xs = torch.stack([xs, torch.zeros_like(xs)], dim=1)
        xs1, xs2 = xs[:, 0].contiguous(), xs[:, 1].contiguous()
        ns = xs1.shape[0]
        mean = torch.empty(ns, dtype=torch.float64, device=self.device)
        var = torch.empty_like(mean)
        check(getattr(self.lib, _fn)(self._h, _ptr(xs1), _ptr(xs2), ns, _ptr(mean), _ptr(var), _stream(self.device)))
        return mean, var

    def factor_build(self, kind: str, basis: str, x: torch.Tensor, grid: torch.Tensor, ell: float, flags: int = 0):
        n = x.shape[0]
        m = _basis_m(basis, np.empty(grid.shape[0]))
        o = dict(dtype=torch.float64, device=self.device)
        A, dA, K, dK = torch.empty(m, n, **o), torch.empty(m, n, **o), torch.empty(m, m, **o), torch.empty(m, m, **o)
        check(self.lib.vggp_factor_build(self._h, KIND[kind], BASIS[basis], _ptr(x), n, _ptr(grid), m, float(ell), int(flags),
                                         _ptr(A), _ptr(dA), _ptr(K), _ptr(dK), _stream(self.device)))
        return A, dA, K, dK

    def cholesky_inverse(self, K: torch.Tensor):
        m = K.shape[0]
        L, Li = torch.empty_like(K), torch.empty_like(K)
        jit = C.c_double()
        check(self.lib.vggp_cholesky_inverse(self._h, _ptr(K), m, _ptr(L), _ptr(Li), C.byref(jit), _stream(self.device)))
        return L, Li, jit.value

    def eigh(self, G: torch.Tensor, block: bool = False):
        m = G.shape[0]
        lam = torch.empty(m, dtype=torch.float64, device=self.device)
        Qt = torch.empty_like(G)
        sw = C.c_int32()
        check(self.lib.vggp_eigh(self._h, _ptr(G), m, _ptr(lam), _ptr(Qt), C.byref(sw),
                                 _lib.FLAG_BLOCK_JACOBI if block else 0, _stream(self.device)))
        return lam, Qt, sw.value

    def gemm(self, A: torch.Tensor, B: torch.Tensor) -> torch.Tensor:
        M, K = A.shape
        K2, N = B.shape
        assert K == K2
        Cm = torch.empty(M, N, dtype=torch.float64, device=self.device)
        for t in (A, B):
            if not (t.is_cuda and t.dtype == torch.float64):
                raise TypeError("gemm operands must be float64 GPU tensors")
        check(self.lib.vggp_gemm(self._h, A.data_ptr(), A.stride(0), A.stride(1), B.data_ptr(), B.stride(0),
                                 B.stride(1), Cm.data_ptr(), N, M, N, K, _stream(self.device)))
        return Cm

    def kron_solve(self, L1: torch.Tensor, L2: torch.Tensor, Y: torch.Tensor) -> torch.Tensor:
        n1, n2 = Y.shape
        X = torch.empty_like(Y)
        check(self.lib.vggp_kron_solve(self._h, _ptr(L1), n1, _ptr(L2), n2, _ptr(Y), _ptr(X), _stream(self.device)))
        return X

    def trsm(self, L: torch.Tensor, R: torch.Tensor, trans: bool = False) -> torch.Tensor:
        m, ncols = R.shape
        X = torch.empty_like(R)
        check(self.lib.vggp_trsm(self._h, _ptr(L), m, _ptr(R), ncols, _ptr(X), 1 if trans else 0, _stream(self.device)))
        return X

    def profile(self, enable: bool = True) -> None:
        check(self.lib.vggp_profile(self._h, 1 if enable else 0))

    def profile_read(self, reset: bool = True):
        ms = (C.c_double * _lib.NSTAGE)()
        steps = C.c_int32()
        check(self.lib.vggp_profile_read(self._h, ms, C.byref(steps), 1 if reset else 0))
        names = [self.lib.vggp_stage_name(i).decode() for i in range(_lib.NSTAGE)]
        return dict(zip(names, list(ms))), steps.value

    def project_kernel_name(self) -> str:
        return self.lib.vggp_project_kernel_name().decode()

    def sumsq(self, y: torch.Tensor) -> float:
        out = C.c_double()
        check(self.lib.vggp_sumsq(self._h, _ptr(y), y.numel(), C.byref(out), _stream(self.device)))
        return out.value
```

Baseline: 5.465 billion grid-points/s.

## Add small-batch panel GEMM kernel and reduce-only slab sums for eigensolver chain

Adds a new panel GEMM kernel that holds whole K-panels in LDS and uses f64 MFMA. It is chosen for batches with fewer than 128 tiles and K up to 256, which covers the small m=128 matrix chain in the warm-start eigensolver. Slab reductions that used to be identity GEMMs (Id × sum of slabs) now run as a reduce-only form that skips the matmul. The aim is to cut launch latency and wasted FLOPs in this latency-bound chain of small GEMMs. In exchange it adds a second GEMM code path with fallback rules, an env switch to disable it, and a new public slab-GEMM API.

```diff
diff --git a/include/vggp.h b/include/vggp.h
--- a/include/vggp.h
+++ b/include/vggp.h
@@ -130,6 +130,10 @@
               const double* B, int64_t sb_k, int64_t sb_n,
               double* C, int64_t ldc, int64_t M, int64_t N, int64_t K, void* stream);
 
+int vggp_gemm_slabs(vggp_ctx* ctx, const double* A, int64_t sa_m, int64_t sa_k, int a_nslab, int64_t a_slab,
+                    const double* B, int64_t sb_k, int64_t sb_n, int b_nslab, int64_t b_slab,
+                    double* C, int64_t ldc, int64_t M, int64_t N, int64_t K, double alpha, int accum, int path, void* stream);
+
 int vggp_trsm(vggp_ctx* ctx, const double* L, int64_t m, const double* R, int64_t ncols, double* X, int trans, void* stream);
 
 int vggp_kron_solve(vggp_ctx* ctx, const double* L1, int64_t n1, const double* L2, int64_t n2,
diff --git a/variational_gridded_gaussian_processes_amd/_lib.py b/variational_gridded_gaussian_processes_amd/_lib.py
--- a/variational_gridded_gaussian_processes_amd/_lib.py
+++ b/variational_gridded_gaussian_processes_amd/_lib.py
@@ -75,6 +75,7 @@
     "vggp_cholesky_inverse": (_I, [_P, _P, _I64, _P, _P, C.POINTER(_D), _P]),
     "vggp_eigh": (_I, [_P, _P, _I64, _P, _P, C.POINTER(C.c_int32), _I, _P]),
     "vggp_gemm": (_I, [_P, _P, _I64, _I64, _P, _I64, _I64, _P, _I64, _I64, _I64, _I64, _P]),
+    "vggp_gemm_slabs": (_I, [_P, _P, _I64, _I64, _I, _I64, _P, _I64, _I64, _I, _I64, _P, _I64, _I64, _I64, _I64, _D, _I, _I, _P]),
     "vggp_kron_solve": (_I, [_P, _P, _I64, _P, _I64, _P, _P, _P]),
     "vggp_trsm": (_I, [_P, _P, _I64, _P, _I64, _P, _I, _P]),
     "vggp_sumsq": (_I, [_P, _P, _I64, C.POINTER(_D), _P]),
diff --git a/variational_gridded_gaussian_processes_amd/build.py b/variational_gridded_gaussian_processes_amd/build.py
--- a/variational_gridded_gaussian_processes_amd/build.py
+++ b/variational_gridded_gaussian_processes_amd/build.py
@@ -7,7 +7,7 @@
 
 HERE = os.path.dirname(os.path.abspath(__file__))
 CSRC = os.path.join(HERE, "csrc")
-SOURCES = ["api.hip", "gemm.hip", "factor_build.hip", "chol.hip", "trsm.hip", "eigh.hip", "mspace.hip", "thin.hip", "masked.hip", "comm.hip", "paired.hip"]
+SOURCES = ["api.hip", "gemm.hip", "gemm_panel.hip", "factor_build.hip", "chol.hip", "trsm.hip", "eigh.hip", "mspace.hip", "thin.hip", "masked.hip", "comm.hip", "paired.hip"]
 HEADERS = ["common.h", "ctx.h", "factor_elem.h", "gemm_body.h", os.path.join("..", "..", "include", "vggp.h")]
 LIB = os.path.join(HERE, "libvggp_hip.so")
 
diff --git a/variational_gridded_gaussian_processes_amd/csrc/api.hip b/variational_gridded_gaussian_processes_amd/csrc/api.hip
--- a/variational_gridded_gaussian_processes_amd/csrc/api.hip
+++ b/variational_gridded_gaussian_processes_amd/csrc/api.hip
@@ -78,6 +78,7 @@
     VG_HIP(vg_chol_setup());
     VG_HIP(vg_eigh_setup());
     VG_HIP(vg_trsm_setup());
+    VG_HIP(vg_gemm_panel_setup());
     VG_HIP(vg_thin_tail_setup());
     vggp_ctx* c = new (std::nothrow) vggp_ctx();
     if (!c) { vg_set_error("out of host memory"); return VGGP_ENOMEM; }
@@ -722,6 +723,16 @@
     const double* Hr[2] = {H0[0], H0[1]};
     int hrn[2] = {ghn[0], ghn[1]};
     VgEigJob ej[2];
+    int red[4], nred = 0;
+    auto add_reduced = [&](VgDim& d, const double* src, double* dst, int nsl, long slab) {
+        red[nred++] = vg_gemm_add(&g, d.Id, d.m, 1, src, d.m, 1, dst, d.m, d.m, d.m, d.m, 1, 0, nsl, slab);
+    };
+    auto launch_reducing = [&]() -> hipError_t {
+        if (vg_gemm_panel_ok(&g))
+            for (int i = 0; i < nred; ++i) g.p[red[i]].A = nullptr;
+        nred = 0;
+        return vg_gemm_chain_launch(&g, st);
+    };
     if (warm && subspace && thin) {
         const bool early = thin_early && !ride;
         const double* Gr[2] = {G0[0], G0[1]};
@@ -732,11 +743,11 @@
             VgDim& d = c->d[k];
             vg_gemm_add(&g, d.QtPrev, d.m, 1, G0[k], d.m, 1, d.TM, d.m, d.sub_r, d.m, d.m, 1, 0, ghn[k], ghs[k]);
             if (from_slabs && ghn[k] > 1) {
-                vg_gemm_add(&g, d.Id, d.m, 1, G0[k], d.m, 1, gdst[k], d.m, d.m, d.m, d.m, 1, 0, ghn[k], ghs[k]);
-                vg_gemm_add(&g, d.Id, d.m, 1, H0[k], d.m, 1, gdst[k] + (long)d.m * d.m, d.m, d.m, d.m, d.m, 1, 0, ghn[k], ghs[k]);
+                add_reduced(d, G0[k], gdst[k], ghn[k], ghs[k]);
+                add_reduced(d, H0[k], gdst[k] + (long)d.m * d.m, ghn[k], ghs[k]);
             }
         }
-        VG_HIP(vg_gemm_launch(&g, st));
+        VG_HIP(launch_reducing());
         VG_MARK(8);
         for (int k = 0; k < 2; ++k)
             if (from_slabs && ghn[k] > 1) { Gr[k] = gdst[k]; grn[k] = 1; Hr[k] = gdst[k] + (long)c->d[k].m * c->d[k].m; hrn[k] = 1; }
@@ -757,7 +768,7 @@
             const int ic = vg_gemm_add(&g, C3, m2, 1, d2.V1s, 1, m2, c->tCV, d2.sub_r, (int)(3 * m1), d2.sub_r, (int)m2);
             g.p[ic].a_nslab = ccn; g.p[ic].a_slab = ccs;
         }
-        VG_HIP(vg_gemm_launch(&g, st));
+        VG_HIP(vg_gemm_chain_launch(&g, st));
         VG_MARK(10);
         VgGemmBatch gx;
         vg_gemm_init(&gx);
@@ -798,13 +809,13 @@
                 VgDim& d = c->d[k];
                 vg_gemm_add(&g, d.Ws, d.sub_r, 1, d.V1s, d.m, 1, d.QtPrev, d.m, d.sub_r, d.m, d.sub_r);
             }
-            VG_HIP(vg_gemm_launch(&g, st));
+            VG_HIP(vg_gemm_chain_launch(&g, st));
             VG_MARK(14);
             vg_gemm_init(&g);
             for (int q = 0; q < 3; ++q)
                 vg_gemm_add(&g, d1.V1s, m1, 1, c->tCV + (long)q * m1 * d2.sub_r, d2.sub_r, 1, c->tAC + (long)q * d1.sub_r * d2.sub_r, d2.sub_r,
                             d1.sub_r, d2.sub_r, (int)m1);
-            VG_HIP(vg_gemm_launch(&g, st));
+            VG_HIP(vg_gemm_chain_launch(&g, st));
             VG_MARK(15);
         }
         VgThinTail tt{};
@@ -829,7 +840,7 @@
                 VgDim& d = c->d[k];
                 vg_gemm_add(&g, d.Ws, d.sub_r, 1, d.V1s, d.m, 1, d.QtPrev, d.m, d.sub_r, d.m, d.sub_r);
             }
-            VG_HIP(vg_gemm_launch(&g, st));
+            VG_HIP(vg_gemm_chain_launch(&g, st));
         }
         return VGGP_OK;
     }
@@ -843,11 +854,11 @@
             VgDim& d = c->d[k];
             vg_gemm_add(&g, d.Fp, d.m, 1, G0[k], d.m, 1, d.TM, d.m, d.m, d.m, d.m, 1, 0, ghn[k], ghs[k]);
             if (from_slabs && ghn[k] > 1) {
-                vg_gemm_add(&g, d.Id, d.m, 1, G0[k], d.m, 1, gdst[k], d.m, d.m, d.m, d.m, 1, 0, ghn[k], ghs[k]);
-                vg_gemm_add(&g, d.Id, d.m, 1, H0[k], d.m, 1, gdst[k] + (long)d.m * d.m, d.m, d.m, d.m, d.m, 1, 0, ghn[k], ghs[k]);
+                add_reduced(d, G0[k], gdst[k], ghn[k], ghs[k]);
+                add_reduced(d, H0[k], gdst[k] + (long)d.m * d.m, ghn[k], ghs[k]);
             }
         }
-        VG_HIP(vg_gemm_launch(&g, st));
+        VG_HIP(launch_reducing());
         VG_MARK(8);
         for (int k = 0; k < 2; ++k)
             if (from_slabs && ghn[k] > 1) { Gr[k] = gdst[k]; grn[k] = 1; Hr[k] = gdst[k] + (long)c->d[k].m * c->d[k].m; hrn[k] = 1; }
@@ -866,7 +877,7 @@
             vg_gemm_add(&g, d.V1s, d.m, 1, Gr[k], d.m, 1, d.Zs, d.m, (int)r, d.m, d.m, 1, 0, grn[k], ghs[k]);
             vg_gemm_add(&g, d.Fp + r * d.m, d.m, 1, d.V1s, 1, d.m, d.TH, (int)r, (int)(d.m - r), (int)r, d.m);
         }
-        VG_HIP(vg_gemm_launch(&g, st));
+        VG_HIP(vg_gemm_chain_launch(&g, st));
         VG_MARK(10);
         VgGemmBatch gx;
         vg_gemm_init(&gx);
@@ -897,13 +908,13 @@
             vg_gemm_add(&g, d.Ws, r, 1, d.V1s, d.m, 1, d.E, d.m, (int)r, d.m, (int)r);
             vg_gemm_add(&g, d.Ws, r, 1, d.Zs, d.m, 1, d.TM, d.m, (int)r, d.m, (int)r);
         }
-        VG_HIP(vg_gemm_launch(&g, st));
+        VG_HIP(vg_gemm_chain_launch(&g, st));
         vg_gemm_init(&g);
         for (int k = 0; k < 2; ++k) {
             VgDim& d = c->d[k];
             vg_gemm_add(&g, d.TM, d.m, 1, d.E, 1, d.m, d.Gw, d.m, d.m, d.m, d.m);
         }
-        VG_HIP(vg_gemm_launch(&g, st));
+        VG_HIP(vg_gemm_chain_launch(&g, st));
     } else if (warm && newton > 0) {
         const double* Gr[2] = {G0[0], G0[1]};
         int grn[2] = {ghn[0], ghn[1]};
@@ -914,17 +925,17 @@
             VgDim& d = c->d[k];
             vg_gemm_add(&g, Scur[k], d.m, 1, G0[k], d.m, 1, d.TM, d.m, d.m, d.m, d.m, 1, 0, ghn[k], ghs[k]);
             if (from_slabs && ghn[k] > 1) {
-                vg_gemm_add(&g, d.Id, d.m, 1, G0[k], d.m, 1, gdst[k], d.m, d.m, d.m, d.m, 1, 0, ghn[k], ghs[k]);
-                vg_gemm_add(&g, d.Id, d.m, 1, H0[k], d.m, 1, gdst[k] + (long)d.m * d.m, d.m, d.m, d.m, d.m, 1, 0, ghn[k], ghs[k]);
+                add_reduced(d, G0[k], gdst[k], ghn[k], ghs[k]);
+                add_reduced(d, H0[k], gdst[k] + (long)d.m * d.m, ghn[k], ghs[k]);
             }
         }
-        VG_HIP(vg_gemm_launch(&g, st));
+        VG_HIP(launch_reducing());
         VG_MARK(8);
         for (int k = 0; k < 2; ++k)
             if (from_slabs && ghn[k] > 1) { Gr[k] = gdst[k]; grn[k] = 1; Hr[k] = gdst[k] + (long)c->d[k].m * c->d[k].m; hrn[k] = 1; }
         vg_gemm_init(&g);
         for (int k = 0; k < 2; ++k) { VgDim& d = c->d[k]; vg_gemm_add(&g, d.TM, d.m, 1, Scur[k], 1, d.m, d.Gw, d.m, d.m, d.m, d.m); }
-        VG_HIP(vg_gemm_launch(&g, st));
+        VG_HIP(vg_gemm_chain_launch(&g, st));
         VG_MARK(12);
         static const bool newton_null = getenv("VGGP_NO_NULL_SKIP") == nullptr;
         int bi = 0;
@@ -942,7 +953,7 @@
             VG_MARK(9);
             vg_gemm_init(&g);
             for (int k = 0; k < 2; ++k) { VgDim& d = c->d[k]; vg_gemm_add(&g, d.U, d.m, 1, d.U, d.m, 1, d.TH, d.m, d.m, d.m, d.m, 1, 0, 1, 0, 0.5, 1); }
-            VG_HIP(vg_gemm_launch(&g, st));
+            VG_HIP(vg_gemm_chain_launch(&g, st));
             double* Snew[2];
             vg_gemm_init(&g);
             for (int k = 0; k < 2; ++k) {
@@ -951,7 +962,7 @@
                 Snew[k] = bufs[bi];
                 vg_gemm_add(&g, d.TH, d.m, 1, Scur[k], d.m, 1, Snew[k], d.m, d.m, d.m, d.m);
             }
-            VG_HIP(vg_gemm_launch(&g, st));
+            VG_HIP(vg_gemm_chain_launch(&g, st));
             bi = (bi + 1) % 3;
             if (it + 1 < newton) {
                 double* Sns[2];
@@ -963,10 +974,10 @@
                     vg_gemm_add(&g, Snew[k], d.m, 1, Snew[k], 1, d.m, d.TM, d.m, d.m, d.m, d.m);
                     vg_gemm_add(&g, d.Id, d.m, 1, Snew[k], d.m, 1, Sns[k], d.m, d.m, d.m, d.m, 1, 0, 1, 0, 1.5, 0);
                 }
-                VG_HIP(vg_gemm_launch(&g, st));
+                VG_HIP(vg_gemm_chain_launch(&g, st));
                 vg_gemm_init(&g);
                 for (int k = 0; k < 2; ++k) { VgDim& d = c->d[k]; vg_gemm_add(&g, d.TM, d.m, 1, Snew[k], d.m, 1, Sns[k], d.m, d.m, d.m, d.m, 1, 0, 1, 0, -0.5, 1); }
-                VG_HIP(vg_gemm_launch(&g, st));
+                VG_HIP(vg_gemm_chain_launch(&g, st));
                 bi = (bi + 1) % 3;
                 for (int k = 0; k < 2; ++k) Scur[k] = Sns[k];
             } else {
@@ -974,10 +985,10 @@
             }
             vg_gemm_init(&g);
             for (int k = 0; k < 2; ++k) { VgDim& d = c->d[k]; vg_gemm_add(&g, Scur[k], d.m, 1, Gr[k], d.m, 1, d.TM, d.m, d.m, d.m, d.m, 1, 0, grn[k], ghs[k]); }
-            VG_HIP(vg_gemm_launch(&g, st));
+            VG_HIP(vg_gemm_chain_launch(&g, st));
             vg_gemm_init(&g);
             for (int k = 0; k < 2; ++k) { VgDim& d = c->d[k]; vg_gemm_add(&g, d.TM, d.m, 1, Scur[k], 1, d.m, d.Gw, d.m, d.m, d.m, d.m); }
-            VG_HIP(vg_gemm_launch(&g, st));
+            VG_HIP(vg_gemm_chain_launch(&g, st));
         }
         VgNewtonCheckJob nj[2];
         for (int k = 0; k < 2; ++k) {
@@ -1011,21 +1022,21 @@
             vg_gemm_add(&g, extrap ? d.Fp : d.QtPrev, d.m, 1, G0[k], d.m, 1, d.TM, d.m, d.m, d.m, d.m, 1, 0, ghn[k], ghs[k]);
             if (from_slabs && ghn[k] > 1) {
                 if (refine) {
-                    vg_gemm_add(&g, d.Id, d.m, 1, G0[k], d.m, 1, gdst[k], d.m, d.m, d.m, d.m, 1, 0, ghn[k], ghs[k]);
+                    add_reduced(d, G0[k], gdst[k], ghn[k], ghs[k]);
                     Gr[k] = gdst[k]; grn[k] = 1;
                 }
-                vg_gemm_add(&g, d.Id, d.m, 1, H0[k], d.m, 1, gdst[k] + (long)d.m * d.m, d.m, d.m, d.m, d.m, 1, 0, ghn[k], ghs[k]);
+                add_reduced(d, H0[k], gdst[k] + (long)d.m * d.m, ghn[k], ghs[k]);
                 Hr[k] = gdst[k] + (long)d.m * d.m; hrn[k] = 1;
             }
         }
-        VG_HIP(vg_gemm_launch(&g, st));
+        VG_HIP(launch_reducing());
         VG_MARK(8);
         vg_gemm_init(&g);
         for (int k = 0; k < 2; ++k) {
             VgDim& d = c->d[k];
             vg_gemm_add(&g, d.TM, d.m, 1, extrap ? d.Fp : d.QtPrev, 1, d.m, d.Gw, d.m, d.m, d.m, d.m);
         }
-        VG_HIP(vg_gemm_launch(&g, st));
+        VG_HIP(vg_gemm_chain_launch(&g, st));
         VG_MARK(12);
         if (refine) {
             VgRefineJob rj[2];
@@ -1048,26 +1059,26 @@
                 vg_gemm_add(&g, d.TH, d.m, 1, S0, d.m, 1, d.E, d.m, d.m, d.m, d.m);
                 vg_gemm_add(&g, d.U, d.m, 1, d.U, d.m, 1, d.X, d.m, d.m, d.m, d.m);
             }
-            VG_HIP(vg_gemm_launch(&g, st));
+            VG_HIP(vg_gemm_chain_launch(&g, st));
             vg_gemm_init(&g);
             for (int k = 0; k < 2; ++k) {
                 VgDim& d = c->d[k];
                 const double* S0 = extrap ? d.Fp : d.QtPrev;
                 vg_gemm_add(&g, d.X, d.m, 1, S0, d.m, 1, d.E, d.m, d.m, d.m, d.m, 1, 0, 1, 0, 0.5, 1);
             }
-            VG_HIP(vg_gemm_launch(&g, st));
+            VG_HIP(vg_gemm_chain_launch(&g, st));
             vg_gemm_init(&g);
             for (int k = 0; k < 2; ++k) {
                 VgDim& d = c->d[k];
                 vg_gemm_add(&g, d.E, d.m, 1, Gr[k], d.m, 1, d.TM, d.m, d.m, d.m, d.m, 1, 0, grn[k], ghs[k]);
             }
-            VG_HIP(vg_gemm_launch(&g, st));
+            VG_HIP(vg_gemm_chain_launch(&g, st));
             vg_gemm_init(&g);
             for (int k = 0; k < 2; ++k) {
                 VgDim& d = c->d[k];
                 vg_gemm_add(&g, d.TM, d.m, 1, d.E, 1, d.m, d.Gw, d.m, d.m, d.m, d.m);
             }
-            VG_HIP(vg_gemm_launch(&g, st));
+            VG_HIP(vg_gemm_chain_launch(&g, st));
         }
     }
     VG_MARK(12);
@@ -1110,7 +1121,7 @@
             VgDim& d = c->d[k];
             vg_gemm_add(&g, d.QtPrev, d.m, 1, d.QtPrev2, 1, d.m, d.U, d.m, d.m, d.m, d.m);
         }
-    VG_HIP(vg_gemm_launch(&g, st));
+    VG_HIP(vg_gemm_chain_launch(&g, st));
     VG_MARK(14);
     vg_gemm_init(&g);
     for (int k = 0; k < 2; ++k) {
@@ -1127,7 +1138,7 @@
             vg_gemm_add(&g, Uk, d.m, 1, d.QtPrev, d.m, 1, d.Ep, d.m, d.m, d.m, d.m);
             vg_gemm_add(&g, Uk, d.m, 1, d.QtPrev, d.m, 1, d.Fp, d.m, d.m, d.m, d.m, 1, 0, 1, 0, 1.5, 0);
         }
-    VG_HIP(vg_gemm_launch(&g, st));
+    VG_HIP(vg_gemm_chain_launch(&g, st));
     VG_MARK(15);
 
     VgMspace ms;
@@ -1157,7 +1168,7 @@
             VgDim& d = c->d[k];
             vg_gemm_add(&g, d.Ep, d.m, 1, d.Ep, 1, d.m, d.Wp, d.m, d.m, d.m, d.m);
         }
-    VG_HIP(vg_gemm_launch(&g, st));
+    VG_HIP(vg_gemm_chain_launch(&g, st));
     VG_MARK(17);
     VG_HIP(vg_final_launch(&ms, st));
     VG_MARK(18);
@@ -2096,6 +2107,33 @@
     return VGGP_OK;
 }
 
+extern "C" int vggp_gemm_slabs(vggp_ctx* c, const double* A, int64_t sa_m, int64_t sa_k, int a_nslab, int64_t a_slab, const double* B,
+                               int64_t sb_k, int64_t sb_n, int b_nslab, int64_t b_slab, double* C, int64_t ldc, int64_t M, int64_t N,
+                               int64_t K, double alpha, int accum, int path, void* stream) {
+    if (!c) { vg_set_error("null context"); return VGGP_EINVAL; }
+    VG_REQUIRE(B && C && M >= 1 && N >= 1 && ldc >= N && (K >= 1 || !A), "vggp_gemm_slabs: bad argument");
+    VG_REQUIRE(M < (1L << 30) && N < (1L << 30) && K < (1L << 30), "vggp_gemm_slabs: dimension too large");
+    VG_REQUIRE(a_nslab >= 1 && b_nslab >= 1 && path >= 0 && path <= 2, "vggp_gemm_slabs: bad slab count or path");
+    VG_REQUIRE(A || path != 1, "vggp_gemm_slabs: the reduce-only form (A == NULL) exists in the panel kernel only");
+    VG_ENTER_DEVICE(c->device);
+    VgGemmBatch g;
+    vg_gemm_init(&g);
+    const int i = vg_gemm_add(&g, A, sa_m, sa_k, B, sb_k, sb_n, C, (int)ldc, (int)M, (int)N, A ? (int)K : 1, 1, 0, b_nslab, b_slab, alpha,
+                              accum ? 1 : 0);
+    g.p[i].a_nslab = A ? a_nslab : 1; g.p[i].a_slab = A ? a_slab : 0;
+    hipStream_t st = stream ? (hipStream_t)stream : c->own_stream;
+    if (path == 1) {
+        VG_HIP(vg_gemm_launch(&g, st));
+    } else if (path == 2) {
+        VG_REQUIRE(vg_gemm_panel_fits(&g), "vggp_gemm_slabs: the shape does not qualify for the panel kernel");
+        VG_HIP(vg_gemm_panel_launch(&g, st));
+    } else {
+        VG_REQUIRE(A || vg_gemm_panel_ok(&g), "vggp_gemm_slabs: the reduce-only form needs the panel kernel");
+        VG_HIP(vg_gemm_chain_launch(&g, st));
+    }
+    return VGGP_OK;
+}
+
 extern "C" int vggp_trsm(vggp_ctx* c, const double* L, int64_t m, const double* R, int64_t ncols, double* X, int trans,
                          void* stream) {
     if (!c) { vg_set_error("null context"); return VGGP_EINVAL; }
diff --git a/variational_gridded_gaussian_processes_amd/csrc/common.h b/variational_gridded_gaussian_processes_amd/csrc/common.h
--- a/variational_gridded_gaussian_processes_amd/csrc/common.h
+++ b/variational_gridded_gaussian_processes_amd/csrc/common.h
@@ -91,6 +91,11 @@
 void vg_gemm_xcd_group(VgGemmBatch* b, int prob);
 hipError_t vg_gemm_launch(const VgGemmBatch* b, hipStream_t st, int tag = 0);
 const char* vg_last_project_kernel();
+hipError_t vg_gemm_panel_setup();
+bool vg_gemm_panel_fits(const VgGemmBatch* b);
+bool vg_gemm_panel_ok(const VgGemmBatch* b);
+hipError_t vg_gemm_panel_launch(const VgGemmBatch* b, hipStream_t st);
+hipError_t vg_gemm_chain_launch(const VgGemmBatch* b, hipStream_t st);
 
 #define VG_RED_MAXSEG 8
 struct VgRedSeg { const double* in; double* out; long n; long slab; int nslab; int block_start; };
diff --git a/variational_gridded_gaussian_processes_amd/csrc/gemm_panel.hip b/variational_gridded_gaussian_processes_amd/csrc/gemm_panel.hip
--- /dev/null
+++ b/variational_gridded_gaussian_processes_amd/csrc/gemm_panel.hip
@@ -0,0 +1,230 @@
+#include "common.h"
+
+#include <cstdlib>
+
+typedef double vgp_d4 __attribute__((ext_vector_type(4)));
+
+#define VGP_T 32
+#define VGP_NT 256
+#define VGP_MAXSLAB 16
+#define VGP_MAXK 256
+
+typedef const __attribute__((address_space(1))) double* vgp_gptr;
+typedef const __attribute__((address_space(1))) char* vgp_gbytes;
+__device__ __forceinline__ double vgp_ld(const unsigned long long base, const unsigned off) {
+    return *reinterpret_cast<vgp_gptr>(reinterpret_cast<vgp_gbytes>(base) + off);
+}
+__device__ __forceinline__ unsigned long long vgp_uniform(const double* q) {
+    const unsigned long long a = reinterpret_cast<unsigned long long>(q);
+    const unsigned lo = __builtin_amdgcn_readfirstlane((unsigned)a), hi = __builtin_amdgcn_readfirstlane((unsigned)(a >> 32));
+    return ((unsigned long long)hi << 32) | lo;
+}
+
+template <int E, int S0, int NP, bool FIRST>
+__device__ __forceinline__ void vgp_slab_group(double (&v)[E], const double (&x)[E], const double* base, const unsigned (&off)[E],
+                                               const bool (&ok)[E], const long slab) {
+    double t[3][E];
+    unsigned long long sb[3];
+#pragma unroll
+    for (int u = 0; u < 3; ++u) sb[u] = vgp_uniform(base + (long)(S0 + (u < NP ? u : 0)) * slab);
+    unsigned o[E];
+#pragma unroll
+    for (int r = 0; r < E; ++r) { o[r] = off[r]; if (NP > 0) asm volatile("" : "+v"(o[r])); }
+#pragma unroll
+    for (int u = 0; u < 3; ++u)
+#pragma unroll
+        for (int r = 0; r < E; ++r) {
+            if (u < NP) {
+                const double y = vgp_ld(sb[u], o[r]);
+                t[u][r] = ok[r] ? y : 0.0;
+            } else {
+                t[u][r] = 0.0;
+            }
+        }
+    if (FIRST) {
+#pragma unroll
+        for (int r = 0; r < E; ++r) v[r] = ok[r] ? x[r] : 0.0;
+    }
+    if (NP > 0) {
+#pragma unroll
+        for (int r = 0; r < E; ++r) v[r] += (t[0][r] + t[1][r]) + t[2][r];
+    }
+}
+template <int E, int S0>
+__device__ __forceinline__ void vgp_rounds(double (&v)[E], const double (&x)[E], const double* base, const unsigned (&off)[E],
+                                           const bool (&ok)[E], const int nslab, const long slab) {
+    constexpr bool F = S0 == 1;
+    const int rem = nslab - S0;
+    if (rem <= 0) { if (F) vgp_slab_group<E, S0, 0, F>(v, x, base, off, ok, slab); return; }
+    if (rem == 1) { vgp_slab_group<E, S0, 1, F>(v, x, base, off, ok, slab); return; }
+    if (rem == 2) { vgp_slab_group<E, S0, 2, F>(v, x, base, off, ok, slab); return; }
+    vgp_slab_group<E, S0, 3, F>(v, x, base, off, ok, slab);
+    if constexpr (S0 + 3 < VGP_MAXSLAB) {
+        if (E > 8) __builtin_amdgcn_sched_barrier(0);
+        vgp_rounds<E, S0 + 3>(v, x, base, off, ok, nslab, slab);
+    }
+}
+
+template <int KC, int E, int RS>
+__device__ __forceinline__ void vgp_map(const long s_row, const long s_k, const int row0, const int R, const int k0, const int K,
+                                        unsigned (&off)[E], bool (&ok)[E], int (&l)[E]) {
+    const int tid = threadIdx.x;
+    const bool kc = (s_k == 1);
+#pragma unroll
+    for (int r = 0; r < E; ++r) {
+        const int row = kc ? tid / KC + (VGP_NT / KC) * r : tid % VGP_T;
+        const int k = kc ? tid % KC : tid / VGP_T + (VGP_NT / VGP_T) * r;
+        const int gr = row0 + row, gk = k0 + k;
+        ok[r] = gr < R && gk < K;
+        off[r] = (unsigned)((min(gr, R - 1) * s_row + min(gk, K - 1) * s_k) * (long)sizeof(double));
+        l[r] = row * RS + gk;
+    }
+}
+
+template <int KC, int NH>
+__device__ __forceinline__ void vgp_body(const VgGemmBatch& b, double* lds) {
+    constexpr int RS = KC * NH + 2;
+    constexpr int E = VGP_T * KC / VGP_NT;
+    const int bid = blockIdx.x;
+    int pi = 0;
+    for (int i = 1; i < b.nprob; ++i)
+        if (bid >= b.p[i].tile_start) pi = i;
+    const VgGemmP& p = b.p[pi];
+    const int t = bid - p.tile_start;
+    const int tm = t / p.tiles_n, tn = t - tm * p.tiles_n;
+    const int row0 = tm * VGP_T, col0 = tn * VGP_T;
+    const int tid = threadIdx.x;
+    const int M = p.M, N = p.N, K = p.K;
+
+    if (!p.A) {
+        constexpr int ER = VGP_T * VGP_T / VGP_NT;
+        unsigned off[ER];
+        bool ok[ER];
+        double x[ER], v[ER];
+#pragma unroll
+        for (int r = 0; r < ER; ++r) {
+            const int gr = row0 + tid / VGP_T + (VGP_NT / VGP_T) * r, gc = col0 + tid % VGP_T;
+            ok[r] = gr < M && gc < N;
+            off[r] = (unsigned)((min(gr, M - 1) * p.sb_k + min(gc, N - 1) * p.sb_n) * (long)sizeof(double));
+            x[r] = vgp_ld(vgp_uniform(p.B), off[r]);
+        }
+        vgp_rounds<ER, 1>(v, x, p.B, off, ok, p.b_nslab, p.b_slab);
+#pragma unroll
+        for (int r = 0; r < ER; ++r) {
+            const int gr = row0 + tid / VGP_T + (VGP_NT / VGP_T) * r, gc = col0 + tid % VGP_T;
+            if (ok[r]) {
+                const double w = p.alpha * v[r];
+                double* cp = p.C + (long)gr * p.ldc + gc;
+                *cp = p.accum ? *cp + w : w;
+            }
+        }
+        return;
+    }
+
+    double* As = lds;
+    double* Bs = lds + VGP_T * RS;
+#pragma unroll
+    for (int h = 0; h < NH; ++h) {
+        if (h * KC < K) {
+            unsigned oa[E], ob[E];
+            bool oka[E], okb[E];
+            int la[E], lb[E];
+            double xa[E], xb[E], ra[E], rb[E];
+            vgp_map<KC, E, RS>(p.sa_m, p.sa_k, row0, M, h * KC, K, oa, oka, la);
+            vgp_map<KC, E, RS>(p.sb_n, p.sb_k, col0, N, h * KC, K, ob, okb, lb);
+#pragma unroll
+            for (int r = 0; r < E; ++r) { xa[r] = vgp_ld(vgp_uniform(p.A), oa[r]); xb[r] = vgp_ld(vgp_uniform(p.B), ob[r]); }
+            vgp_rounds<E, 1>(rb, xb, p.B, ob, okb, p.b_nslab, p.b_slab);
+            vgp_rounds<E, 1>(ra, xa, p.A, oa, oka, p.a_nslab, p.a_slab);
+#pragma unroll
+            for (int r = 0; r < E; ++r) { As[la[r]] = ra[r]; Bs[lb[r]] = rb[r]; }
+            if (NH > 1) __builtin_amdgcn_sched_barrier(0);
+        }
+    }
+    __syncthreads();
+
+    const int lane = tid & 63, wave = tid >> 6;
+    const int wr = wave >> 1, wc = wave & 1;
+    const int fi = lane & 15, fk = lane >> 4;
+    const double* ap = As + (wr * 16 + fi) * RS + fk;
+    const double* bp = Bs + (wc * 16 + fi) * RS + fk;
+    vgp_d4 acc = (vgp_d4){0.0, 0.0, 0.0, 0.0};
+    const int kr = (K + 3) & ~3;
+#pragma unroll 8
+    for (int kk = 0; kk < kr; kk += 4) acc = __builtin_amdgcn_mfma_f64_16x16x4f64(ap[kk], bp[kk], acc, 0, 0, 0);
+
+    double* __restrict__ C = p.C;
+    const int ldc = p.ldc;
+#pragma unroll
+    for (int r = 0; r < 4; ++r) {
+        const int row = row0 + wr * 16 + fk + 4 * r;
+        const int col = col0 + wc * 16 + fi;
+        if (row < M && col < N) {
+            const double v = p.alpha * acc[r];
+            double* cp = C + (long)row * ldc + col;
+            *cp = p.accum ? *cp + v : v;
+        }
+    }
+}
+
+extern __shared__ double vg_gemm_panel_lds[];
+__global__ __launch_bounds__(VGP_NT) void vg_gemm_panel_k32_kernel(const VgGemmBatch b) { vgp_body<32, 1>(b, vg_gemm_panel_lds); }
+__global__ __launch_bounds__(VGP_NT) void vg_gemm_panel_k128_kernel(const VgGemmBatch b) { vgp_body<128, 1>(b, vg_gemm_panel_lds); }
+__global__ __launch_bounds__(VGP_NT) void vg_gemm_panel_k256_kernel(const VgGemmBatch b) { vgp_body<128, 2>(b, vg_gemm_panel_lds); }
+
+static constexpr size_t vgp_lds_bytes(int kmax) { return (size_t)2 * VGP_T * (kmax + 2) * sizeof(double); }
+
+hipError_t vg_gemm_panel_setup() {
+    hipError_t e = hipFuncSetAttribute(reinterpret_cast<const void*>(vg_gemm_panel_k128_kernel), hipFuncAttributeMaxDynamicSharedMemorySize,
+                                       (int)vgp_lds_bytes(128));
+    if (e != hipSuccess) return e;
+    return hipFuncSetAttribute(reinterpret_cast<const void*>(vg_gemm_panel_k256_kernel), hipFuncAttributeMaxDynamicSharedMemorySize,
+                               (int)vgp_lds_bytes(256));
+}
+
+bool vg_gemm_panel_fits(const VgGemmBatch* b) {
+    if (b->nprob == 0 || b->total_tiles == 0 || b->total_tiles >= 128) return false;
+    for (int i = 0; i < b->nprob; ++i) {
+        const VgGemmP& p = b->p[i];
+        if (p.ksplit != 1 || p.K < 1 || p.K > VGP_MAXK || p.tri != VG_TRI_NONE || p.rev || p.dotw || p.dot_out || p.xcd_group || !p.C || !p.B ||
+            p.a_nslab > VGP_MAXSLAB || p.b_nslab > VGP_MAXSLAB)
+            return false;
+        const long lim = 1L << 28;
+        if (p.sb_k < 0 || p.sb_n < 0 || (p.K - 1) * p.sb_k + (p.N - 1) * p.sb_n >= lim) return false;
+        if (!p.A) { if ((p.M - 1) * p.sb_k + (p.N - 1) * p.sb_n >= lim) return false; }
+        else if (p.sa_m < 0 || p.sa_k < 0 || (p.M - 1) * p.sa_m + (p.K - 1) * p.sa_k >= lim) return false;
+    }
+    return true;
+}
+
+bool vg_gemm_panel_ok(const VgGemmBatch* b) {
+    static const bool off = getenv("VGGP_NO_PANEL_GEMM") != nullptr;
+    return !off && vg_gemm_panel_fits(b);
+}
+
+hipError_t vg_gemm_panel_launch(const VgGemmBatch* b, hipStream_t st) {
+    if (!vg_gemm_panel_fits(b)) return hipErrorInvalidValue;
+    VgGemmBatch s = *b;
+    s.total_tiles = 0;
+    int kmax = 1;
+    for (int i = 0; i < s.nprob; ++i) {
+        VgGemmP& p = s.p[i];
+        p.tiles_m = (p.M + VGP_T - 1) / VGP_T;
+        p.tiles_n = (p.N + VGP_T - 1) / VGP_T;
+        p.tile_start = s.total_tiles;
+        s.total_tiles += p.tiles_m * p.tiles_n;
+        if (p.A && p.K > kmax) kmax = p.K;
+    }
+    if (s.total_tiles == 0) return hipSuccess;
+    if (kmax <= 32) hipLaunchKernelGGL(vg_gemm_panel_k32_kernel, dim3(s.total_tiles), dim3(VGP_NT), vgp_lds_bytes(32), st, s);
+    else if (kmax <= 128) hipLaunchKernelGGL(vg_gemm_panel_k128_kernel, dim3(s.total_tiles), dim3(VGP_NT), vgp_lds_bytes(128), st, s);
+    else hipLaunchKernelGGL(vg_gemm_panel_k256_kernel, dim3(s.total_tiles), dim3(VGP_NT), vgp_lds_bytes(256), st, s);
+    return hipGetLastError();
+}
+
+hipError_t vg_gemm_chain_launch(const VgGemmBatch* b, hipStream_t st) {
+    if (vg_gemm_panel_ok(b)) return vg_gemm_panel_launch(b, st);
+    for (int i = 0; i < b->nprob; ++i)
+        if (!b->p[i].A) return hipErrorInvalidValue;
+    return vg_gemm_launch(b, st);
+}
diff --git a/variational_gridded_gaussian_processes_amd/engine.py b/variational_gridded_gaussian_processes_amd/engine.py
--- a/variational_gridded_gaussian_processes_amd/engine.py
+++ b/variational_gridded_gaussian_processes_amd/engine.py
@@ -348,6 +348,25 @@
                                  B.stride(1), Cm.data_ptr(), N, M, N, K, _stream(self.device)))
         return Cm
 
+    def gemm_slabs(self, A, B: torch.Tensor, out: torch.Tensor = None, alpha: float = 1.0, accum: bool = False,
+                   path: int = 0) -> torch.Tensor:
+        for t in (A, B):
+            if t is not None and not (t.is_cuda and t.dtype == torch.float64 and t.dim() == 3):
+                raise TypeError("gemm_slabs operands must be 3-D float64 GPU tensors")
+        if A is not None:
+            _, M, K = A.shape
+            _, K2, N = B.shape
+            assert K == K2
+        else:
+            _, M, N = B.shape
+            K = 1
+        Cm = torch.empty(M, N, dtype=torch.float64, device=self.device) if out is None else out
+        assert Cm.shape == (M, N) and Cm.is_contiguous() and (out is not None or not accum)
+        a = (A.data_ptr(), A.stride(1), A.stride(2), A.shape[0], A.stride(0)) if A is not None else (None, 0, 0, 1, 0)
+        check(self.lib.vggp_gemm_slabs(self._h, *a, B.data_ptr(), B.stride(1), B.stride(2), B.shape[0], B.stride(0),
+                                       Cm.data_ptr(), N, M, N, K, alpha, 1 if accum else 0, path, _stream(self.device)))
+        return Cm
+
     def kron_solve(self, L1: torch.Tensor, L2: torch.Tensor, Y: torch.Tensor) -> torch.Tensor:
         n1, n2 = Y.shape
         X = torch.empty_like(Y)
```

New measurement: 5.414 billion grid-points/s. About the same (-0.9%).
